# ghy1228/LDPC_Error_Floor

Measured on AMD Instinct MI355X. Metric: decoded codewords/sec, wman N576 R3/4, 20 NMS iters, higher is better.
Workload: dtype i32

## Files before the change

include/ldpc_nms.h:

```cpp
#ifndef LDPC_NMS_H
#define LDPC_NMS_H

#include <stdint.h>

#ifdef __cplusplus
extern "C" {
#endif

#define LDPC_NMS_ABI_VERSION 3

typedef struct ldpc_graph ldpc_graph;
typedef struct ldpc_ctx ldpc_ctx;

enum ldpc_status {
    LDPC_OK = 0,
    LDPC_ERR_ARG = -1,
    LDPC_ERR_HIP = -2,
    LDPC_ERR_OOM = -3,
    LDPC_ERR_STATE = -4,
    LDPC_ERR_UNSUPPORTED = -5
};

enum ldpc_decoding_type {
    LDPC_DEC_SP = 0,
    LDPC_DEC_MS = 1,
    LDPC_DEC_QMS = 2,
    LDPC_DEC_MS_NONUDGE = 3
};

enum ldpc_kernel {
    LDPC_KERNEL_AUTO = 0,
    LDPC_KERNEL_FLOOD = 1,
    LDPC_KERNEL_FUSED = 2
};

typedef struct ldpc_decode_params {
    int32_t T;
    int32_t decoding_type;
    int32_t q_bit;
    int32_t target_bits;
    float clip_llr;
    int32_t kernel;
    int32_t outputs_size;
    int32_t reserved;
} ldpc_decode_params;

typedef struct ldpc_decode_outputs {
    float* app_all;
    uint32_t* hard_bits;
    uint32_t* synd_bits;
    int64_t* counters;
    uint8_t* frame_flags;
    uint32_t* iter_wrong;
} ldpc_decode_outputs;

int ldpc_abi_version(void);
const char* ldpc_status_string(int status);

int ldpc_graph_create(const int32_t* proto, int32_t M, int32_t N, int32_t z, int32_t device,
                      ldpc_graph** out);
int ldpc_graph_destroy(ldpc_graph* g);
int ldpc_graph_query(const ldpc_graph* g, int32_t* dims);

int ldpc_weights_set(ldpc_graph* g, int32_t T, const float* alpha, const float* alpha_ucn,
                     const float* beta);

int ldpc_ctx_create(ldpc_graph* g, int64_t B_max, int32_t T_max, ldpc_ctx** out);
int ldpc_ctx_destroy(ldpc_ctx* c);

int ldpc_decode(ldpc_ctx* c, const float* llr_dev, int64_t B, const ldpc_decode_params* p,
                const ldpc_decode_outputs* o, void* stream);

int ldpc_kernel_info(const ldpc_ctx* c, const ldpc_decode_params* p, int64_t* bytes_per_cw,
                     char* name, int32_t name_len);

int ldpc_ctx_last_kernel(const ldpc_ctx* c, char* name, int32_t name_len);

int ldpc_channel_awgn(float* llr_dev, int64_t B, int32_t n_vars, double sigma, uint64_t seed,
                      int64_t offset, int32_t decoding_type, int32_t q_bit, int32_t punct_start,
                      int32_t punct_end, int32_t short_start, int32_t short_end, float clip_llr,
                      void* stream);

typedef struct ldpc_channel_params {
    double sigma;
    uint64_t seed;
    int64_t offset;
    int32_t punct_start, punct_end, short_start, short_end;
    int32_t reserved[4];
} ldpc_channel_params;

int ldpc_decode_awgn(ldpc_ctx* ctx, int64_t B, const ldpc_decode_params* params,
                     const ldpc_channel_params* channel, const ldpc_decode_outputs* outputs,
                     void* stream);

int ldpc_awgn_in_kernel(const ldpc_ctx* ctx, const ldpc_decode_params* params, int32_t has_short,
                        int32_t app);

typedef struct ldpc_es_outputs {
    int32_t size;
    int32_t reserved;
    int64_t* counters;
    uint8_t* frame_flags;
    uint8_t* n_iter;
    int64_t* iter_hist;
} ldpc_es_outputs;

int ldpc_decode_es(ldpc_ctx* ctx, const float* llr_dev, int64_t B, const ldpc_decode_params* params,
                   const ldpc_es_outputs* es_outputs, void* stream);
int ldpc_decode_awgn_es(ldpc_ctx* ctx, int64_t B, const ldpc_decode_params* params,
                        const ldpc_channel_params* channel, const ldpc_es_outputs* es_outputs,
                        void* stream);
int ldpc_es_supported(const ldpc_ctx* ctx, const ldpc_decode_params* params);

typedef struct ldpc_word_outputs {
    int32_t size;
    int32_t reserved;
    uint32_t* hard_last;
    uint8_t* word_flags;
    int64_t* counters;
    uint8_t* frame_flags;
} ldpc_word_outputs;

int ldpc_decode_word(ldpc_ctx* ctx, const float* llr_dev, int64_t B, const ldpc_decode_params* params,
                     const ldpc_word_outputs* word_outputs, void* stream);
int ldpc_word_supported(const ldpc_ctx* ctx, const ldpc_decode_params* params);

typedef struct ldpc_es_word_outputs {
    int32_t size;
    int32_t reserved;
    uint32_t* hard_stop;
    uint8_t* word_flags;
    int64_t* counters;
    uint8_t* frame_flags;
    uint8_t* n_iter;
    int64_t* iter_hist;
    uint64_t reserved1;
} ldpc_es_word_outputs;

int ldpc_decode_es_word(ldpc_ctx* ctx, const float* llr_dev, int64_t B, const ldpc_decode_params* params,
                        const ldpc_es_word_outputs* outputs, void* stream);
int ldpc_decode_awgn_es_word(ldpc_ctx* ctx, int64_t B, const ldpc_decode_params* params,
                             const ldpc_channel_params* channel, const ldpc_es_word_outputs* outputs,
                             void* stream);
int ldpc_es_word_supported(const ldpc_ctx* ctx, const ldpc_decode_params* params);

int ldpc_channel_awgn_rows(float* rows_dev, const int64_t* idx_dev, int64_t n, int32_t n_vars,
                           double sigma, uint64_t seed, int64_t offset, int32_t decoding_type,
                           int32_t q_bit, int32_t punct_start, int32_t punct_end,
                           int32_t short_start, int32_t short_end, float clip_llr, void* stream);

int ldpc_collect_frames(const uint8_t* flags_dev, int64_t B, uint32_t mask, uint32_t want,
                        int64_t* idx_dev, int64_t cap, int64_t* count_dev, void* stream);

int ldpc_gather_rows(const float* src_dev, int64_t n_cols, const int64_t* idx_dev, int64_t n,
                     float* dst_dev, void* stream);

#define LDPC_UNCOR_ROW_BOUND(n_cols) (13 + 48 * (int64_t)(n_cols))
int ldpc_format_uncor_rows(const float* rows, int64_t n, int64_t n_cols, char* out, int64_t cap,
                           int64_t* len);

#ifdef __cplusplus
}
#endif
#endif
```

include/ldpc_nms_debug.h:

```cpp
#ifndef LDPC_NMS_DEBUG_H
#define LDPC_NMS_DEBUG_H

#include <stdint.h>

#ifdef __cplusplus
extern "C" {
#endif

int ldpc_debug_bs_bounds(const int32_t* proto, int32_t M, int32_t N, int32_t z, int32_t T,
                         int32_t mode, int32_t alpha_uniform, int32_t beta_uniform, float clip,
                         int32_t flags, int32_t* violations, char* msg, int32_t msg_len);

#ifdef __cplusplus
}
#endif

#endif
```

ldpc_error_floor_amd/build.py:

```python
from __future__ import annotations

import argparse
import os
import shutil
import subprocess
import sys
import sysconfig
from concurrent.futures import ThreadPoolExecutor

PKG = os.path.dirname(os.path.abspath(__file__))
ROOT = os.path.dirname(PKG)
CSRC = os.path.join(PKG, "csrc")
INCLUDE = os.path.join(ROOT, "include")
BUILD = os.path.join(PKG, "_build")
ARCH = os.environ.get("LDPC_OFFLOAD_ARCH", "gfx950")

HIP_SOURCES = ["ldpc_capi.hip", "ldpc_flood.hip", "ldpc_fused.hip", "ldpc_fused5.hip",
               "ldpc_bs.hip", "ldpc_bsc.hip", "ldpc_ffl.hip", "ldpc_channel.hip", "ldpc_collect.hip",
               "ldpc_word.hip"]
HEADERS = ["ldpc_internal.h", "ldpc_fused.h", "ldpc_fused5_kernel.h", "ldpc_bs_kernel.h", "ldpc_bs_host.h", "ldpc_bitplane.h",
           "ldpc_awgn.h", "ldpc_host.h", "ldpc_quant.h"]
HOST_SOURCES = ["ldpc_host.cpp"]
F5_SHAPE_SRC = "ldpc_fused5_shape.hip"
BS_INST_SRC = "ldpc_bs_inst.hip"


def _table_count(header, decl):
    import re
    src = open(os.path.join(CSRC, header)).read()
    body = src.split(decl, 1)[1].split("\n};", 1)[0]
    return len(re.findall(r"^\s*\{", body, re.M))


def _f5_shape_count():
    return _table_count("ldpc_fused5_kernel.h", "constexpr Shape5 kShapes5[] = {")


def _bs_inst_count():
    return _table_count("ldpc_bs_kernel.h", "constexpr BsInst kBsInst[] = {")
LIB = os.path.join(PKG, "libldpc_nms.so")
EXT = os.path.join(PKG, "_ldpc_nms" + sysconfig.get_config_var("EXT_SUFFIX"))


BS_INST_FLAGS = ["-mllvm", "-amdgpu-use-amdgpu-trackers"]


def source_fingerprint() -> str:
    import hashlib
    h = hashlib.sha256()
    files = sorted(HIP_SOURCES + HEADERS + HOST_SOURCES + [F5_SHAPE_SRC, BS_INST_SRC])
    for f in files:
        with open(os.path.join(CSRC, f), "rb") as fh:
            h.update(f.encode() + b"\0" + fh.read())
    with open(os.path.join(INCLUDE, "ldpc_nms.h"), "rb") as fh:
        h.update(fh.read())
    h.update(" ".join(_flags()).encode())
    h.update(" ".join(BS_INST_FLAGS).encode())
    return h.hexdigest()[:16]


def _flags(absolute=False):
    inc = (INCLUDE, CSRC) if absolute else (os.path.relpath(INCLUDE, ROOT), os.path.relpath(CSRC, ROOT))
    return ["--offload-arch=" + ARCH, "-O3", "-std=c++17", "-fPIC", "-ffp-contract=off",
            "-I" + inc[0], "-I" + inc[1], "-Wall", "-Wno-unused-result",
            "-mllvm", "-pragma-unroll-threshold=500000"]


def _hipcc():
    for cand in (os.environ.get("HIPCC"), "/opt/rocm/bin/hipcc", shutil.which("hipcc")):
        if cand and os.path.exists(cand):
            return cand
    raise RuntimeError("hipcc not found (ROCm required to build the HIP extension)")


def _newer(target, deps):
    if not os.path.exists(target):
        return True
    t = os.path.getmtime(target)
    return any(os.path.getmtime(d) > t for d in deps if os.path.exists(d))


def _run(cmd):
    r = subprocess.run(cmd, capture_output=True, text=True)
    if r.returncode != 0:
        raise RuntimeError(f"build failed: {' '.join(cmd)}\n{r.stdout}\n{r.stderr}")
    return r


def build(force=False, jobs=4, verbose=False):
    os.makedirs(BUILD, exist_ok=True)
    hipcc = _hipcc()
    hdrs = [os.path.join(CSRC, h) for h in HEADERS] + [os.path.join(INCLUDE, "ldpc_nms.h")]
    flags = _flags(absolute=True)
    objs, jobs_list = [], []
    units = [(src, src.replace(".hip", ".o"), []) for src in HIP_SOURCES]
    units += [(src, src.replace(".cpp", ".o"), []) for src in HOST_SOURCES]
    units += [(F5_SHAPE_SRC, f"ldpc_fused5_s{i}.o", [f"-DF5_SHAPE={i}"])
              for i in range(_f5_shape_count())]
    units += [(BS_INST_SRC, f"ldpc_bs_i{i}.o", [f"-DBS_INST={i}"] + BS_INST_FLAGS)
              for i in range(_bs_inst_count())]
    for src, obj, defs in units:
        s = os.path.join(CSRC, src)
        o = os.path.join(BUILD, obj)
        objs.append(o)
        if force or _newer(o, [s] + hdrs + [os.path.abspath(__file__)]):
            jobs_list.append([hipcc] + flags + defs + ["-c", s, "-o", o])
    with ThreadPoolExecutor(max_workers=max(1, jobs)) as ex:
        for r in ex.map(_run, jobs_list):
            if verbose and r.stderr:
                print(r.stderr, file=sys.stderr)
    if force or _newer(LIB, objs):
        _run([hipcc, "--offload-arch=" + ARCH, "-shared", "-fPIC", "-o", LIB] + objs)
    py_src = os.path.join(CSRC, "pybind_module.cpp")
    if force or _newer(EXT, [py_src, LIB, os.path.join(INCLUDE, "ldpc_nms.h")]):
        import pybind11
        cxx = os.environ.get("CXX", "g++")
        _run([cxx, "-O2", "-std=c++17", "-shared", "-fPIC", "-fvisibility=hidden",
              "-I" + pybind11.get_include(), "-I" + sysconfig.get_paths()["include"],
              "-I" + INCLUDE, py_src, "-o", EXT, "-L" + PKG, "-lldpc_nms",
              "-Wl,-rpath,$ORIGIN"])
    return LIB, EXT


def main():
    ap = argparse.ArgumentParser()
    ap.add_argument("--force", action="store_true")
    ap.add_argument("--jobs", type=int, default=min(8, os.cpu_count() or 1))
    a = ap.parse_args()
    lib, ext = build(force=a.force, jobs=a.jobs, verbose=True)
    print(lib)
    print(ext)


if __name__ == "__main__":
    main()
```

ldpc_error_floor_amd/csrc/ldpc_bs.hip:

```cpp
#include <algorithm>
#include <array>
#include <cmath>
#include <cstdio>
#include <cstdlib>
#include <cstring>
#include <functional>
#include <string>
#include <utility>
#include <vector>

#include "ldpc_bs_host.h"

namespace ldpc {
namespace bs {

__global__ void k_bs_tables(const float* __restrict__ alpha, const float* __restrict__ alpha_ucn,
                            const float* __restrict__ beta, const int32_t* __restrict__ row_ptr,
                            int T, int E, int N, int arows, int ar, int bcols, float step, float inv,
                            int qmax, float cu, uint32_t* alut, uint32_t* blut) {
    const int f = blockIdx.x * blockDim.x + threadIdx.x;
    const int na = T * ar, nbt = T * bcols;
    if (f >= na + nbt) return;
    int g[16];
    uint32_t* out;
// ... 36 lines not shown
    int inst = -1, nw = 0, cn_lanes = 0, arows = 1, bcols = 1;
    uint32_t off_slots = 0, off_pad = 0, off_zero = 0, off_red = 0, off_alut = 0, off_blut = 0, off_hdz = 0,
             off_ch = 0, off_hdl = 0;
    uint32_t off_esu = 0;
    int cn_dmin = 0;
    bool ucn = false;
    bool colalign = false;
    float cu = 0.f;
    size_t lds = 0;
    std::vector<int32_t> lay;
};

static uint32_t q8_tab_lds(const BsPlan& p) { return p.off_slots; }
static bool q8_tab_fits(const BsPlan& p) {
    return (size_t)(p.off_pad - p.off_slots) >= sizeof(uint32_t) * AWGN_TAB_W;
}

static bool colalign_fits(const host::GraphTables& h, int nw_packed) {
    return h.z <= 32 && 32 * h.N <= 64 * 16 && (32 * h.N + 63) / 64 <= nw_packed + 1;
}

std::vector<int32_t> slot_layout_rows(const host::GraphTables& h, const std::vector<int>& rl, size_t* nslot) {
    std::vector<int32_t> lay((size_t)2 * h.M, 0);
    size_t cur = 0;
    for (int i = 0; i < h.M; ++i) {
        const int LPC = rl[(size_t)i], sep = 32 / LPC;
        auto ok = [&](int A) {
            for (int d = 1; d < LPC; ++d) {
                const int r = (d * A) % 32;
                if (std::min(r, 32 - r) < sep) return false;
            }
            return true;
        };
        const int deg = h.row_ptr[i + 1] - h.row_ptr[i];
        size_t first = cur;
        if (i > 0) first += (size_t)((((int64_t)lay[2 * (i - 1)] + h.z - (int64_t)cur) % 32 + 32) % 32);
        int A = ((deg + LPC - 1) / LPC) * h.z;
        while (!ok(A)) ++A;
        const int last_rows = (deg - (LPC - 1) + LPC - 1) / LPC;
        cur = first + (size_t)(LPC - 1) * A + (size_t)std::max(last_rows, 0) * h.z;
        lay[2 * i] = (int32_t)first;
        lay[2 * i + 1] = A;
    }
    *nslot = cur;
    return lay;
}
std::vector<int32_t> slot_layout(const host::GraphTables& h, int LPC, size_t* nslot) {
    return slot_layout_rows(h, std::vector<int>((size_t)h.M, LPC), nslot);
}

bool bs_mode(int mode) { return mode == MODE_Q5 || mode == MODE_QM5 || mode == MODE_Q4 || mode == MODE_Q3; }
float bs_step(int mode) { return mode == MODE_Q5 ? 0.5f : mode == MODE_Q3 ? 2.0f : 1.0f; }
int bs_qmax(int mode) { return mode == MODE_Q4 ? 7 : mode == MODE_Q3 ? 3 : QMAX; }
static float mode_step_bs(int mode) { return bs_step(mode); }

static BsPlan plan_inst(const DevGraph& g, int i, bool ucn, float clip, int min_cdeg, int mode, int T) {
    BsPlan p;
    const BsInst& k = kBsInst[i];
    const host::GraphTables& h = *g.host;
    if (h.max_cdeg > k.D || h.max_vdeg > k.DV || (ucn && !k.UCN)) return p;
    p.inst = i;
    p.ucn = ucn;
    const int nv = g.n_vars, nc = g.n_checks;
    p.cn_lanes = 64 * ((k.LPC * nc + 63) / 64);
    int vch = (nv + 63) / 64;
    const int cch = p.cn_lanes / 64;
    if (k.VPL == 1 && k.CPL == 1) {
        static const int eca = [] { const char* e = getenv("LDPC_BS_COLALIGN"); return e ? atoi(e) : 1; }();
        p.colalign = eca != 0 && colalign_fits(h, std::max(vch, cch));
        if (p.colalign) vch = (32 * h.N + 63) / 64;
    }
    if (k.VPL == 1 && k.CPL == 1) p.nw = std::max(vch, cch);
    else p.nw = std::max((vch + k.VPL - 1) / k.VPL, (cch + k.CPL - 1) / k.CPL);
    if (p.nw > 16) return p;
    if (k.VPL > 1 || k.CPL > 1) {
        p.nw = 16;
        if (vch > k.VPL * p.nw || cch > k.CPL * p.nw) return p;
    }
    const char* eap = getenv("LDPC_BS_AROWS");
    p.arows = ((g.w_alpha_uniform && !ucn) || (g.w_alpha_pair_uniform && !(eap && atoi(eap) == 0))) ? 1 : h.M;
    p.bcols = g.w_beta_uniform ? 1 : h.N;
    p.cn_dmin = (p.cn_lanes == k.LPC * nc) ? min_cdeg : 0;
    if (k.BIG) {
        const float cu = clip / mode_step_bs(mode);
        if (cu > (float)bs_qmax(mode)) p.cu = cu;
    }
    size_t nslot = 0;
    p.lay = slot_layout(h, k.LPC, &nslot);
    size_t o = 0;
    if (k.UCN) {
        p.off_hdz = (uint32_t)(4 * (size_t)nv);
        o = ((size_t)4 * (nv + 1) + 127) & ~(size_t)127;
    }
    p.off_slots = (uint32_t)o;
    p.off_pad = (uint32_t)(o + nslot * SLOT_B);
    p.off_zero = p.off_pad + SLOT_B;
    const size_t slot_end = (size_t)p.off_zero + SLOT_B;
    if (k.PK && slot_end > 65535) return p;
    if (k.UCN && p.off_hdz > 65535) return p;
    o = (slot_end + 15) & ~(size_t)15;
    p.off_red = (uint32_t)o;
    o += 64 + (((size_t)4 * T + 15) & ~(size_t)15) + 4 * FLORW;
    if (k.ES) {
        p.off_esu = (uint32_t)o;
        o += ((size_t)4 * T + 15) & ~(size_t)15;
    }
    p.off_alut = (uint32_t)o;
    o += (size_t)2 * (k.UCN ? 2 : 1) * p.arows * LUT_W * 4;
    p.off_blut = (uint32_t)o;
    o += (size_t)2 * p.bcols * BLUT_W * 4;
    if (k.PK && k.CPL == 1 && (k.ES ? (size_t)p.off_alut + (size_t)p.arows * LUT_W * 4 : o) > 65535) return p;
    if (k.CPL == 1) {
        p.off_ch = (uint32_t)o;
        o += (size_t)4 * 64 * p.nw;
    }
    if (k.UCN && k.CPL == 1) {
        const int EPL = (k.D + k.LPC - 1) / k.LPC, HDW = (EPL + 1) / 2;
        p.off_hdl = (uint32_t)o;
        o += (size_t)4 * HDW * 64 * p.nw;
    }
    p.lds = (o + 15) & ~(size_t)15;
    if (p.lds > BS_LDS_MAX) return p;
    p.ok = true;
    return p;
}

BsPlan bs_plan(const DevGraph& g, int mode, bool ucn, bool per_edge_w, float clip, int T, bool es = false) {
    BsPlan p;
    const char* e = getenv("LDPC_BS");
    if (e && atoi(e) == 0) return p;
    const char* el = getenv("LDPC_BS_LPC");
    const int want_lpc = el ? atoi(el) : 0;
    const char* ei = getenv("LDPC_BS_INST");
    const int want_inst = ei ? atoi(ei) : -1;
    if (!bs_mode(mode)) return p;
    if (per_edge_w || !g.host || !g.w_beta_nonneg) return p;
    const host::GraphTables& h = *g.host;
    int min_cdeg = 1 << 30;
    for (int i = 0; i < h.M; ++i) min_cdeg = std::min(min_cdeg, h.row_ptr[i + 1] - h.row_ptr[i]);
    if (min_cdeg < 2) return p;
    for (int i = 0; i < kBsNInst; ++i) {
        if (kBsInst[i].ES != es) continue;
        if (es) {
            BsPlan q = plan_inst(g, i, ucn, clip, min_cdeg, mode, T);
            if (q.ok) return q;
            continue;
        }
        if (want_lpc != 0 && want_lpc != kBsInst[i].LPC) continue;
        if (want_inst >= 0 && want_inst != i) continue;
        BsPlan q = plan_inst(g, i, ucn, clip, min_cdeg, mode, T);
        if (q.ok) return q;
    }
    return p;
}

#ifndef BS_DEAL_DEFAULT
#define BS_DEAL_DEFAULT 2
#endif
std::vector<int> deal_chunks(const std::vector<int>& cost, int nw, int cap) {
    const int n = (int)cost.size();
    std::vector<int> order(n), slot((size_t)nw * cap, -1);
    for (int c = 0; c < n; ++c) order[c] = c;
    std::stable_sort(order.begin(), order.end(), [&](int x, int y) { return cost[x] > cost[y]; });
    const char* e = getenv("LDPC_BS_DEAL");
    if (e && atoi(e) == 0) {
        std::vector<int> used(nw, 0), load(4, 0);
        for (int c : order) {
            int best = -1, bw = -1;
            for (int sm = 0; sm < 4; ++sm) {
                int w_s = -1;
                for (int w = sm; w < nw; w += 4)
                    if (used[w] < cap && (w_s < 0 || used[w] < used[w_s])) w_s = w;
                if (w_s >= 0 && (best < 0 || load[sm] < load[best])) { best = sm; bw = w_s; }
            }
            slot[(size_t)bw * cap + used[bw]] = c;
            ++used[bw];
            load[best] += cost[c];
        }
        return slot;
    }
    const int deal_mode = e ? atoi(e) : BS_DEAL_DEFAULT;
    if (deal_mode == 2 && cap == 1 && n <= nw && nw <= 16) {
        int slots[4] = {0, 0, 0, 0};
        for (int w = 0; w < nw; ++w) ++slots[w % 4];
        std::vector<int> cur(n, -1), best(n, -1);
        int load[4] = {0, 0, 0, 0}, used[4] = {0, 0, 0, 0};
        long long best_key = -1;
        std::function<void(int)> rec = [&](int i) {
            const int mx = std::max(std::max(load[0], load[1]), std::max(load[2], load[3]));
            if (best_key >= 0 && (long long)mx * 1000000 > best_key) return;
            if (i == n) {
                const long long key = (long long)mx * 1000000 + (long long)load[0] * load[0] + (long long)load[1] * load[1] +
                                      (long long)load[2] * load[2] + (long long)load[3] * load[3];
                if (best_key < 0 || key < best_key) { best_key = key; best = cur; }
                return;
            }
            for (int sm = 0; sm < 4; ++sm) {
                if (used[sm] >= slots[sm]) continue;
                bool dup = false;
                for (int q = 0; q < sm; ++q)
                    if (used[q] < slots[q] && load[q] == load[sm] && slots[q] - used[q] == slots[sm] - used[sm]) dup = true;
                if (dup) continue;
                load[sm] += cost[order[i]];
                ++used[sm];
                cur[i] = sm;
                rec(i + 1);
                load[sm] -= cost[order[i]];
                --used[sm];
            }
        };
        rec(0);
        int next[4] = {0, 1, 2, 3};
        for (int i = 0; i < n; ++i) {
            const int sm = best[i];
            slot[(size_t)next[sm]] = order[i];
            next[sm] += 4;
        }
        return slot;
    }
    std::vector<std::vector<int>> vch(nw);
    std::vector<int> vload(nw, 0);
    for (int c : order) {
        int best = -1;
        for (int w = 0; w < nw; ++w)
            if ((int)vch[w].size() < cap &&
                (best < 0 || vload[w] < vload[best] || (vload[w] == vload[best] && vch[w].size() < vch[best].size())))
                best = w;
        vch[best].push_back(c);
        vload[best] += cost[c];
    }
    std::vector<int> vorder(nw), sload(4, 0), next(4);
    for (int w = 0; w < nw; ++w) vorder[w] = w;
    std::stable_sort(vorder.begin(), vorder.end(), [&](int x, int y) { return vload[x] > vload[y]; });
    for (int sm = 0; sm < 4; ++sm) next[sm] = sm;
    for (int v : vorder) {
        int sm = -1;
        for (int q = 0; q < 4; ++q)
            if (next[q] < nw && (sm < 0 || sload[q] < sload[sm])) sm = q;
        const int w = next[sm];
        next[sm] += 4;
        sload[sm] += vload[v];
        for (size_t u = 0; u < vch[v].size(); ++u) slot[(size_t)w * cap + u] = vch[v][u];
    }
    return slot;
}

std::vector<int32_t> uniform_lanes(const host::GraphTables& h, int LPC, int cn_lanes) {
    std::vector<int32_t> lanes((size_t)cn_lanes, -1);
    const int nc = h.M * h.z;
    for (int ql = 0; ql < cn_lanes; ++ql)
        if (ql / LPC < nc) lanes[(size_t)ql] = (ql / LPC) | ((ql % LPC) << 16) | (LPC << 20);
    return lanes;
}

std::vector<int> check_chunk_cost_lanes(const host::GraphTables& h, const std::vector<int32_t>& lanes) {
    const int cch = (int)(lanes.size() / 64);
    std::vector<int> cost(cch, 2);
    for (int ch = 0; ch < cch; ++ch) {
        int pos = 0;
        for (int l = 0; l < 64; ++l) {
            const int32_t d = lanes[(size_t)64 * ch + l];
            if (d < 0) continue;
            const int i = (d & 0xFFFF) / h.z, L = (d >> 20) & 15;
            pos = std::max(pos, (h.row_ptr[i + 1] - h.row_ptr[i] + L - 1) / L);
        }
        cost[ch] += pos;
    }
    return cost;
}
std::vector<int> check_chunk_cost(const host::GraphTables& h, int LPC, int cch) {
    return check_chunk_cost_lanes(h, uniform_lanes(h, LPC, 64 * cch));
}

std::vector<int> column_rotation_lanes(const host::GraphTables& h, int EPL, const std::vector<int32_t>& lanes) {
    const int z = h.z, cn_lanes = (int)lanes.size();
    std::vector<int> toff(h.N, 0);
    {
        std::vector<std::vector<std::pair<int, int>>> grp;
        std::vector<std::vector<int>> bycol(h.N);
        for (int h0 = 0; h0 < cn_lanes; h0 += 32)
            for (int m = 0; m < EPL; ++m) {
                std::vector<std::pair<int, int>> gl;
                for (int ql = h0; ql < h0 + 32 && ql < cn_lanes; ++ql) {
                    const int32_t d = lanes[(size_t)ql];
                    if (d < 0) continue;
                    const int cc = d & 0xFFFF, cj = (d >> 16) & 15, LPC = (d >> 20) & 15;
                    const int i = cc / z, hc = cc - i * z, kk = LPC * m + cj;
                    if (kk >= h.row_ptr[i + 1] - h.row_ptr[i]) continue;
                    const int pe = h.row_ptr[i] + kk;
                    gl.emplace_back(h.pe_col[pe], (hc + h.pe_shift[pe]) % z);
                }
                if (gl.empty()) continue;
                for (const auto& x : gl)
                    if (bycol[x.first].empty() || bycol[x.first].back() != (int)grp.size())
                        bycol[x.first].push_back((int)grp.size());
                grp.push_back(std::move(gl));
            }
        auto gcost = [&](const std::vector<std::pair<int, int>>& gl) {
            int cnt[32] = {0}, mx = 0, sq = 0;
            uint32_t seen[32];
            int ns = 0;
            for (const auto& x : gl) {
                const uint32_t t = (uint32_t)(x.first * z + (x.second + toff[x.first]) % z);
                bool dup = false;
                for (int q = 0; q < ns && !dup; ++q) dup = seen[q] == t;
                if (dup) continue;
// ... 134 lines not shown
    int vcost_before = 0, vcost_after = 0;
    std::vector<uint32_t> A((size_t)64 * DV);
    std::vector<int> dl(64);
    for (int w = 0; w < p.nw; ++w)
        for (int u = 0; u < k.VPL; ++u) {
            const int ch = vslot[(size_t)w * k.VPL + u];
            int dmax = 0, dmin = 1 << 30;
            if (ch < 0) {
                wdeg[3 * ((size_t)u * p.nw + w)] = -1;
                wdeg[3 * ((size_t)u * p.nw + w) + 1] = 0;
                wdeg[3 * ((size_t)u * p.nw + w) + 2] = -1;
                continue;
            }
            int col = -2;
            std::fill(A.begin(), A.end(), p.off_zero);
            std::fill(dl.begin(), dl.end(), 0);
            for (int l = 0; l < 64; ++l) {
                const int o = 64 * ch + l;
                if (o >= nvo || order[o] < 0) { dmin = 0; continue; }
                const int v = order[o], j = v / z, hh = v - j * z;
                col = (col == -2 || col == j) ? j : -1;
                const int c0 = h.col_ptr[j], dv = h.col_ptr[j + 1] - c0;
                for (int f = 0; f < dv; ++f) {
                    const int pe = h.col_pe[c0 + f], i = h.pe_row[pe];
                    int hc = hh - h.pe_shift[pe];
                    hc = hc < 0 ? hc + z : hc;
                    A[(size_t)l * DV + f] = slot_addr(i, pe - h.row_ptr[i], hc);
                }
                dl[l] = dv;
                dmax = std::max(dmax, dv);
                dmin = std::min(dmin, dv);
            }
            if (vorder) {
                const std::pair<int, int> c = host::order_variable_edges(A, dl, DV, std::min(DV, dmax));
                vcost_before += c.first;
                vcost_after += c.second;
            }
            for (int l = 0; l < 64; ++l) {
                const int o = 64 * ch + l;
                if (o >= nvo || order[o] < 0) continue;
                uint32_t* q = &vn[((size_t)u * nl + 64 * w + l) * VNW];
                for (int pw = 0; pw < VNA; ++pw) q[pw] = 0u;
                for (int f = 0; f < DV; ++f) put(q, f, A[(size_t)l * DV + f]);
                q[VNA] = k.UCN ? ((uint32_t)order[o] | (hd_index(order[o]) << 16)) : (uint32_t)order[o];
            }
            wdeg[3 * ((size_t)u * p.nw + w)] = dmax;
            wdeg[3 * ((size_t)u * p.nw + w) + 1] = dmin;
            wdeg[3 * ((size_t)u * p.nw + w) + 2] = col < 0 ? -1 : col;
        }
    if (getenv("LDPC_BS_VORDER_LOG"))
        fprintf(stderr, "bsl variable-phase bank cycles per slot word: %d -> %d\n", vcost_before, vcost_after);
    const int cch = p.cn_lanes / 64;
    std::vector<int32_t> cchunk((size_t)p.nw * k.CPL, -1);
    if (k.CPL == 1 && k.VPL == 1) {
        for (int w = 0; w < p.nw; ++w) cchunk[w] = w < cch ? w : -1;
    } else {
        const std::vector<int> cs = deal_chunks(check_chunk_cost(h, LPC, cch), p.nw, k.CPL);
        for (size_t x = 0; x < cs.size(); ++x) cchunk[x] = cs[x];
    }
    std::vector<uint32_t> chd;
    if (k.UCN) {
        chd.assign((size_t)p.cn_lanes * HDW, 0u);
        for (int ql = 0; ql < p.cn_lanes; ++ql) {
            const int cc = ql / LPC, cj = ql % LPC;
            for (int m = 0; m < EPL; ++m) {
                uint32_t addr = p.off_hdz;
                const int kk = LPC * m + cj;
                if (cc < g.n_checks) {
                    const int i = cc / z, hc = cc - i * z;
                    if (kk < h.row_ptr[i + 1] - h.row_ptr[i]) {
                        const int pe = h.row_ptr[i] + kk;
                        const int v = h.pe_col[pe] * z + (hc + h.pe_shift[pe]) % z;
                        addr = 4 * hd_index(v);
                    }
                }
                chd[(size_t)ql * HDW + (m >> 1)] |= addr << (16 * (m & 1));
            }
        }
    }
    BsHostTables t;
    t.vn.swap(vn);
    t.wdeg.swap(wdeg);
    t.cchunk.swap(cchunk);
    t.chd.swap(chd);
    return t;
}
static int bs_graph_tables(const DevGraph& g, const BsPlan& p, void*& graph, int& inst, hipStream_t s) {
    if (graph && inst != p.inst) {
        (void)hipFree(graph);
        graph = nullptr;
    }
    if (graph) return LDPC_OK;
    BsHostTables t = bs_host_tables(g, p);
    const std::vector<uint32_t>& vn = t.vn;
    const std::vector<int32_t>& wdeg = t.wdeg;
    const std::vector<int32_t>& cchunk = t.cchunk;
    const std::vector<uint32_t>& chd = t.chd;
    const size_t nwords = vn.size() + wdeg.size() + p.lay.size() + cchunk.size() + chd.size();
    void* d = nullptr;
    if (hipMalloc(&d, nwords * 4) != hipSuccess) { (void)hipGetLastError(); return LDPC_ERR_OOM; }
    uint32_t* dp = reinterpret_cast<uint32_t*>(d);
    size_t at = 0;
    bool ok = true;
    auto up = [&](const void* src, size_t n) {
        if (n) ok = ok && hipMemcpyAsync(dp + at, src, n * 4, hipMemcpyHostToDevice, s) == hipSuccess;
        at += n;
    };
    up(vn.data(), vn.size());
    up(wdeg.data(), wdeg.size());
    up(p.lay.data(), p.lay.size());
    up(cchunk.data(), cchunk.size());
    up(chd.data(), chd.size());
    if (!ok || hipStreamSynchronize(s) != hipSuccess) {
        (void)hipFree(d);
        return LDPC_ERR_HIP;
    }
    graph = d;
    inst = p.inst;
    return LDPC_OK;
}

static BsPlan bs_route(const DevGraph& g, const BsReq& r, bool* to_bsc) {
    BsPlan p = bs_plan(g, r.mode, r.ucn, r.per_edge_w, r.clip, r.T, r.es);
    *to_bsc = !p.ok && (!r.es || !bs_plan(g, r.mode, r.ucn, r.per_edge_w, r.clip, r.T).ok);
    return p;
}

bool bs_supported(const DevGraph& g, const BsReq& r) {
    bool to_bsc;
    return bs_route(g, r, &to_bsc).ok || (to_bsc && bsc_supported(g, r));
}

bool bs_q8_ok(const DevGraph& g, const BsReq& r, bool has_short) {
    bool to_bsc;
    const BsPlan p = bs_route(g, r, &to_bsc);
    if (!p.ok) return to_bsc && bsc_q8_ok(g, r, has_short);
    return (!has_short || p.cu > 0.f) && q8_tab_fits(p);
}

const char* bs_kernel_name(const DevGraph& g, const BsReq& r) {
    static thread_local char buf[64];
    bool to_bsc;
    const BsPlan p = bs_route(g, r, &to_bsc);
    if (!p.ok) return to_bsc ? bsc_kernel_name(g, r) : "";
    const BsInst& k = kBsInst[p.inst];
    char x[16] = "";
    if (k.VPL > 1 || k.CPL > 1) snprintf(x, sizeof(x), ",x%d/%d", k.VPL, k.CPL);
    snprintf(buf, sizeof(buf), "bsl[p32,w%d,d%d,v%d,l%d%s%s%s]", p.nw, k.D, k.DV, k.LPC, x, p.ucn ? ",ucn" : "",
             r.es ? ",es" : "");
    return buf;
}

static int bs_run(const DevGraph& g, const Bufs& b, FusedWorkspace& ws, const BsPlan& p, const float* llr,
                  const BsReq& r, const BsOut& o, hipStream_t s) {
    void*& graph = r.es ? ws.bs_es_graph : ws.bs_graph;
    int st = bs_graph_tables(g, p, graph, r.es ? ws.bs_es_graph_inst : ws.bs_graph_inst, s);
    if (st != LDPC_OK) return st;
    const BsInst& k = kBsInst[p.inst];
    const float step = mode_step_bs(r.mode);
    const int ar = (k.UCN ? 2 : 1) * p.arows;
    uint32_t *alut = nullptr, *blut = nullptr;
    st = bs_make_tables(b, g, p.arows, ar, p.bcols, step, bs_qmax(r.mode), p.cu, r.ucn, ws, &alut, &blut, s);
    if (st != LDPC_OK) return st;
    const int DV = k.DV;
    const int VNW = (k.PK ? (DV + 1) / 2 : DV) + 1;
    const uint32_t* gt = reinterpret_cast<const uint32_t*>(graph);
    BsLaunch a{};
    a.n_iter = o.n_iter;
    a.iter_hist = o.iter_hist;
    a.hdw = o.hdw;
    a.word = o.word ? 1 : 0;
    a.llr = llr;
    a.gen = bs_gen(b, q8_tab_lds(p));
    a.B = b.B;
    a.n_vars = g.n_vars;
    a.n_checks = g.n_checks;
    a.T = b.T;
    a.target_bits = b.target_bits;
    a.cn_lanes = p.cn_lanes;
    a.cn_dmin = p.cn_dmin;
    a.fold_wave = p.cn_lanes < 64 * p.nw ? (uint32_t)(p.nw - 1) : (p.nw > 1 ? 1u : 0u);
    a.inv = 1.0f / step;
    a.cu = p.cu > 0.f ? p.cu : -1.f;
    a.qmax = bs_qmax(r.mode);
    a.ucn = p.ucn ? 1 : 0;
    a.ucn_iter = g.w_ucn_iter;
    a.beta_id = g.w_beta_id_mask;
    a.row_ptr = g.row_ptr;
    a.z = g.z;
    a.vn_tab = gt;
    const size_t nvt = (size_t)k.VPL * 64 * p.nw * VNW;
    a.vn_wdeg = reinterpret_cast<const int32_t*>(gt + nvt);
    a.row_lay = a.vn_wdeg + 3 * (size_t)k.VPL * p.nw;
    a.cn_chunk = a.row_lay + 2 * (size_t)g.M;
    a.cn_hd = reinterpret_cast<const uint32_t*>(a.cn_chunk + (size_t)p.nw * k.CPL);
    a.alut = alut;
    a.blut = blut;
    a.arows = p.arows;
    a.bcols = p.bcols;
    a.btid = (bs_qmax(r.mode) == QMAX && !getenv("LDPC_BS_NOBFIX")) ? g.beta_tid : nullptr;
    a.btid_n = g.N;
    a.counters = o.counters;
    a.flags = o.flags;
    a.bad = o.bad;
    a.iter_wrong = r.es ? nullptr : b.iter_wrong;
    a.hdx = o.hdx;
    bs_stagger(k.VPL > 1 || k.CPL > 1, &a.stagger, &a.stagger_n);
    a.off_slots = p.off_slots;
    a.off_pad = p.off_pad;
    a.off_zero = p.off_zero;
    a.off_red = p.off_red;
    a.off_alut = p.off_alut;
    a.off_blut = p.off_blut;
    a.off_hdz = p.off_hdz;
    a.off_hdl = p.off_hdl;
    a.off_ch = p.off_ch;
    if (const char* e = getenv("LDPC_DIAG_ABLATE")) a.ablate = atoi(e);
    const int npacks = (int)((b.B + PACK - 1) / PACK);
    int grid = -1;
    if (const char* e = getenv("LDPC_BS_GRID")) grid = std::max(atoi(e), 0);
    static const auto kLaunch = launch_table(std::make_integer_sequence<int, kBsNInst>{});
    static const size_t lds_min = [] { const char* e = getenv("LDPC_BS_LDS_MIN"); return e ? (size_t)atol(e) : 0; }();
    const size_t lds = std::min(std::max(p.lds, lds_min), (size_t)BS_LDS_MAX);
    const uint64_t rkey = (uint64_t)p.inst << 48 | (uint64_t)p.nw << 32 | (uint64_t)lds;
    if (ws.bs_resident_key != rkey) {
        ws.bs_resident_key = rkey;
        std::fill(ws.bs_resident, ws.bs_resident + 3, 0);
    }
#ifdef BS_STAMP
    static unsigned long long* dst = nullptr;
    if (!dst && hipMalloc(reinterpret_cast<void**>(&dst), 256 * 8) != hipSuccess) return LDPC_ERR_OOM;
    if (hipMemsetAsync(dst, 0, 256 * 8, s) != hipSuccess) return LDPC_ERR_HIP;
    a.stamps = dst;
    st = kLaunch[p.inst](a, npacks, p.nw, lds, s, b.q8 != nullptr, grid, ws.bs_resident);
    unsigned long long hst[256];
    if (st != LDPC_OK || hipMemcpyAsync(hst, dst, sizeof(hst), hipMemcpyDeviceToHost, s) != hipSuccess ||
        hipStreamSynchronize(s) != hipSuccess)
        return st != LDPC_OK ? st : LDPC_ERR_HIP;
    fprintf(stderr, "bs_stamp inst %d T %d q8 %d: per pack, shader clocks [check, check-barrier, var, var-barrier | "
            "entry, channel, ch-barrier, tables, first-var, check-setup | epilogue]\n", p.inst, b.T, b.q8 != nullptr);
    static const int order[] = {0, 1, 2, 3, 8, 9, 10, 11, 12, 4, 5};
    for (int w = 0; w < p.nw && w < 16; ++w) {
        const double n = (double)(hst[16 * w + 15] ? hst[16 * w + 15] : 1);
        fprintf(stderr, "  wave %2d:", w);
        for (const int i : order) fprintf(stderr, " %8.0f", hst[16 * w + i] / n);
        fprintf(stderr, "  | SIMD %5.3f %5.3f %5.3f %5.3f\n", (hst[16 * w + 13] & 0xFFFFFFFFull) / n,
                (hst[16 * w + 13] >> 32) / n, (hst[16 * w + 14] & 0xFFFFFFFFull) / n, (hst[16 * w + 14] >> 32) / n);
    }
    return st;
#else
    return kLaunch[p.inst](a, npacks, p.nw, lds, s, b.q8 != nullptr, grid, ws.bs_resident);
#endif
}

int bs_decode(const DevGraph& g, const Bufs& b, FusedWorkspace& ws, const float* llr, const BsReq& r,
              const BsOut& o, hipStream_t s) {
    bool to_bsc;
    const BsPlan p = bs_route(g, r, &to_bsc);
    if (!p.ok) return to_bsc ? bsc_decode(g, b, ws, llr, r, o, s) : LDPC_ERR_UNSUPPORTED;
    return bs_run(g, b, ws, p, llr, r, o, s);
}

}

namespace ldpc {
namespace bs {
struct BoundsReport {
    int violations = 0;
    std::string first;
    void fail(const char* what, long long idx, long long lim) {
        if (violations++ == 0) {
            char buf[160];
            snprintf(buf, sizeof(buf), "%s: index %lld outside [0, %lld)", what, idx, lim);
            first = buf;
        }
    }
    void in(const char* what, long long idx, long long lim) {
        if (idx < 0 || idx >= lim) fail(what, idx, lim);
    }
    void lds(const char* what, long long a, long long n, long long lo, long long hi) {
        if (a < lo || a + n > hi) fail(what, a, hi);
    }
    void apart(const char* what, long long a, long long n, long long b, long long m) {
        if (a < b + m && b < a + n) fail(what, a + n, b);
    }
};

static int bs_bounds_check(const DevGraph& g, const BsPlan& p, const BsHostTables& t, int T, int flags,
                           BoundsReport& r) {
    const BsInst& k = kBsInst[p.inst];
    const host::GraphTables& h = *g.host;
    const int LPC = k.LPC, VPL = k.VPL, CPL = k.CPL, DV = k.DV;
    const int EPL = (k.D + LPC - 1) / LPC, HDW = (EPL + 1) / 2, OB = 4 / LPC;
    const int VNA = k.PK ? (DV + 1) / 2 : DV, VNW = VNA + 1;
    const int NT = 64 * p.nw, nwv = p.nw, nv = g.n_vars, z = h.z;
    const bool UCN = k.UCN, ucn = UCN && (p.ucn || k.ES);
    const int AR = UCN ? 2 * p.arows : p.arows;
    const long long AL = (long long)AR * LUT_W, BL = (long long)p.bcols * BLUT_W;
    const long long lds = (long long)p.lds;
    const bool SKIPM = CPL > 1;
    const bool GBL = CPL == 1;
    const bool HDL = UCN && CPL == 1;
    if (getenv("LDPC_BOUNDS_VERBOSE"))
        fprintf(stderr, "bs plan: inst %d nw %d ucn %d lds %lld (slots %u..%u, alut %u, blut %u, ch %u, hdl %u)\n",
                p.inst, p.nw, (int)p.ucn, lds, p.off_slots, p.off_pad, p.off_alut, p.off_blut, p.off_ch, p.off_hdl);
    r.in("lds size", lds, (long long)BS_LDS_MAX + 1);
    if ((long long)t.vn.size() != (long long)VPL * NT * VNW) r.fail("vn_tab size", (long long)t.vn.size(), (long long)VPL * NT * VNW);
    r.lds("RED", p.off_red, 4LL * (16 + ((T + 3) & ~3) + FLORW), 0, k.ES ? p.off_esu : p.off_alut);
    if (k.ES) {
        r.lds("syndrome words", p.off_esu, 4LL * T, p.off_red, p.off_alut);
        r.apart("syndrome words / RED", p.off_esu, 4LL * T, p.off_red, 4LL * (16 + ((T + 3) & ~3) + FLORW));
        if (p.off_esu != p.off_red + 4u * (uint32_t)(16 + ((T + 3) & ~3) + FLORW)) r.fail("syndrome words' offset", p.off_esu, p.off_red);
        if (p.off_alut & 15) r.fail("alpha tables off 16 B", p.off_alut & 15, 1);
    }
    r.lds("ALUT", p.off_alut, 4 * 2 * AL, 0, p.off_blut);
    r.lds("BLUT", p.off_blut, 4 * 2 * BL, 0, lds);
    r.lds("PAD+ZERO", p.off_pad, 2 * SLOT_B, p.off_slots, p.off_red);
    if (UCN) r.lds("HD", 0, 4LL * (nv + 1), 0, p.off_slots);
    if (q8_tab_fits(p)) {
        const long long tb = q8_tab_lds(p);
        const long long tn = (flags & LDPC_BOUNDS_BIG_TABLES) ? (long long)(p.off_pad - p.off_slots) + 4
                                                              : 4LL * AWGN_TAB_W;
        r.lds("channel tables", tb, tn, p.off_slots, p.off_pad);
        if (UCN) r.apart("channel tables / HD", tb, tn, 0, 4LL * (nv + 1));
        r.apart("channel tables / PAD+ZERO", tb, tn, p.off_pad, 2 * SLOT_B);
        r.apart("channel tables / RED", tb, tn, p.off_red, (long long)p.off_alut - p.off_red);
        r.apart("channel tables / ALUT", tb, tn, p.off_alut, 4 * 2 * AL);
        r.apart("channel tables / BLUT", tb, tn, p.off_blut, 4 * 2 * BL);
    }
    for (int u = 0; u < VPL; ++u)
        for (int w = 0; w < nwv; ++w) {
            const long long wi = 3LL * (u * nwv + w);
            r.in("vn_wdeg", wi + 2, (long long)t.wdeg.size());
            if (wi + 2 >= (long long)t.wdeg.size()) continue;
            const int dw = t.wdeg[(size_t)wi], pcol = t.wdeg[(size_t)wi + 2];
            if (pcol >= 0) r.in("btid column", pcol, h.N);
            if (dw >= 0 && T > 1) {
                const long long col = p.bcols == 1 ? 0 : pcol;
                if (col >= 0) r.in("btid", (long long)(T - 1) * h.N + col, (long long)T * h.N);
            }
            for (int l = 0; l < 64; ++l) {
                const long long ti = ((long long)u * NT + 64LL * w + l) * VNW;
                r.in("vn_tab", ti + VNA, (long long)t.vn.size());
                if (ti + VNA >= (long long)t.vn.size()) continue;
                const uint32_t* q = &t.vn[(size_t)ti];
                const int vv = (int)q[VNA];
                const int v = (UCN && vv >= 0) ? (vv & 0xFFFF) : vv;
                if (v >= nv) r.fail("variable", v, nv);
                if (vv >= 0 && UCN) r.in("HD index", (long long)((uint32_t)vv >> 16), nv);
                if (vv >= 0 && p.bcols > 1) r.in("beta table", v / (nv / p.bcols), p.bcols);
                for (int f = 0; f < DV && f < dw; ++f) {
                    const uint32_t a = k.PK ? ((f & 1) ? (q[f >> 1] >> 16) : (q[f >> 1] & 0xFFFFu)) : q[f];
                    if (a != p.off_zero) r.lds("variable slot", a, SLOT_B, p.off_slots, p.off_pad);
                }
            }
        }
    for (int w = 0; w < nwv; ++w)
        for (int c = 0; c < CPL; ++c) {
            r.in("cn_chunk", (long long)w * CPL + c, (long long)t.cchunk.size());
            const int gchunk = CPL == 1 ? w : t.cchunk[(size_t)w * CPL + c];
            const bool active = CPL == 1 ? w * 64 < p.cn_lanes : gchunk >= 0;
            int gm = EPL;
            if (SKIPM) {
                uint32_t any = 0u;
                for (int l = 0; l < 64; ++l) {
                    const int ql = std::max(gchunk, 0) * 64 + l, cc = ql / LPC;
                    const int ci = std::min(cc / z, g.n_checks / z - 1);
                    const int gdeg = cc < g.n_checks ? h.row_ptr[ci + 1] - h.row_ptr[ci] : 0;
                    any |= (1u << ((gdeg + LPC - 1) / LPC)) - 1u;
                }
                gm = __builtin_popcount(any);
                if (active) r.in("real positions - 1 (the min2 switch)", gm - 1, EPL);
            }
            for (int l = 0; l < 64; ++l) {
                const int ql = std::max(gchunk, 0) * 64 + l, cc = ql / LPC, cj = l % LPC;
                const int ci = std::min(cc / z, g.n_checks / z - 1);
                r.in("row_ptr", ci + 1, h.M + 1);
                r.in("row_lay", 2LL * ci + 1, (long long)p.lay.size());
                const int gdeg = cc < g.n_checks ? h.row_ptr[ci + 1] - h.row_ptr[ci] : 0;
                if (UCN) {
                    const bool guard = (flags & LDPC_BOUNDS_PRE_GUARD) ? true : ql < p.cn_lanes;
                    if (ucn && gchunk >= 0 && guard)
                        for (int pp = 0; pp < HDW; ++pp) r.in("cn_hd", (long long)ql * HDW + pp, (long long)t.chd.size());
                }
                if (GBL) r.lds("per-lane words", p.off_ch + 4LL * (64 * w + l), 4, p.off_ch, lds);
                if (HDL)
                    for (int pp = 0; pp < HDW; ++pp) r.lds("HD addresses", p.off_hdl + 4LL * (pp * NT + 64 * w + l), 4, p.off_hdl, lds);
                if (!active) continue;
                const long long gbase = p.off_slots +
                    ((long long)p.lay[2 * ci] + (long long)cj * p.lay[2 * ci + 1] + (cc - ci * z)) * SLOT_B;
                for (int m = 0; m < EPL; ++m) {
                    if (SKIPM && m >= gm) continue;
                    const bool re = LPC * m + LPC - 1 < p.cn_dmin || LPC * m + cj < gdeg;
                    const long long a = re ? gbase + (long long)m * z * SLOT_B : p.off_pad;
                    r.lds("check slot", a, SLOT_B, p.off_slots, p.off_red);
                    if (re && a + SLOT_B > p.off_pad) r.fail("check slot past the slot region", a, p.off_pad);
                    if (ucn && cc < g.n_checks && ql < p.cn_lanes && (size_t)ql * HDW + (m >> 1) < t.chd.size()) {
                        const uint32_t hw = t.chd[(size_t)ql * HDW + (m >> 1)];
                        const uint32_t ha = (m & 1) ? (hw >> 16) : (hw & 0xFFFFu);
                        r.lds("HD read", ha, 4, 0, (long long)p.off_hdz + 4);
                    }
                }
                const long long ctab = p.off_alut + (long long)(p.arows > 1 ? ci : 0) * LUT_W * 4 + (long long)cj * OB * 64;
                const long long last = ctab + 4LL * AL + (UCN ? (long long)p.arows * LUT_W * 4 : 0) + (OB - 1) * 64 + 3 * 16;
                r.lds("alpha table", ctab, 16, p.off_alut, p.off_alut + 4 * 2 * AL);
                if (k.PK && CPL == 1) r.in("packed alpha-table address", ctab, 65536);
                r.lds("alpha table (odd t, alpha')", last, 16, p.off_alut, p.off_alut + 4 * 2 * AL);
            }
        }
    return r.violations;
}
}
}

extern "C" int ldpc_debug_bs_bounds(const int32_t* proto, int32_t M, int32_t N, int32_t z, int32_t T,
                                    int32_t mode, int32_t alpha_uniform, int32_t beta_uniform,
                                    float clip, int32_t flags, int32_t* violations, char* msg,
                                    int32_t msg_len) {
    using namespace ldpc;
    using namespace ldpc::bs;
    if (!proto || !violations || T <= 0) return LDPC_ERR_ARG;
    host::GraphTables h;
    const int st = host::build_graph(proto, M, N, z, h);
    if (st != LDPC_OK) return st;
    DevGraph g{};
    g.M = h.M; g.N = h.N; g.z = h.z; g.E = h.E;
    g.n_checks = h.M * h.z; g.n_vars = h.N * h.z; g.n_edges = h.E * h.z; g.max_cdeg = h.max_cdeg;
    g.h_row_ptr = h.row_ptr.data();
    g.host = &h;
    g.w_alpha_uniform = alpha_uniform;
    g.w_alpha_pair_uniform = alpha_uniform;
    g.w_beta_uniform = beta_uniform;
    g.w_beta_nonneg = 1;
    int min_cdeg = 1 << 30;
    for (int i = 0; i < h.M; ++i) min_cdeg = std::min(min_cdeg, h.row_ptr[i + 1] - h.row_ptr[i]);
    int checked = 0;
    *violations = 0;
    std::string first;
    for (int i = 0; i < kBsNInst; ++i)
        for (int u = 0; u < 2; ++u) {
            if (kBsInst[i].ES && !(flags & LDPC_BOUNDS_ES)) continue;
            const BsPlan p = plan_inst(g, i, u != 0, clip, min_cdeg, mode, T);
            if (!p.ok) continue;
            const BsHostTables t = bs_host_tables(g, p);
            BoundsReport r;
            bs_bounds_check(g, p, t, T, flags, r);
            ++checked;
            if (r.violations && first.empty()) {
                char buf[64];
                snprintf(buf, sizeof(buf), "instance %d%s: ", i, u ? " ucn" : "");
                first = std::string(buf) + r.first;
            }
            *violations += r.violations;
        }
    for (int b1 = 0; b1 < 2; ++b1) {
        if (b1 && !beta_uniform) continue;
        g.w_beta_one = b1;
        BoundsReport r;
        const int n = bsc_debug_bounds(g, mode, clip, T, flags, r.violations, r.first);
        if (n <= 0) continue;
        ++checked;
        if (r.violations && first.empty()) first = std::string(b1 ? "bsc beta=1: " : "bsc: ") + r.first;
        *violations += r.violations;
    }
    g.w_beta_one = 1;
    if ((flags & LDPC_BOUNDS_ES_BSC) && beta_uniform && !bs_plan(g, mode, false, false, clip, T).ok) {
        BoundsReport r;
        if (bsc_debug_bounds(g, mode, clip, T, flags, r.violations, r.first, true) > 0) {
            ++checked;
            if (r.violations && first.empty()) first = std::string("bsc early stop: ") + r.first;
            *violations += r.violations;
        }
    }
    if (msg && msg_len > 0) {
        std::strncpy(msg, first.c_str(), (size_t)msg_len - 1);
        msg[msg_len - 1] = 0;
    }
    return checked;
}
```

ldpc_error_floor_amd/csrc/ldpc_bs_kernel.h:

```cpp
#pragma once
#include <type_traits>
#include <cstdint>

#include "ldpc_beta_tabs.h"
#include "ldpc_fused.h"
#include "ldpc_fused5_kernel.h"
#include "ldpc_bitplane.h"

namespace ldpc {
namespace bs {

constexpr int PACK = 32;
constexpr int SLOT_W = 5;
constexpr int SLOT_B = SLOT_W * 4;
constexpr int LUT_W = 64;
constexpr int BLUT_W = LUT_W + 4;
constexpr int QMAX = 15;
constexpr size_t BS_LDS_MAX = 160 * 1024;

struct BsInst { int D, DV, LPC, VPL, CPL; bool UCN, BIG, PK; int WPE; bool ES = false; };
constexpr BsInst kBsInst[] = {
    {15, 6, 4, 1, 1, false, false, true, 8},
    {16, 8, 4, 1, 1, false, false, true, 8},
    {15, 6, 2, 1, 1, false, false, true, 8},
    {24, 4, 4, 1, 1, true, true, true, 6},
    {10, 8, 2, 2, 2, false, true, false, 4},
    {10, 8, 2, 2, 2, true, true, false, 4},
    {10, 8, 4, 2, 3, true, true, false, 4},
    {15, 6, 4, 1, 1, true, false, true, 6, true},
    {24, 4, 4, 1, 1, true, true, true, 6, true},
};
constexpr int kBsNInst = sizeof(kBsInst) / sizeof(kBsInst[0]);

struct BsGen {
    const uint32_t* tab;
    uint32_t k0, k1;
    int64_t offset;
    int nb, kmin;
    int ps, pe, ss, se;
    uint32_t lds;
};

struct BsArgs {
    const float* llr;
    int64_t B;
    int n_vars, n_checks, T, target_bits, cn_lanes, cn_dmin;
    float inv;
    float cu;
    int qmax;
    int ucn;
    uint64_t beta_id;
    const int32_t* row_ptr;
    const int32_t* row_lay;
    int z;
    const uint32_t* vn_tab;
    const int32_t* vn_wdeg;
    const int32_t* cn_chunk;
    const uint32_t* cn_hd;
    const uint32_t* alut;
    const uint32_t* blut;
    int arows, bcols;
    const int32_t* btid;
    int btid_n;
    int64_t* counters;
    uint8_t* flags;
    uint32_t* bad;
    uint32_t* iter_wrong;
    int stagger, stagger_n;
    uint32_t* hdx;
    uint32_t off_slots, off_pad, off_zero, off_red, off_alut, off_blut, off_hdz;
    uint32_t fold_wave;
    uint32_t off_ch;
    int ablate;
    uint64_t ucn_iter;
    uint32_t off_hdl;
    BsGen gen;
    unsigned long long* stamps;
};

struct BsArgsEs : BsArgs {
    uint8_t* n_iter;
    int64_t* iter_hist;
};

struct BsArgsEw : BsArgsEs {
    uint32_t* hdw;
};

struct BsArgsXp : BsArgs {
    int word;
};

template <class A>
__device__ __forceinline__ const __attribute__((address_space(4))) A& kern_args() {
    return *(const __attribute__((address_space(4))) A*)__builtin_amdgcn_kernarg_segment_ptr();
}

typedef unsigned int v4u __attribute__((ext_vector_type(4)));
typedef __attribute__((address_space(3))) uint32_t LdsW;
typedef __attribute__((address_space(3))) v4u LdsQ;

__device__ __forceinline__ uint32_t lds_w(uint32_t addr) { return *reinterpret_cast<const LdsW*>(addr); }
__device__ __forceinline__ v4u lds_q(uint32_t addr) { return *reinterpret_cast<const LdsQ*>(addr); }
__device__ __forceinline__ void lds_put(uint32_t addr, uint32_t x) { *reinterpret_cast<LdsW*>(addr) = x; }

__device__ __forceinline__ void read_slot(uint32_t& n, uint32_t (&M)[4], uint32_t addr) {
    const LdsW* p = reinterpret_cast<const LdsW*>(addr);
    n = p[0];
    M[0] = p[1];
    M[1] = p[2];
    M[2] = p[3];
    M[3] = p[4];
}
__device__ __forceinline__ void write_slot(uint32_t addr, uint32_t n, const uint32_t (&M)[4]) {
    LdsW* p = reinterpret_cast<LdsW*>(addr);
    p[0] = n;
    p[1] = M[0];
    p[2] = M[1];
    p[3] = M[2];
    p[4] = M[3];
}

template <int NI>
__device__ __forceinline__ void lut(uint32_t (&o)[NI][4], const uint32_t (&in)[NI][4], uint32_t tab) {
    uint32_t tj = tab;
#pragma unroll
    for (int j = 0; j < 4; ++j) {
        if (j > 0) asm volatile("" : "+v"(tj) : "v"(o[0][j - 1]));
        uint32_t g[NI][4];
#pragma unroll
        for (int q = 0; q < 4; ++q) {
            const v4u w = lds_q(tj + (uint32_t)(j * 64 + q * 16));
#pragma unroll
            for (int u = 0; u < NI; ++u) {
                const uint32_t l0 = B3(T_LEAF, in[u][0], w.x, w.y), l1 = B3(T_LEAF, in[u][0], w.z, w.w);
                g[u][q] = mux(in[u][1], l1, l0);
            }
        }
#pragma unroll
        for (int u = 0; u < NI; ++u)
            o[u][j] = mux(in[u][3], mux(in[u][2], g[u][3], g[u][2]), mux(in[u][2], g[u][1], g[u][0]));
    }
}

typedef __attribute__((address_space(4))) const uint32_t ConstW;
__device__ __forceinline__ uint32_t leaf_s(uint32_t m, uint32_t X, uint32_t Y) {
    uint32_t t, l;
    asm("v_and_b32 %0, %1, %2" : "=v"(t) : "s"(X), "v"(m));
    asm("v_xor_b32 %0, %1, %2" : "=v"(l) : "s"(Y), "v"(t));
    return l;
}
__device__ __forceinline__ void lut_s(uint32_t (&o)[4], const uint32_t (&a)[4], const ConstW* tab) {
#pragma unroll
    for (int j = 0; j < 4; ++j) {
        uint32_t g[4];
#pragma unroll
        for (int q = 0; q < 4; ++q) {
            const uint32_t l0 = leaf_s(a[0], tab[j * 16 + 4 * q], tab[j * 16 + 4 * q + 1]);
            const uint32_t l1 = leaf_s(a[0], tab[j * 16 + 4 * q + 2], tab[j * 16 + 4 * q + 3]);
            g[q] = mux(a[1], l1, l0);
// ... 134 lines not shown
    a = X[0][3] | cand[0];
#pragma unroll
    for (int m = 1; m < K; ++m) a = B3(T_ANDOR, a, X[m][3], cand[m]);
    a = grp_and<LPC>(a);
    m2[3] = a;
#pragma unroll
    for (int m = 0; m < K; ++m) c2[m] = B3(T_NANDEQ, cand[m], X[m][3], a);
#pragma unroll
    for (int i = 2; i >= 0; --i) {
        a = X[0][i] | ~c2[0];
#pragma unroll
        for (int m = 1; m < K; ++m) a = B3(T_ANDORN, a, X[m][i], c2[m]);
        a = grp_and<LPC>(a);
        m2[i] = a;
        if (i > 0) {
#pragma unroll
            for (int m = 0; m < K; ++m) c2[m] = B3(T_ANDEQ, c2[m], X[m][i], a);
        }
    }
#pragma unroll
    for (int i = 0; i < 4; ++i) m2[i] = mux(two, m1[i], m2[i]);
}

#ifdef BS_DIAG
#define ABL(bit) (a.ablate & (bit))
#else
#define ABL(bit) 0
#endif
#ifdef BS_MARK
#define PH(name, k) asm volatile(";@ph " name ".%0" ::"i"(k))
#define PH4(name, k, x) asm volatile(";@ph " name ".%4" : "+v"(x[0]), "+v"(x[1]), "+v"(x[2]), "+v"(x[3]) : "i"(k))
#define PH8(name, k, x, y)                                                                        \
    asm volatile(";@ph " name ".%8" : "+v"(x[0]), "+v"(x[1]), "+v"(x[2]), "+v"(x[3]), "+v"(y[0]),  \
                 "+v"(y[1]), "+v"(y[2]), "+v"(y[3]) : "i"(k))
#define PH9(name, k, x, y, z)                                                                     \
    asm volatile(";@ph " name ".%9" : "+v"(x[0]), "+v"(x[1]), "+v"(x[2]), "+v"(x[3]), "+v"(y[0]),  \
                 "+v"(y[1]), "+v"(y[2]), "+v"(y[3]), "+v"(z) : "i"(k))
#else
#define PH(name, k) ((void)0)
#define PH4(name, k, x) ((void)0)
#define PH8(name, k, x, y) ((void)0)
#define PH9(name, k, x, y, z) ((void)0)
#endif
__device__ __forceinline__ void t8x8(uint32_t& lo, uint32_t& hi) {
    uint32_t t;
    t = B3((TA ^ TB) & TC, lo, lo >> 7, 0x00AA00AAu);
    lo = B3(T_XOR3, lo, t, t << 7);
    t = B3((TA ^ TB) & TC, hi, hi >> 7, 0x00AA00AAu);
    hi = B3(T_XOR3, hi, t, t << 7);
    t = B3((TA ^ TB) & TC, lo, lo >> 14, 0x0000CCCCu);
    lo = B3(T_XOR3, lo, t, t << 14);
    t = B3((TA ^ TB) & TC, hi, hi >> 14, 0x0000CCCCu);
    hi = B3(T_XOR3, hi, t, t << 14);
    t = B3((TA ^ TB) & TC, lo, hi << 4, 0xF0F0F0F0u);
    lo ^= t;
    hi ^= t >> 4;
}
template <bool BIG>
__device__ __forceinline__ void pack_bytes(const uint32_t (&D)[8], uint32_t valid, uint32_t& cs,
                                           uint32_t (&cm)[4], uint32_t& bg) {
    uint32_t lo[4], hi[4];
#pragma unroll
    for (int g = 0; g < 4; ++g) {
        lo[g] = D[2 * g];
        hi[g] = D[2 * g + 1];
        t8x8(lo[g], hi[g]);
    }
    const uint32_t a = __builtin_amdgcn_perm(lo[1], lo[0], 0x06020400u), b = __builtin_amdgcn_perm(lo[1], lo[0], 0x07030501u);
    const uint32_t c = __builtin_amdgcn_perm(lo[3], lo[2], 0x06020400u), d = __builtin_amdgcn_perm(lo[3], lo[2], 0x07030501u);
    const uint32_t L0 = __builtin_amdgcn_perm(c, a, 0x05040100u) & valid, L2 = __builtin_amdgcn_perm(c, a, 0x07060302u) & valid;
    const uint32_t L1 = __builtin_amdgcn_perm(d, b, 0x05040100u) & valid, L3 = __builtin_amdgcn_perm(d, b, 0x07060302u) & valid;
    const uint32_t e = __builtin_amdgcn_perm(hi[1], hi[0], 0x05010400u), f = __builtin_amdgcn_perm(hi[3], hi[2], 0x05010400u);
    const uint32_t n = ~__builtin_amdgcn_perm(f, e, 0x05040100u) & valid;
    bg = BIG ? (__builtin_amdgcn_perm(f, e, 0x07060302u) & valid) : 0u;
    cs = n;
    cm[0] = L0;
    cm[1] = B3(T_XAND, L1, n, L0);
    cm[2] = B3(T_XAND, L2, n, L0 | L1);
    cm[3] = B3(T_XAND, L3, n, L0 | L1 | L2);
}
template <bool BIG>
__device__ __forceinline__ int pack_channel(const float (&xv)[PACK], float inv, int qmax, float cu,
                                            uint32_t valid, uint32_t& cs, uint32_t (&cm)[4], uint32_t& bg) {
    const float qf = (float)qmax;
    uint32_t D[8];
    int off = 0;
#pragma unroll
    for (int k = 0; k < 8; ++k) D[k] = 0u;
#pragma unroll
    for (int r = 0; r < PACK; ++r) {
        const float x = xv[r] * inv;
        const float q = __builtin_amdgcn_fmed3f(rintf(x), -qf, qf);
        const bool big = BIG && fabsf(x) == cu;
        off |= (q != x && !big) ? 1 : 0;
        D[r >> 2] = __builtin_amdgcn_cvt_pk_u8_f32(q + (big ? 48.f : 16.f), r & 3, D[r >> 2]);
    }
    pack_bytes<BIG>(D, valid, cs, cm, bg);
    return off;
}
typedef unsigned int v2u_g __attribute__((ext_vector_type(2)));
typedef __attribute__((address_space(3))) const v2u_g LdsU2;
__device__ __forceinline__ void gen_bytes(const BsGen& g, int64_t pk, int v, int qmax, uint32_t (&D)[8]) {
    const int bit = v + 1;
    if (g.ss > 0 && bit >= g.ss && bit <= g.se) {
#pragma unroll
        for (int i = 0; i < 8; ++i) D[i] = (uint32_t)(48 - qmax) * 0x01010101u;
        return;
    }
    if (g.ps > 0 && bit >= g.ps && bit <= g.pe) {
#pragma unroll
        for (int i = 0; i < 8; ++i) D[i] = 0x10101010u;
        return;
    }
    LdsU2* bucket = reinterpret_cast<LdsU2*>((uintptr_t)g.lds);
    const LdsW* thi = reinterpret_cast<const LdsW*>((uintptr_t)(g.lds + 8u * (1u << AWGN_KB)));
    const LdsW* tlo = thi + AWGN_NB_MAX;
    const uint64_t g0 = (uint64_t)g.offset + (uint64_t)pk * 32u;
    const int sh = (int)(g.offset & 3);
    const uint32_t boff = (uint32_t)(16 + g.kmin);
    auto word = [&](const int (&l)[4]) __attribute__((always_inline)) -> uint32_t {
        return ((uint32_t)l[0] + boff) | ((uint32_t)l[1] + boff) << 8 | ((uint32_t)l[2] + boff) << 16 |
               ((uint32_t)l[3] + boff) << 24;
    };
#pragma unroll
    for (int i = 0; i < 8; ++i) {
        const uint64_t gq = (g0 + 4u * (uint32_t)i) >> 2;
        int la[4];
        awgn_levels4b(g, bucket, thi, tlo, (uint32_t)v, gq, la);
        uint32_t w = word(la);
        if (sh) {
            int lb[4];
            awgn_levels4b(g, bucket, thi, tlo, (uint32_t)v, gq + 1, lb);
            w = __builtin_amdgcn_alignbyte(word(lb), w, (uint32_t)sh);
        }
        D[i] = w;
    }
}
__device__ __forceinline__ void gen_tables(const BsGen& g, int tid, int NT) {
    copy_async(g.lds, g.tab, AWGN_TAB_W, __builtin_amdgcn_readfirstlane(tid >> 6), NT);
}

constexpr double STAGGER_US = 60.0;
constexpr int FLORW = 32;
constexpr bool bs_loops(const BsInst& k) { return k.VPL == 1 && k.CPL == 1 && !k.UCN; }
#if defined(BS_INST) && BS_INST <= 2
#define BS_LOOP_TU 1
#else
#define BS_LOOP_TU 0
#endif
#define BS_PACK_SETUP(pk)                                                                          \
    const int64_t b0 = (int64_t)(pk) * PACK;                                                       \
    const int nvalid = (int)min<int64_t>(PACK, a.B - b0);                                          \
    const uint32_t valid = (nvalid >= 32) ? 0xFFFFFFFFu : ((1u << nvalid) - 1u);                   \
    uint32_t* RED = reinterpret_cast<uint32_t*>(smem + a.off_red);                                 \
    const int flor = 16 + ((a.T + 3) & ~3);                                                        \
    const int AR = UCN ? 2 * a.arows : a.arows;                                                    \
    const int AL = AR * LUT_W, BL = a.bcols * BLUT_W;                                              \
    uint32_t* ALUT = reinterpret_cast<uint32_t*>(smem + a.off_alut);                               \
    uint32_t* BLUT = reinterpret_cast<uint32_t*>(smem + a.off_blut);                               \
    const bool ucn = UCN && a.ucn;                                                                 \
    auto ucn_on = [&](int t) __attribute__((always_inline)) -> bool {                              \
        return ucn && (t >= 64 || ((a.ucn_iter >> t) & 1));                                        \
    };

template <int D, int DV, int LPC, int VPL, int CPL, bool UCN, bool BIG, bool PK, int WPE, bool XP, int LB, bool Q8,
          bool ES = false, bool EW = false>
__global__ void __launch_bounds__(LB) __attribute__((amdgpu_waves_per_eu(WPE)))
k_bs(std::conditional_t<ES, std::conditional_t<EW, BsArgsEw, BsArgsEs>, std::conditional_t<XP, BsArgsXp, BsArgs>> a) {
    static_assert(LPC == 2 || LPC == 4, "lanes per check");
    using KArgs = std::conditional_t<ES, std::conditional_t<EW, BsArgsEw, BsArgsEs>, std::conditional_t<XP, BsArgsXp, BsArgs>>;
    static_assert(!ES || (UCN && VPL == 1 && CPL == 1 && !XP), "early stop: one-chunk UCN-compiled instances");
    static_assert(!EW || ES, "the stop-iteration word: early-stop builds");
    constexpr int SB = (DV * QMAX + QMAX <= 127) ? 8 : 9;
    constexpr int EPL = (D + LPC - 1) / LPC;
    constexpr bool SKIPM = CPL > 1;
    constexpr int OB = 4 / LPC;
    constexpr int VNA = PK ? (DV + 1) / 2 : DV;
    constexpr int VNW = VNA + 1;
    constexpr int HDW = (EPL + 1) / 2;
    constexpr bool PKG = PK && CPL == 1;
    constexpr bool ONE = VPL == 1 && CPL == 1;
    constexpr int PRIO = ONE ? (DV >= 6 ? 4 : 2) : 0;
    constexpr int PROPRIO = PRIO == 4 ? 3 : 0;
    constexpr bool T0A = ONE;
    constexpr bool EBR = T0A;
    constexpr int SBSET = ONE ? 3 : 2;
    constexpr int KEEP0 = ONE ? 3 : (UCN ? 4 : 7);
    constexpr int KEEP = DV <= 4 ? DV : (KEEP0 < DV ? KEEP0 : DV - 1);
    constexpr bool BKPF = !XP && VPL > 1;
    extern __shared__ __attribute__((aligned(16))) unsigned char smem[];
    if ((uint32_t)(uintptr_t)smem != 0u) __builtin_trap();
#ifdef BS_STAMP
    uint64_t sacc[13] = {};
    uint64_t sts = __builtin_amdgcn_s_memtime();
#define BS_ST(i)                                                                                   \
    do {                                                                                           \
        const uint64_t tn_ = __builtin_amdgcn_s_memtime();                                         \
        sacc[i] += tn_ - sts;                                                                      \
        sts = tn_;                                                                                 \
    } while (0)
#else
#define BS_ST(i) ((void)0)
#endif
    const int tid = threadIdx.x;
    const int NT = blockDim.x;
    const int lane = tid & 63;
    const int wave = __builtin_amdgcn_readfirstlane(tid >> 6);
    const int nwv = NT >> 6;
    const int nv = a.n_vars;
#if !BS_LOOP_TU
    BS_PACK_SETUP(blockIdx.x)
#endif

    if (PROPRIO > 0) __builtin_amdgcn_s_setprio(PROPRIO);
    uint32_t va[VPL][VNA];
    int vv[VPL], dw[VPL], dwmin[VPL], pcol[VPL];
    uint32_t tab_b[VPL];
#pragma unroll
    for (int u = 0; u < VPL; ++u) {
        const uint32_t* vt = a.vn_tab + ((size_t)u * NT + tid) * VNW;
#pragma unroll
        for (int p = 0; p < VNA; ++p) va[u][p] = vt[p];
        vv[u] = (int)vt[VNA];
        dw[u] = __builtin_amdgcn_readfirstlane(a.vn_wdeg[3 * (u * nwv + wave)]);
        dwmin[u] = __builtin_amdgcn_readfirstlane(a.vn_wdeg[3 * (u * nwv + wave) + 1]);
        pcol[u] = __builtin_amdgcn_readfirstlane(a.vn_wdeg[3 * (u * nwv + wave) + 2]);
        tab_b[u] = (a.bcols > 1 && vv[u] >= 0) ? (uint32_t)(((UCN ? (vv[u] & 0xFFFF) : vv[u]) / (nv / a.bcols)) * BLUT_W * 4) : 0u;
    }
    constexpr int FOLDB = BS_LOOP_TU ? 0x100 : 0;
    int cn_dmin = a.cn_dmin | ((FOLDB && (uint32_t)wave == a.fold_wave) ? FOLDB : 0);

    if (a.stagger > 0 && (int)blockIdx.x < a.stagger_n) {
        const int n = (int)(((uint32_t)blockIdx.x * 97u % (uint32_t)a.stagger_n) * (uint32_t)a.stagger /
                            (uint32_t)a.stagger_n);
        for (int i = 0; i < n; ++i) __builtin_amdgcn_s_sleep(8);
    }
#if BS_LOOP_TU
    auto lane_now = [&]() __attribute__((always_inline)) -> int {
        uint32_t all = ~0u;
        asm volatile("" : "+s"(all));
        return (int)__builtin_amdgcn_mbcnt_hi(all, __builtin_amdgcn_mbcnt_lo(all, 0u));
    };
    unsigned pack = blockIdx.x;
#ifdef BS_STAMP
    unsigned long long npk = 0ull;
#endif
    do {
    if (pack != blockIdx.x) {
        __syncthreads();
        if (PROPRIO > 0) __builtin_amdgcn_s_setprio(PROPRIO);
    }
    typedef __attribute__((address_space(4))) const BsArgs PackArgs;
    PackArgs* kap = (PackArgs*)__builtin_amdgcn_kernarg_segment_ptr();
    asm volatile("" : "+s"(kap));
    PackArgs& a = *kap;
    const int tid = wave * 64 + lane_now(), lane = tid & 63;
    BS_PACK_SETUP(pack)
#define BS_PK pack
#define BS_NEXT_PACK continue
#define BS_LANE_IS0 (lane_now() == 0)
#else
#define BS_PK blockIdx.x
#define BS_NEXT_PACK return
#define BS_LANE_IS0 (lane == 0)
#endif
    if (tid < SLOT_W) {
        reinterpret_cast<uint32_t*>(smem + a.off_pad)[tid] = 0xFFFFFFFFu;
        reinterpret_cast<uint32_t*>(smem + a.off_zero)[tid] = 0u;
    }
    if (UCN && tid == 0) lds_put(a.off_hdz, 0u);
    if (tid < 8) RED[tid] = (tid == 1) ? 0xFFFFFFFFu : 0u;
#ifdef BS_STAMP
    if (tid == 0) {
        uint32_t hw0;
        asm volatile("s_getreg_b32 %0, hwreg(HW_REG_HW_ID)" : "=s"(hw0));
        RED[12] = (hw0 >> 4) & 3u;
    }
#endif
    if (tid < FLORW) RED[flor + tid] = 0u;
    [[maybe_unused]] uint32_t es_done = ~valid;
    if constexpr (ES) {
        for (int w = tid; w < a.T; w += NT) RED[flor + FLORW + w] = 0u;
    }
    [[maybe_unused]] uint32_t es_hd = 0u;
#if BS_LOOP_TU
    BsGen gen{};
    if constexpr (Q8) {
        gen.tab = a.gen.tab;
        gen.k0 = a.gen.k0;
        gen.k1 = a.gen.k1;
        gen.offset = a.gen.offset;
        gen.nb = a.gen.nb;
        gen.kmin = a.gen.kmin;
        gen.ps = a.gen.ps;
        gen.pe = a.gen.pe;
        gen.ss = a.gen.ss;
        gen.se = a.gen.se;
        gen.lds = a.gen.lds;
    }
#define BS_GEN gen
#else
#define BS_GEN a.gen
#endif
    if constexpr (Q8) gen_tables(BS_GEN, tid, NT);
    if (Q8 || !EBR) __syncthreads();
    BS_ST(8);
    uint32_t cs[VPL], cm[VPL][4], bg[VPL];
    int off = 0;
    if (T0A) {
        copy_async(a.off_alut, a.alut, AL, wave, NT);
        copy_async(a.off_blut, a.blut, BL, wave, NT);
    }
    const __amdgpu_buffer_rsrc_t llr_rs = __builtin_amdgcn_make_buffer_rsrc(
        (void*)(a.llr + b0 * nv), 0, nvalid * nv * 4, 0x00020000);
    auto llr_at = [&](int r, int v) __attribute__((always_inline)) -> float {
        return __builtin_bit_cast(float, __builtin_amdgcn_raw_buffer_load_b32(llr_rs, 4 * v, 4 * r * nv, 0));
    };
    auto var_of = [&](int u) __attribute__((always_inline)) -> int {
        return (UCN && vv[u] >= 0) ? (vv[u] & 0xFFFF) : vv[u];
    };
    float xv[VPL][PACK];
#if BS_LOOP_TU
#pragma unroll
    for (int r = 0; r < PACK; ++r) xv[0][r] = 0.f;
#endif
    if constexpr (Q8) {
#pragma unroll
        for (int u = 0; u < VPL; ++u) {
            cs[u] = 0u;
            bg[u] = 0u;
#pragma unroll
            for (int p = 0; p < 4; ++p) cm[u][p] = 0u;
            const int v = var_of(u);
            if (v >= 0 && !ABL(32)) {
                uint32_t Dq[8];
                gen_bytes(BS_GEN, BS_PK, v, a.qmax, Dq);
                pack_bytes<BIG>(Dq, valid, cs[u], cm[u], bg[u]);
            }
        }
    } else {
    if (var_of(0) >= 0 && !ABL(32)) {
#pragma unroll
        for (int r = 0; r < PACK; ++r) xv[0][r] = llr_at(r, var_of(0));
    }
    if (EBR) {
        asm volatile("" ::: "memory");
        __builtin_amdgcn_s_waitcnt(0xC07F);
        __builtin_amdgcn_s_barrier();
        asm volatile("" ::: "memory");
    }
#pragma unroll
    for (int u = 0; u < VPL; ++u) {
        cs[u] = 0u;
        bg[u] = 0u;
#pragma unroll
        for (int p = 0; p < 4; ++p) cm[u][p] = 0u;
        const int v = var_of(u);
        const int u1 = u + 1 < VPL ? u + 1 : u;
        const int vn = (u + 1 < VPL && !ABL(32)) ? var_of(u1) : -1;
        if (v >= 0 && !ABL(32))
            off |= pack_channel<BIG>(xv[u], a.inv, a.qmax, a.cu, valid, cs[u], cm[u], bg[u]);
        if (vn >= 0) {
#pragma unroll
            for (int r = 0; r < PACK; ++r) xv[u1][r] = llr_at(r, vn);
        }
    }
    }
    if (off) atomicOr(&RED[7], 1u);
    BS_ST(9);
    __syncthreads();
    BS_ST(10);
    if (RED[7]) {
        if constexpr (ES) {
            if (tid < nvalid) {
                if (a.flags) a.flags[b0 + tid] = 0x80;
                if (kern_args<KArgs>().n_iter) kern_args<KArgs>().n_iter[b0 + tid] = 0;
            }
        }
        if (tid == 0) a.bad[BS_PK] = 1u;
        BS_NEXT_PACK;
    }
    if (tid == 0) a.bad[BS_PK] = 0u;
    if (!T0A) {
        for (int w = tid; w < AL; w += NT) ALUT[w] = a.alut[w];
        for (int w = tid; w < BL; w += NT) BLUT[w] = a.blut[w];
        __syncthreads();
    }
    BS_ST(11);

    int bkp[VPL];
#pragma unroll
    for (int u = 0; u < VPL; ++u) bkp[u] = -1;
    auto beta_lw = [&](const int u, const uint32_t bslice, const int tb, const uint32_t (&cmu)[4],
                       uint32_t (&lw)[4], const bool use_bk) __attribute__((always_inline)) {
        int bk = -1;
        if constexpr (!XP) {
            if (use_bk && a.btid) {
                const int col = (a.bcols == 1) ? 0 : pcol[u];
                if (BKPF) bk = __builtin_amdgcn_readfirstlane(bkp[u]);
                else if (col >= 0)
                    bk = __builtin_amdgcn_readfirstlane((int)((const ConstW*)a.btid)[(size_t)tb * a.btid_n + col]);
            }
        }
        if (ABL(2) || (tb < 64 && ((a.beta_id >> tb) & 1))) {
            PH("vn_beta_id", u);
#pragma unroll
            for (int i = 0; i < 4; ++i) lw[i] = cmu[i];
        } else if (bk >= 0 && bk < kNBetaTab) {
            PH("vn_beta_fix", u);
            beta_asm(lw, cmu, bk);
            if constexpr (BIG) {
                if (a.bcols == 1) {
                    const ConstW* tg = (const ConstW*)(a.blut) + (size_t)tb * BLUT_W;
#pragma unroll
                    for (int i = 0; i < 4; ++i) lw[i] = mux(bg[u], tg[LUT_W + i], lw[i]);
                } else {
                    const v4u gb = lds_q(bslice + tab_b[u] + LUT_W * 4);
                    lw[0] = mux(bg[u], gb.x, lw[0]);
                    lw[1] = mux(bg[u], gb.y, lw[1]);
                    lw[2] = mux(bg[u], gb.z, lw[2]);
                    lw[3] = mux(bg[u], gb.w, lw[3]);
                }
            }
        } else if (a.bcols == 1) {
            PH("vn_beta_sg", u);
            const ConstW* tg = (const ConstW*)(a.blut) + (size_t)tb * BLUT_W;
            lut_s(lw, cmu, tg);
            if constexpr (BIG) {
#pragma unroll
                for (int i = 0; i < 4; ++i) lw[i] = mux(bg[u], tg[LUT_W + i], lw[i]);
            }
        } else {
            PH("vn_beta_lds", u);
            const uint32_t btab = bslice + tab_b[u];
            const uint32_t cmi[1][4] = {{cmu[0], cmu[1], cmu[2], cmu[3]}};
            uint32_t lo[1][4];
            lut<1>(lo, cmi, btab);
#pragma unroll
            for (int i = 0; i < 4; ++i) lw[i] = lo[0][i];
            if constexpr (BIG) {
                const v4u gb = lds_q(btab + LUT_W * 4);
                lw[0] = mux(bg[u], gb.x, lw[0]);
                lw[1] = mux(bg[u], gb.y, lw[1]);
                lw[2] = mux(bg[u], gb.z, lw[2]);
                lw[3] = mux(bg[u], gb.w, lw[3]);
            }
        }
    };
    auto vn_phase = [&](const bool first, const bool last, const uint32_t bslice, const int tb)
                        __attribute__((always_inline)) {
        (void)tid;
        uint32_t wr = 0u, apos = 0u, nb = 0u;
#pragma unroll
        for (int u = 0; u < VPL; ++u) {
            if (VPL > 1 && dw[u] < 0) continue;
            PH("vn_setup", (last ? 100 : 0) + u);
#pragma unroll
            for (int p = 0; p < VNA; ++p) asm volatile("" : "+v"(va[u][p]));
            auto vaddr = [&](int f) __attribute__((always_inline)) -> uint32_t {
                if constexpr (PK) return (f & 1) ? (va[u][f >> 1] >> 16) : (va[u][f >> 1] & 0xFFFFu);
                else return va[u][f];
            };
            const int v = (UCN && vv[u] >= 0) ? (vv[u] & 0xFFFF) : vv[u];
            const uint32_t hda = UCN ? 4u * ((uint32_t)vv[u] >> 16) : 0u;
            const uint32_t cmu[4] = {cm[u][0], cm[u][1], cm[u][2], cm[u][3]};
            const bool counted = v >= 0 && v < a.target_bits;
            uint32_t lw[1][4];
            PH("vn_beta", (last ? 100 : 0) + u);
            if (!last) beta_lw(u, bslice, tb, cmu, lw[0], !first);
            const int dwu = dw[u];
            auto vbody = [&](auto sbc) __attribute__((always_inline)) {
                constexpr int SB = decltype(sbc)::value;
                uint32_t mn[KEEP > 0 ? KEEP : 1], mb[KEEP > 0 ? KEEP : 1][4];
                uint32_t S[SB];
#pragma unroll
                for (int i = 0; i < SB; ++i) S[i] = 0u;
                if (!first) {
#pragma unroll
                    for (int f = 0; f < DV; ++f) {
                        if (f < dwu) {
                            PH("vn_sum", 1000 * (SB - 6) + (last ? 100 : 0) + 10 * u + f);
                            uint32_t M[4], n, b[4];
                            read_slot(n, M, vaddr(f));
#pragma unroll
                            for (int i = 0; i < 4; ++i) b[i] = M[i] ^ n;
                            if (f == 0) set_b<SB>(S, b, n);
                            else add_b<SB>(S, b, n);
                            if (f < KEEP) {
                                mn[f < KEEP ? f : 0] = n;
#pragma unroll
                                for (int i = 0; i < 4; ++i) mb[f < KEEP ? f : 0][i] = b[i];
                            }
                        }
                    }
                    if constexpr (SB == 8) PH8("vn_app", 1000 * (SB - 6) + (last ? 100 : 0) + u, S, (S + 4));
                    else PH("vn_app", 1000 * (SB - 6) + (last ? 100 : 0) + u);
                    uint32_t hd, nz = 0u;
                    const uint32_t c_s = cs[u];
                    if (last) {
                        uint32_t A[SB];
#pragma unroll
                        for (int i = 0; i < SB; ++i) A[i] = S[i];
                        const uint32_t cb[4] = {cmu[0] ^ c_s, cmu[1] ^ c_s, cmu[2] ^ c_s, cmu[3] ^ c_s};
                        add_b<SB>(A, cb, c_s);
                        hd = ~A[SB - 1];
#pragma unroll
                        for (int i = 0; i < SB; ++i) nz |= A[i];
                    } else {
                        uint32_t c = c_s;
#pragma unroll
                        for (int i = 0; i < SB - 1; ++i) c = B3(T_MAJ, S[i], i < 4 ? (cmu[i] ^ c_s) : c_s, c);
                        hd = B3(T_XNOR3, S[SB - 1], c_s, c);
                    }
                    if (UCN && !last && v >= 0 && (ES || ucn_on(tb))) lds_put(hda, hd);
                    hd &= valid;
                    if constexpr (XP) {
                        const bool word = kern_args<KArgs>().word != 0;
                        const size_t row = word ? (size_t)BS_PK : (size_t)(tb - 1) * (size_t)((a.B + 31) >> 5) + BS_PK;
                        if (v >= 0 && (last || !word)) a.hdx[row * nv + v] = hd;
                    }
                    if (ABL(8)) hd = 0u;
                    if (counted) {
                        wr |= hd;
                        if (last) {
                            apos |= hd & nz;
                            if constexpr (ES) nb += (uint32_t)__popc(hd & ~es_done);
                            else
                            nb += (uint32_t)__popc(hd);
                        }
                    }
                    if constexpr (EW) {
                        if (last) es_hd |= hd & ~es_done;
                    }
                }
                if (last) return;
                if constexpr (SB == 8) PH8("vn_tv", 1000 * (SB - 6) + (last ? 100 : 0) + u, S, (S + 4));
                else PH("vn_tv", 1000 * (SB - 6) + (last ? 100 : 0) + u);
                uint32_t lb[4];
#pragma unroll
                for (int i = 0; i < 4; ++i) lb[i] = lw[0][i] ^ cs[u];
                add_b<SB>(S, lb, cs[u]);
                uint32_t Tv[6];
                clamp6<SB>(Tv, S);
                const int dwm = dwmin[u];
                if (first) {
                    if (UCN && v >= 0 && ucn_on(0)) lds_put(hda, ~Tv[5]);
                    uint32_t x[7], X[4];
#pragma unroll
                    for (int i = 0; i < 7; ++i) x[i] = Tv[i < 6 ? i : 5];
                    abs_sat(X, x);
#pragma unroll
                    for (int f = 0; f < DV; ++f)
                        if (f < dwu && (f < dwm || vaddr(f) != a.off_zero)) write_slot(vaddr(f), x[6], X);
                } else {
#pragma unroll
                    for (int f = 0; f < DV; ++f) {
                        if (f < dwu) {
                            if (ABL(4)) continue;
                            PH("vn_vc", 1000 * (SB - 6) + (last ? 100 : 0) + 10 * u + f);
                            uint32_t x[7], X[4], n, b[4];
                            if (f < KEEP) {
                                n = mn[f < KEEP ? f : 0];
#pragma unroll
                                for (int i = 0; i < 4; ++i) b[i] = mb[f < KEEP ? f : 0][i];
                            } else {
                                uint32_t M[4];
                                read_slot(n, M, vaddr(f));
#pragma unroll
                                for (int i = 0; i < 4; ++i) b[i] = M[i] ^ n;
                            }
                            sub_tv(x, Tv, b, n);
                            abs_sat(X, x);
                            if (f < dwm || vaddr(f) != a.off_zero) write_slot(vaddr(f), x[6], X);
                        }
                    }
                }
            };
            if constexpr (SB >= 8) {
                if ((SBSET & 1) && dwu * QMAX + QMAX <= 63) vbody(std::integral_constant<int, 7>{});
                else if ((SBSET & 2) && SB == 9 && dwu * QMAX + QMAX <= 127) vbody(std::integral_constant<int, (SB == 9 ? 8 : SB)>{});
                else vbody(std::integral_constant<int, SB>{});
            } else {
                vbody(std::integral_constant<int, SB>{});
            }
        }
        if (!first && !last) {
            PH("vn_flags", 0);
            if (!ABL(8)) {
                const uint32_t la = __builtin_amdgcn_mbcnt_hi(~0u, __builtin_amdgcn_mbcnt_lo(~0u, 0u)) & 31u;
                __hip_atomic_fetch_or(RED + flor + la, wr, __ATOMIC_RELAXED, __HIP_MEMORY_SCOPE_WORKGROUP);
            }
        } else if (!first) {
            PH("vn_flags", last ? 100 : 0);
            if (!ABL(8)) wr = wave_or(wr);
            if (last) {
                apos = wave_or(apos);
                nb = wave_add(nb);
            }
            if (BS_LANE_IS0) {
                if (wr) atomicOr(&RED[0], wr);
                if (last) {
                    if (apos) atomicOr(&RED[2], apos);
                    if (nb) atomicAdd(&RED[3], nb);
                }
            }
        }
    };

    vn_phase(true, false, a.off_blut, 0);
    BS_ST(12);
    const int cj = lane % LPC;
    int gchunk[CPL], gdeg[CPL], gm[CPL];
    uint32_t gbase[CPL], gtab[CPL], ghd[CPL][UCN ? HDW : 1];
#pragma unroll
    for (int c = 0; c < CPL; ++c) {
        gchunk[c] = (CPL == 1) ? wave : __builtin_amdgcn_readfirstlane(a.cn_chunk[wave * CPL + c]);
        const int ql = max(gchunk[c], 0) * 64 + lane;
        const int cc = ql / LPC;
        const int ci = min(cc / a.z, a.n_checks / a.z - 1);
        gdeg[c] = (cc < a.n_checks) ? a.row_ptr[ci + 1] - a.row_ptr[ci] : 0;
        gm[c] = SKIPM ? (int)__popc(wave_or((1u << ((gdeg[c] + LPC - 1) / LPC)) - 1u)) : EPL;
        gbase[c] = a.off_slots + (uint32_t)((a.row_lay[2 * ci] + cj * a.row_lay[2 * ci + 1] + (cc - ci * a.z)) * SLOT_B);
        gtab[c] = a.off_alut + (uint32_t)((a.arows > 1 ? ci : 0) * LUT_W * 4) + (uint32_t)(cj * OB * 64);
        if constexpr (PKG) gbase[c] |= gtab[c] << 16;
        if constexpr (UCN) {
#pragma unroll
            for (int p = 0; p < HDW; ++p) ghd[c][p] = ((ES || ucn) && gchunk[c] >= 0 && ql < a.cn_lanes) ? a.cn_hd[(size_t)ql * HDW + p] : 0u;
        }
    }
    constexpr bool RPW = CPL > 1;
    constexpr int RB = EPL;
    static_assert(CPL * RB <= 32, "real-position word");
    static_assert(!SKIPM || EPL <= 8, "BS_MIN2_CASE covers 1..8");
    uint32_t rpk = 0u;
#pragma unroll
    for (int c = 0; c < CPL; ++c)
#pragma unroll
        for (int m = 0; m < EPL; ++m)
            if (RPW && (LPC * m + LPC - 1 < cn_dmin || LPC * m + cj < gdeg[c])) rpk |= 1u << (RB * c + m);
    const uint32_t cstride = (uint32_t)(a.z * SLOT_B);
    const uint32_t tabu = (uint32_t)(a.arows * LUT_W * 4);
    constexpr bool GBL = CPL == 1;
    if constexpr (GBL) lds_put(a.off_ch + 4u * (uint32_t)tid, gbase[0]);
    constexpr bool HDL = UCN && CPL == 1;
    if constexpr (HDL) {
#pragma unroll
        for (int p = 0; p < HDW; ++p) lds_put(a.off_hdl + 4u * (uint32_t)(p * NT + tid), ghd[0][p]);
    }
    __syncthreads();

    BS_ST(4);
    for (int t = 0; t < (ABL(16) ? 0 : a.T); ++t) {
        PH("top", 0);
        if (!ONE && wave == 0 && t > 0) {
            const uint32_t ln = __builtin_amdgcn_mbcnt_hi(~0u, __builtin_amdgcn_mbcnt_lo(~0u, 0u));
            uint32_t x = ln < 32u ? RED[flor + ln] : 0u;
            if (ln < 32u) RED[flor + ln] = 0u;
            const uint32_t w0 = wave_or(x);
            RED[16 + t - 1] = w0;
            RED[1] &= w0;
        }
        const int nx = (t + 1) & 1;
#pragma unroll
        for (int u = 0; u < VPL; ++u) asm volatile("" : "+s"(dw[u]), "+s"(dwmin[u]));
        if (!RPW) asm volatile("" : "+s"(cn_dmin));
        const int cdm = FOLDB ? (cn_dmin & (FOLDB - 1)) : cn_dmin;
        if (RPW) {
#pragma unroll
            for (int u = 0; u < VPL; ++u) asm volatile("" : "+v"(vv[u]));
        }
        if (t + 1 < a.T) {
            int cw = wave, al = AL, bl = BL, bcl = a.bcols;
            if (!(Q8 && VPL == 1 && CPL == 1 && !UCN))
                asm volatile("" : "+s"(cw), "+s"(al), "+s"(bl), "+s"(bcl));
            const uint32_t* alut_p = a.alut;
            const uint32_t* blut_p = a.blut;
            uint32_t off_al = a.off_alut, off_bl = a.off_blut;
            if constexpr (VPL == 1 && CPL == 1 && !(Q8 && !UCN)) {
                typedef __attribute__((address_space(4))) const BsArgs ConstArgs;
                ConstArgs* ka = (ConstArgs*)__builtin_amdgcn_kernarg_segment_ptr();
                asm volatile("" : "+s"(ka));
                alut_p = ka->alut;
                blut_p = ka->blut;
                off_al = ka->off_alut;
                off_bl = ka->off_blut;
            }
            copy_async(off_al + 4u * (uint32_t)(nx * al), alut_p + (size_t)(t + 1) * al, al, cw, NT);
            if (bcl > 1)
                copy_async(off_bl + 4u * (uint32_t)(nx * bl), blut_p + (size_t)(t + 1) * bl, bl, cw, NT);
        }
        if constexpr (BKPF) {
            if (t + 1 < a.T && a.btid) {
#pragma unroll
                for (int u = 0; u < VPL; ++u) {
                    const int col = (a.bcols == 1) ? 0 : pcol[u];
                    bkp[u] = col >= 0 ? a.btid[(size_t)(t + 1) * a.btid_n + col] : -1;
                }
            }
        }
        if (PRIO == 2) __builtin_amdgcn_s_setprio(1);
        if (PRIO == 4) __builtin_amdgcn_s_setprio(2);
#pragma unroll
        for (int c = 0; c < CPL; ++c) {
            const bool active = (CPL == 1) ? wave * 64 < a.cn_lanes : (gchunk[c] >= 0);
            if (!active || ABL(1)) continue;
            PH("ck_addr", c);
            uint32_t cbase;
            if constexpr (GBL) {
                uint32_t all = ~0u;
                asm volatile("" : "+s"(all));
                const uint32_t ln = __builtin_amdgcn_mbcnt_hi(all, __builtin_amdgcn_mbcnt_lo(all, 0u));
                cbase = lds_w(a.off_ch + ((uint32_t)wave << 8) + 4u * ln);
            } else {
                cbase = gbase[c];
                asm volatile("" : "+v"(cbase));
            }
            uint32_t ctab = PKG ? (cbase >> 16) : gtab[c];
            if constexpr (PKG) cbase &= 0xFFFFu;
            int gmc = gm[c];
            asm volatile("" : "+s"(gmc));
            uint32_t rp = rpk;
            if (RPW) asm volatile("" : "+v"(rp));
            const int cdeg = gdeg[c];
            auto real = [&](int m) __attribute__((always_inline)) -> bool {
                if constexpr (RPW) return ((rp >> (RB * c + m)) & 1u) != 0u;
                else return LPC * m + LPC - 1 < cdm || LPC * m + cj < cdeg;
            };
            auto caddr = [&](int m) __attribute__((always_inline)) -> uint32_t {
                return real(m) ? cbase + m * cstride : a.off_pad;
            };
            uint32_t Xs[EPL][4], ns[EPL];
            PH("ck_read", c);
#pragma unroll
            for (int m = 0; m < EPL; ++m) read_slot(ns[m], Xs[m], caddr(m));
            uint32_t syn = 0u;
            PH("ck_syn", c);
            const bool ucn_t = ucn_on(t);
            if constexpr (UCN) {
                if (ucn_t || (ES && t > 0)) {
                    uint32_t hwv[HDW];
                    if constexpr (HDL) {
                        uint32_t all = ~0u;
                        asm volatile("" : "+s"(all));
                        const uint32_t ln = __builtin_amdgcn_mbcnt_hi(all, __builtin_amdgcn_mbcnt_lo(all, 0u));
#pragma unroll
                        for (int p = 0; p < HDW; ++p)
                            hwv[p] = lds_w(a.off_hdl + 4u * (uint32_t)(p * NT) + ((uint32_t)wave << 8) + 4u * ln);
                    } else {
#pragma unroll
                        for (int p = 0; p < HDW; ++p) {
                            asm volatile("" : "+v"(ghd[c][p]));
                            hwv[p] = ghd[c][p];
                        }
                    }
#pragma unroll
                    for (int m = 0; m < EPL; ++m) {
                        if (SKIPM && m >= gmc) continue;
                        const uint32_t hw = hwv[m >> 1];
                        syn ^= lds_w((m & 1) ? (hw >> 16) : (hw & 0xFFFFu));
                    }
                    syn ^= qperm<QP_X1>(syn);
                    if (LPC == 4) syn ^= qperm<QP_X2>(syn);
                    if constexpr (ES) {
                        if (t > 0) {
                            const uint32_t wu = wave_or(syn);
                            if (wu && BS_LANE_IS0)
                                __hip_atomic_fetch_or(RED + flor + FLORW + (t - 1), wu,
                                                      __ATOMIC_RELAXED, __HIP_MEMORY_SCOPE_WORKGROUP);
                        }
                    }
                }
            }
            PH4("ck_min", c, Xs[EPL - 1]);
            uint32_t m1[4] = {Xs[0][0], Xs[0][1], Xs[0][2], Xs[0][3]}, m2[4] = {~0u, ~0u, ~0u, ~0u};
            uint32_t par = ns[0];
            uint32_t cand[EPL];
#pragma unroll
            for (int m = 1; m < EPL; ++m) par ^= ns[m];
            if constexpr (SKIPM) {
                switch (gmc) {
#define BS_MIN2_CASE(k)                                                                            \
    case k:                                                                                        \
        if constexpr (k <= EPL) {                                                                  \
            PH("ck_mink", 16 * c + k);                                                             \
            min2_bits<k, LPC>(m1, m2, cand, Xs);                                                   \
            _Pragma("unroll") for (int m = k; m < EPL; ++m) cand[m] = 0u;                          \
        } else {                                                                                   \
            __builtin_unreachable();                                                               \
        }                                                                                          \
        break;
                    BS_MIN2_CASE(1) BS_MIN2_CASE(2) BS_MIN2_CASE(3) BS_MIN2_CASE(4) BS_MIN2_CASE(5)
                    BS_MIN2_CASE(6) BS_MIN2_CASE(7) BS_MIN2_CASE(8)
#undef BS_MIN2_CASE
                    default:
                        __builtin_unreachable();
                }
            } else {
                min2_bits<EPL, LPC>(m1, m2, cand, Xs);
            }
            PH9("ck_merge", c, m1, m2, par);
            par ^= qperm<QP_X1>(par);
            if (LPC == 4) par ^= qperm<QP_X2>(par);
            uint32_t q1[4], q2[4];
            PH9("ck_tab", c, m1, m2, par);
            {
                const uint32_t mm[2][4] = {{m1[0], m1[1], m1[2], m1[3]}, {m2[0], m2[1], m2[2], m2[3]}};
                const uint32_t tab = ctab + (uint32_t)((t & 1) * AL * 4);
                uint32_t qb[OB][2];
                bool any_unsat = false;
                if constexpr (UCN) any_unsat = ucn_t && (CPL == 1 || __builtin_amdgcn_ballot_w64(syn != 0u) != 0ull);
#pragma unroll
                for (int b = 0; b < OB; ++b) {
                    uint32_t o[2];
                    lut_bit<2>(o, mm, tab + (uint32_t)(b * 64));
                    if constexpr (UCN) {
                        if (any_unsat) {
                            uint32_t ou[2];
                            lut_bit<2>(ou, mm, tab + tabu + (uint32_t)(b * 64));
                            o[0] = mux(syn, ou[0], o[0]);
                            o[1] = mux(syn, ou[1], o[1]);
                        }
                    }
                    qb[b][0] = o[0];
                    qb[b][1] = o[1];
                }
                if (LPC == 4) {
                    q1[0] = qperm<0x00>(qb[0][0]); q1[1] = qperm<0x55>(qb[0][0]);
                    q1[2] = qperm<0xAA>(qb[0][0]); q1[3] = qperm<0xFF>(qb[0][0]);
                    q2[0] = qperm<0x00>(qb[0][1]); q2[1] = qperm<0x55>(qb[0][1]);
                    q2[2] = qperm<0xAA>(qb[0][1]); q2[3] = qperm<0xFF>(qb[0][1]);
                } else {
                    q1[0] = qperm<0xA0>(qb[0][0]); q1[1] = qperm<0xA0>(qb[OB - 1][0]);
                    q1[2] = qperm<0xF5>(qb[0][0]); q1[3] = qperm<0xF5>(qb[OB - 1][0]);
                    q2[0] = qperm<0xA0>(qb[0][1]); q2[1] = qperm<0xA0>(qb[OB - 1][1]);
                    q2[2] = qperm<0xF5>(qb[0][1]); q2[3] = qperm<0xF5>(qb[OB - 1][1]);
                }
            }
#pragma unroll
            for (int m = 0; m < EPL; ++m) {
                if (m == 0) PH8("ck_pass2", 16 * c, q1, q2);
                if (real(m)) {
                    if (m > 0) PH("ck_pass2", 16 * c + m);
                    uint32_t Mg[4];
#pragma unroll
                    for (int i = 0; i < 4; ++i) Mg[i] = mux(cand[m], q2[i], q1[i]);
                    write_slot(cbase + m * cstride, par ^ ns[m], Mg);
                }
            }
        }
        if constexpr (ONE) {
            const bool folds = FOLDB ? (cn_dmin & FOLDB) != 0 : (uint32_t)wave == a.fold_wave;
            if (folds && t > 0) {
                const uint32_t ln = __builtin_amdgcn_mbcnt_hi(~0u, __builtin_amdgcn_mbcnt_lo(~0u, 0u));
                uint32_t x = ln < 32u ? RED[flor + ln] : 0u;
                if (ln < 32u) RED[flor + ln] = 0u;
                const uint32_t w0 = wave_or(x);
                RED[16 + t - 1] = w0;
                RED[1] &= w0;
            }
        }
        BS_ST(0);
        __syncthreads();
        BS_ST(1);
        if constexpr (ES) {
            if (t > 0) {
                const uint32_t un = (uint32_t)__builtin_amdgcn_readfirstlane((int)RED[flor + FLORW + t - 1]);
                const uint32_t nn = ~un & ~es_done;
                es_done |= nn;
                if (nn) {
                    const int v = vv[0] >= 0 ? (vv[0] & 0xFFFF) : -1;
                    uint32_t nb = 0u;
                    if constexpr (EW) {
                        if (v >= 0) {
                            const uint32_t h = lds_w(4u * ((uint32_t)vv[0] >> 16)) & nn;
                            es_hd |= h;
                            if (v < a.target_bits) nb = (uint32_t)__popc(h);
                        }
                    } else
                    if (v >= 0 && v < a.target_bits)
                        nb = (uint32_t)__popc(lds_w(4u * ((uint32_t)vv[0] >> 16)) & nn);
                    nb = wave_add(nb);
                    if (nb && BS_LANE_IS0) atomicAdd(&RED[3], nb);
                }
                if (es_done == 0xFFFFFFFFu) break;
            }
        }
        if (PRIO == 2) __builtin_amdgcn_s_setprio(0);
        if (PRIO == 4) {
            if (dw[0] >= DV - 1) __builtin_amdgcn_s_setprio(1);
            else __builtin_amdgcn_s_setprio(0);
        }
        const uint32_t bslice = a.off_blut + (uint32_t)(nx * BL * 4);
        if (t == a.T - 1) vn_phase(false, true, bslice, t + 1);
        else vn_phase(false, false, bslice, t + 1);
        BS_ST(2);
        __syncthreads();
        BS_ST(3);
    }
    int64_t* e_counters = a.counters;
    uint8_t* e_flags = a.flags;
    uint32_t* e_iter_wrong = a.iter_wrong;
    int64_t e_B = a.B;
    if constexpr (Q8 || (VPL == 1 && CPL == 1 && UCN)) {
        typedef __attribute__((address_space(4))) const BsArgs ConstArgs;
        ConstArgs* ka = (ConstArgs*)__builtin_amdgcn_kernarg_segment_ptr();
        asm volatile("" : "+s"(ka));
        e_counters = ka->counters;
        e_flags = ka->flags;
        e_iter_wrong = ka->iter_wrong;
        e_B = ka->B;
    }
#if BS_LOOP_TU
    const int te = wave * 64 + lane_now();
#else
    const int te = tid;
#endif
    if constexpr (EW) {
        uint32_t* hdw = kern_args<KArgs>().hdw;
        const int v = vv[0] >= 0 ? (vv[0] & 0xFFFF) : -1;
        if (hdw && v >= 0) hdw[(size_t)BS_PK * nv + v] = es_hd;
    }
    if constexpr (ES) {
        __syncthreads();
        if (wave == 0) {
            const uint32_t* ESU = RED + flor + FLORW;
            const int r = te & 31;
            const bool on = te < nvalid;
            int stop = a.T - 1;
            uint32_t all = 1u, wl = 0u;
            bool open = true;
            for (int t = 0; t < a.T; ++t) {
                const bool lastt = t == a.T - 1;
                const uint32_t w = lastt ? RED[0] : RED[16 + t];
                const uint32_t u = lastt ? 0u : ESU[t];
                if (open) {
                    wl = (w >> r) & 1u;
                    all &= wl;
                    if (!((u >> r) & 1u)) {
                        stop = t;
                        open = false;
                    }
                }
            }
            const unsigned long long mw = __builtin_amdgcn_ballot_w64(on && wl != 0u);
            const unsigned long long ma = __builtin_amdgcn_ballot_w64(on && all != 0u);
            if (on) {
                if (e_flags) e_flags[b0 + te] = (uint8_t)(all | (wl << 1));
                if (kern_args<KArgs>().n_iter) kern_args<KArgs>().n_iter[b0 + te] = (uint8_t)(stop + 1);
            }
            if (te == 0 && e_counters) {
                unsigned long long* cc = reinterpret_cast<unsigned long long*>(e_counters);
                const unsigned long long c0 = RED[3], c1 = __popcll(mw), c2 = __popcll(ma);
                if (c0) atomicAdd(cc + 0, c0);
                if (c1) atomicAdd(cc + 1, c1);
                if (c2) atomicAdd(cc + 2, c2);
            }
            if (kern_args<KArgs>().iter_hist) {
                unsigned long long rem = __builtin_amdgcn_ballot_w64(on);
                while (rem) {
                    const int l = __builtin_ctzll(rem);
                    const int ts = __builtin_amdgcn_readlane(stop, l);
                    const unsigned long long m = __builtin_amdgcn_ballot_w64(on && stop == ts);
                    if (te == l)
                        atomicAdd(reinterpret_cast<unsigned long long*>(kern_args<KArgs>().iter_hist) + ts,
                                  (unsigned long long)__popcll(m));
                    rem &= ~m;
                }
            }
        }
    }
    if constexpr (!ES) {
    if (te == 0) {
        const uint32_t wl = RED[0] & valid;
        const uint32_t all = RED[1] & RED[0] & valid;
        const uint32_t ap = RED[2] & valid;
        RED[16 + a.T - 1] = RED[0];
        if (e_counters) {
            unsigned long long* cc = reinterpret_cast<unsigned long long*>(e_counters);
            const unsigned long long c0 = RED[3], c1 = __popc(wl), c2 = __popc(all),
                                     c3 = 2ull * __popc(ap) + __popc(wl & ~ap);
            if (c0) atomicAdd(cc + 0, c0);
            if (c1) atomicAdd(cc + 1, c1);
            if (c2) atomicAdd(cc + 2, c2);
            if (c3) atomicAdd(cc + 3, c3);
        }
        RED[5] = all;
        RED[6] = wl;
    }
    if (e_flags || e_iter_wrong) {
        __syncthreads();
        if (e_flags && te < nvalid)
            e_flags[b0 + te] = (uint8_t)(((RED[5] >> te) & 1) | (((RED[6] >> te) & 1) << 1));
        if (e_iter_wrong)
            for (int t = te; t < a.T; t += NT)
                e_iter_wrong[(size_t)t * (size_t)((e_B + 31) >> 5) + BS_PK] = RED[16 + t] & valid;
    }
    }
    BS_ST(5);
#if BS_LOOP_TU
#ifdef BS_STAMP
    ++npk;
#endif
    } while ((pack += gridDim.x) < (unsigned)((a.B + PACK - 1) / PACK));
#elif defined(BS_STAMP)
    const unsigned long long npk = 1ull;
#endif
#undef BS_PK
#undef BS_NEXT_PACK
#undef BS_LANE_IS0
#undef BS_GEN
#ifdef BS_STAMP
    if (a.stamps && lane == 0 && wave < 16) {
#pragma unroll
        for (int i = 0; i < 13; ++i) atomicAdd(a.stamps + 16 * wave + i, (unsigned long long)sacc[i]);
        atomicAdd(a.stamps + 16 * wave + 15, npk);
        uint32_t hw;
        asm volatile("s_getreg_b32 %0, hwreg(HW_REG_HW_ID)" : "=s"(hw));
        const uint32_t simd = (((hw >> 4) & 3u) - reinterpret_cast<uint32_t*>(smem + a.off_red)[12]) & 3u;
        atomicAdd(a.stamps + 16 * wave + 13 + (simd >> 1), npk << (32 * (simd & 1)));
    }
#endif
#undef BS_ST
}

struct BsLaunch : BsArgsEw {
    int word;
};

template <class K>
K kernel_arg_of(void (*)(K));
template <class K, class L>
K bs_kernel_args(const L& a) {
    if constexpr (std::is_base_of_v<K, L>) return a;
    else return K{a, a.word};
}
template <auto Fn>
void bs_max_lds() {
    static const hipError_t once = hipFuncSetAttribute(reinterpret_cast<const void*>(Fn),
                                                       hipFuncAttributeMaxDynamicSharedMemorySize, (int)BS_LDS_MAX);
    (void)once;
}
template <auto Fn, class L>
int bs_launch_kernel(const L& a, int nblocks, int nw, size_t lds, hipStream_t s) {
    bs_max_lds<Fn>();
    hipLaunchKernelGGL(Fn, dim3(nblocks), dim3(64 * nw), lds, s, bs_kernel_args<decltype(kernel_arg_of(Fn))>(a));
    return hipGetLastError() == hipSuccess ? LDPC_OK : LDPC_ERR_HIP;
}

template <int I, bool XP, bool Q8>
int launch_bs_x(const BsLaunch& a, int npacks, int nw, size_t lds, hipStream_t s, int grid, int* resident) {
    constexpr BsInst k = kBsInst[I];
    static_assert(bs_loops(k) == (BS_LOOP_TU != 0), "BS_LOOP_TU lists the instances of bs_loops");
    constexpr auto fn = &k_bs<k.D, k.DV, k.LPC, k.VPL, k.CPL, k.UCN, k.BIG, k.PK, k.WPE, XP, 1024, Q8>;
    int nblocks = npacks;
    if constexpr (bs_loops(k)) {
        if (grid < 0) {
            if (*resident <= 0) {
                bs_max_lds<fn>();
                int dev = 0, ncu = 0, per_cu = 0;
                if (hipGetDevice(&dev) != hipSuccess ||
                    hipDeviceGetAttribute(&ncu, hipDeviceAttributeMultiprocessorCount, dev) != hipSuccess ||
                    hipOccupancyMaxActiveBlocksPerMultiprocessor(&per_cu, reinterpret_cast<const void*>(fn),
                                                                 64 * nw, lds) != hipSuccess ||
                    ncu <= 0 || per_cu <= 0) {
                    (void)hipGetLastError();
                    return LDPC_ERR_HIP;
                }
                *resident = ncu * per_cu;
            }
            grid = *resident;
        }
        if (grid > 0 && grid < npacks) nblocks = grid;
    }
    return bs_launch_kernel<fn>(a, nblocks, nw, lds, s);
}

template <int I, bool Q8, bool EW>
int launch_bs_es_x(const BsLaunch& a, int npacks, int nw, size_t lds, hipStream_t s) {
    constexpr BsInst k = kBsInst[I];
    static_assert(k.ES && !bs_loops(k), "an early-stop instance");
    return bs_launch_kernel<&k_bs<k.D, k.DV, k.LPC, k.VPL, k.CPL, k.UCN, k.BIG, k.PK, k.WPE, false, 1024, Q8, true, EW>>(
        a, npacks, nw, lds, s);
}
template <int I>
int launch_bs_any(const BsLaunch& a, int npacks, int nw, size_t lds, hipStream_t s, bool q8, int grid, int* resident) {
    if constexpr (kBsInst[I].ES) {
        if (a.hdx) return LDPC_ERR_UNSUPPORTED;
        if (a.hdw)
            return q8 ? launch_bs_es_x<I, true, true>(a, npacks, nw, lds, s)
                      : launch_bs_es_x<I, false, true>(a, npacks, nw, lds, s);
        return q8 ? launch_bs_es_x<I, true, false>(a, npacks, nw, lds, s)
                  : launch_bs_es_x<I, false, false>(a, npacks, nw, lds, s);
    } else {
        if (a.hdx) return q8 ? LDPC_ERR_UNSUPPORTED : launch_bs_x<I, true, false>(a, npacks, nw, lds, s, grid, resident + 1);
        return q8 ? launch_bs_x<I, false, true>(a, npacks, nw, lds, s, grid, resident + 2)
                  : launch_bs_x<I, false, false>(a, npacks, nw, lds, s, grid, resident);
    }
}

template <int I>
int bs_launch(const BsLaunch& a, int npacks, int nw, size_t lds, hipStream_t s, bool q8, int grid, int* resident);

}
}
```

ldpc_error_floor_amd/csrc/ldpc_capi.hip:

```cpp
#include <cstdio>
#include <cstring>
#include <functional>
#include <new>
#include <vector>

#include "ldpc_awgn.h"
#include "ldpc_internal.h"
#include "ldpc_fused.h"

using namespace ldpc;

struct ldpc_graph {
    int device = 0;
    host::GraphTables h;
    int32_t* d_tables = nullptr;
    DevGraph dev{};
    int T_w = 0;
    int per_edge_w = 0;
    std::vector<int32_t> row_merge;
    int32_t* d_row_merge = nullptr;
    float* d_alpha = nullptr;
    float* d_alpha_ucn = nullptr;
    float* d_beta = nullptr;
    int32_t* d_beta_tid = nullptr;
// ... 619 lines not shown
                              : c->fused.last_kernel;
    set_last_kernel(c, served, false, q8 || (gen && kern == LDPC_KERNEL_FUSED));

    if (count && kern == LDPC_KERNEL_FLOOD) {
        hipLaunchKernelGGL(k_finalize, dim3(std::min(1024, (ntiles + 255) / 256)), dim3(256), 0, s, b,
                           out.counters, out.frame_flags);
        if (out.iter_wrong) {
            const int64_t total = (int64_t)p->T * ((B + 31) / 32);
            hipLaunchKernelGGL(k_iter_wrong, dim3((unsigned)std::min<int64_t>(4096, (total + 255) / 256)),
                               dim3(256), 0, s, b, out.iter_wrong);
        }
    }
    if (want_bits) {
        HdSrc src{};
        src.npk = (B + 31) / 32;
        src.ntiles = ntiles;
        src.n_vars = g->h.N * g->h.z;
        if (kern == LDPC_KERNEL_FUSED) {
            const HdView v = fused_bits_view(c->fused);
            src.tile = v.tile;
            src.pack = v.pack;
            src.bad = v.bad;
        } else {
            src.tile = c->hd;
        }
        if (out.hard_bits) {
            const int nw = (g->h.N * g->h.z + 31) / 32;
            const int64_t total = (int64_t)p->T * B * nw;
            hipLaunchKernelGGL(k_export_hard, dim3((unsigned)std::min<int64_t>(4096, (total + 255) / 256)),
                               dim3(256), 0, s, src, B, out.hard_bits, p->T, nw);
        }
        if (out.synd_bits) {
            const int nw = (g->h.M * g->h.z + 31) / 32;
            const int64_t total = (int64_t)p->T * B * nw;
            hipLaunchKernelGGL(k_export_synd, dim3((unsigned)std::min<int64_t>(4096, (total + 255) / 256)),
                               dim3(256), 0, s, g->dev, src, B, out.synd_bits, p->T, nw);
        }
    }
    return hipGetLastError() == hipSuccess ? LDPC_OK : LDPC_ERR_HIP;
}

static int bs_request(const ldpc_ctx* c, int64_t B, const ldpc_decode_params* p, bool es, BsReq* r) {
    const ldpc_graph* g = c->g;
    if (!g->d_alpha || !g->d_beta) return LDPC_ERR_STATE;
    int mode = -1;
    const int chk = host::check_decode(g->h, B, c->B_max, c->T_max, g->T_w, p, &mode);
    if (chk != LDPC_OK) return chk;
    if (p->kernel != LDPC_KERNEL_AUTO && p->kernel != LDPC_KERNEL_FUSED)
        return p->kernel == LDPC_KERNEL_FLOOD ? LDPC_ERR_UNSUPPORTED : LDPC_ERR_ARG;
    *r = BsReq{mode, g->d_alpha_ucn != nullptr, false, p->clip_llr, p->T, es};
    if (p->decoding_type != LDPC_DEC_QMS || g->per_edge_w || !fused_bs_supported(g->dev, *r))
        return LDPC_ERR_UNSUPPORTED;
    return LDPC_OK;
}

static int bs_request_supported(const ldpc_ctx* c, const ldpc_decode_params* p, bool es) {
    if (!c || !p) return LDPC_ERR_ARG;
    BsReq r{};
    const int st = bs_request(c, 1, p, es, &r);
    return st == LDPC_OK ? 1 : st == LDPC_ERR_UNSUPPORTED ? 0 : st;
}
int ldpc_es_supported(const ldpc_ctx* c, const ldpc_decode_params* p) { return bs_request_supported(c, p, true); }
int ldpc_es_word_supported(const ldpc_ctx* c, const ldpc_decode_params* p) { return ldpc_es_supported(c, p); }
int ldpc_word_supported(const ldpc_ctx* c, const ldpc_decode_params* p) { return bs_request_supported(c, p, false); }

struct BsOuts {
    int64_t* counters;
    uint8_t *frame_flags, *n_iter;
    int64_t* iter_hist;
    uint32_t* rows;
    uint8_t* word_flags;
};
static BsOuts bs_outs(const ldpc_es_outputs* o) {
    return BsOuts{o->counters, o->frame_flags, o->n_iter, o->iter_hist, nullptr, nullptr};
}
static BsOuts bs_outs(const ldpc_es_word_outputs* o) {
    return BsOuts{o->counters, o->frame_flags, o->n_iter, o->iter_hist, o->hard_stop, o->word_flags};
}
static BsOuts bs_outs(const ldpc_word_outputs* o) {
    return BsOuts{o->counters, o->frame_flags, nullptr, nullptr, o->hard_last, o->word_flags};
}

static int decode_bs_impl(ldpc_ctx* c, const float* llr_dev, int64_t B, const ldpc_decode_params* p, bool es,
                          const BsOuts& o, void* stream, const uint32_t* q8, const AwgnParams* gen8) {
    BsReq r{};
    const int rq = bs_request(c, B, p, es, &r);
    if (rq != LDPC_OK) return rq;
    ldpc_graph* g = c->g;
    hipStream_t s = reinterpret_cast<hipStream_t>(stream);
    DeviceGuard dg(g->device);
    Bufs b = make_bufs(c, B, p);
    b.q8 = q8;
    b.gen8 = gen8;
    BsOut bo{};
    bo.counters = o.counters;
    bo.flags = o.frame_flags;
    bo.n_iter = o.n_iter;
    bo.iter_hist = o.iter_hist;
    const int st = fused_decode_bs(g->dev, b, c->fused, llr_dev, r, c->B_max, c->ntiles_max, bo, o.rows,
                                   o.word_flags, s);
    if (st != LDPC_OK) return st;
    set_last_kernel(c, bs_kernel_name(g->dev, r), o.rows != nullptr, q8 != nullptr);
    return hipGetLastError() == hipSuccess ? LDPC_OK : LDPC_ERR_HIP;
}

static int decode_awgn_es_impl(ldpc_ctx* c, int64_t B, const ldpc_decode_params* p, const ldpc_channel_params* ch,
                               const BsOuts& o, void* stream) {
    BsReq r{};
    const int st = bs_request(c, B, p, true, &r);
    if (st != LDPC_OK) return st;
    const bool q8 = awgn_q8_on() && bs_q8_ok(c->g->dev, r, ch->short_start > 0);
    return decode_awgn_with(c, B, p, ch, awgn_of(ch, p), q8, stream,
                            [&](const float* llr, const uint32_t* tab, const AwgnParams* gen8) {
                                return decode_bs_impl(c, llr, B, p, true, o, stream, tab, gen8);
                            });
}

int ldpc_decode_es(ldpc_ctx* c, const float* llr_dev, int64_t B, const ldpc_decode_params* p,
                   const ldpc_es_outputs* o, void* stream) {
    if (!c || !llr_dev || !p || !o || o->size != (int32_t)sizeof(ldpc_es_outputs)) return LDPC_ERR_ARG;
    return decode_bs_impl(c, llr_dev, B, p, true, bs_outs(o), stream, nullptr, nullptr);
}

int ldpc_decode_awgn_es(ldpc_ctx* c, int64_t B, const ldpc_decode_params* p, const ldpc_channel_params* ch,
                        const ldpc_es_outputs* o, void* stream) {
    if (!c || !p || !ch || !o || o->size != (int32_t)sizeof(ldpc_es_outputs) || !(ch->sigma > 0.0) ||
        ch->offset < 0)
        return LDPC_ERR_ARG;
    return decode_awgn_es_impl(c, B, p, ch, bs_outs(o), stream);
}

static_assert(sizeof(ldpc_es_word_outputs) == 64, "ldpc_es_word_outputs is part of ABI 3");
int ldpc_decode_es_word(ldpc_ctx* c, const float* llr_dev, int64_t B, const ldpc_decode_params* p,
                        const ldpc_es_word_outputs* o, void* stream) {
    if (!o || o->size != (int32_t)sizeof(ldpc_es_word_outputs) || !o->hard_stop) return LDPC_ERR_ARG;
    if (!c || !llr_dev || !p) return LDPC_ERR_ARG;
    return decode_bs_impl(c, llr_dev, B, p, true, bs_outs(o), stream, nullptr, nullptr);
}

int ldpc_decode_awgn_es_word(ldpc_ctx* c, int64_t B, const ldpc_decode_params* p, const ldpc_channel_params* ch,
                             const ldpc_es_word_outputs* o, void* stream) {
    if (!o || o->size != (int32_t)sizeof(ldpc_es_word_outputs) || !o->hard_stop) return LDPC_ERR_ARG;
    if (!c || !p || !ch || !(ch->sigma > 0.0) || ch->offset < 0) return LDPC_ERR_ARG;
    return decode_awgn_es_impl(c, B, p, ch, bs_outs(o), stream);
}

int ldpc_decode_word(ldpc_ctx* c, const float* llr_dev, int64_t B, const ldpc_decode_params* p,
                     const ldpc_word_outputs* o, void* stream) {
    if (!c || !llr_dev || !p || !o || o->size != (int32_t)sizeof(ldpc_word_outputs) || !o->hard_last)
        return LDPC_ERR_ARG;
    return decode_bs_impl(c, llr_dev, B, p, false, bs_outs(o), stream, nullptr, nullptr);
}

int ldpc_ctx_last_kernel(const ldpc_ctx* c, char* name, int32_t name_len) {
    if (!c || !name || name_len <= 0) return LDPC_ERR_ARG;
    std::strncpy(name, c->last_kernel, (size_t)name_len - 1);
    name[name_len - 1] = 0;
    return LDPC_OK;
}

}
```

ldpc_error_floor_amd/csrc/ldpc_fused.h:

```cpp
#pragma once
#include <string>

#include "ldpc_internal.h"

namespace ldpc {

struct FusedWorkspace {
    uint64_t* hd = nullptr;
    int64_t hd_elems = 0;
    void* tables = nullptr;
    size_t tables_bytes = 0;
    void* bs_graph = nullptr;
    int bs_graph_inst = -1;
    void* bs_es_graph = nullptr;
    int bs_es_graph_inst = -1;
    void* bs_lut = nullptr;
    size_t bs_lut_bytes = 0;
    uint32_t* bs_bad = nullptr;
    int64_t bs_bad_n = 0;
    int bs_resident[3] = {0, 0, 0};
    uint64_t bs_resident_key = ~0ull;
    uint32_t* hdx = nullptr;
    int64_t hdx_elems = 0;
    bool bits_packed = false;
    uint32_t* hdw = nullptr;
    int64_t hdw_elems = 0;
    const char* last_kernel = "";
    uint64_t key_gad[4] = {~0ull, 0, 0, 0}, key_qtab[4] = {~0ull, 0, 0, 0}, key_bslut[4] = {~0ull, 0, 0, 0};
};

template <class T, class N>
int dev_grow(T*& p, N& have, size_t n, size_t elem) {
    if ((size_t)have >= n) return LDPC_OK;
    if (p) (void)hipFree(p);
    p = nullptr;
    have = 0;
    if (hipMalloc(reinterpret_cast<void**>(&p), n * elem) != hipSuccess) {
        (void)hipGetLastError();
        return LDPC_ERR_OOM;
    }
    have = (N)n;
    return LDPC_OK;
}
template <class T, class N>
int dev_grow(T*& p, N& have, size_t n) { return dev_grow(p, have, n, sizeof(T)); }

bool fused_supported(const DevGraph& g, int mode, int T, float clip_llr);
int64_t fused_bytes_per_cw(const DevGraph& g, int T);
int fused_decode(const DevGraph& g, Bufs& b, FusedWorkspace& ws, const float* llr, int mode,
                 bool ucn, bool want_bits, int ntiles_max, int T_max, int per_edge_w,
                 int64_t* counters, uint8_t* flags, hipStream_t s);
struct HdView {
    const uint64_t* tile;
    const uint32_t* pack;
    const uint32_t* bad;
};
HdView fused_bits_view(const FusedWorkspace& ws);
const char* fused_kernel_name(const DevGraph& g, int mode, int T, float clip_llr, bool ucn,
                              bool per_edge_w);

bool fused5_supported(const DevGraph& g, int T);
const char* fused5_shape_name(const DevGraph& g, int T);
int fused5_decode(const DevGraph& g, const Bufs& b, FusedWorkspace& ws, const float* llr,
                  int qmax, float step, int clip_u, bool per_edge_w, uint64_t* hd_out,
                  int64_t* counters, uint8_t* flags, hipStream_t s, const uint32_t* only = nullptr);
int fused5_cw(const DevGraph& g, int T);

struct BsReq {
    int mode;
    bool ucn, per_edge_w;
    float clip;
    int T;
    bool es;
};
struct BsOut {
    int64_t* counters;
    uint8_t* flags;
    uint32_t* bad;
    uint32_t* hdx;
    bool word;
    uint8_t* n_iter;
    int64_t* iter_hist;
    uint32_t* hdw;
};
bool bs_supported(const DevGraph& g, const BsReq& r);
bool bs_q8_ok(const DevGraph& g, const BsReq& r, bool has_short);
const char* bs_kernel_name(const DevGraph& g, const BsReq& r);
bool bsc_supported(const DevGraph& g, const BsReq& r);
bool bsc_q8_ok(const DevGraph& g, const BsReq& r, bool has_short);
const char* bsc_kernel_name(const DevGraph& g, const BsReq& r);
int bs_decode(const DevGraph& g, const Bufs& b, FusedWorkspace& ws, const float* llr, const BsReq& r,
              const BsOut& o, hipStream_t s);
int bsc_decode(const DevGraph& g, const Bufs& b, FusedWorkspace& ws, const float* llr, const BsReq& r,
               const BsOut& o, hipStream_t s);
enum { LDPC_BOUNDS_PRE_GUARD = 1, LDPC_BOUNDS_BIG_TABLES = 2, LDPC_BOUNDS_ES = 4, LDPC_BOUNDS_ES_BSC = 8 };
int bsc_debug_bounds(const DevGraph& g, int mode, float clip, int T, int flags, int& violations,
                     std::string& first, bool es = false);
bool fused_q8_ok(const DevGraph& g, int mode, int T, float clip, bool ucn, bool per_edge_w, bool has_short);
bool fused_awgn_v5(const DevGraph& g, int mode, int T, float clip, bool ucn, bool per_edge_w, bool app);
constexpr int WORD_MAX_VARS = 4096;
bool fused_bs_supported(const DevGraph& g, const BsReq& r);
int fused_decode_bs(const DevGraph& g, const Bufs& b, FusedWorkspace& ws, const float* llr, const BsReq& r,
                    int64_t B_max, int ntiles_max, BsOut o, uint32_t* rows, uint8_t* word_flags, hipStream_t s);
int word_out(const DevGraph& g, const uint32_t* planes, const uint32_t* bad, int64_t B, uint32_t* hard_last,
             uint8_t* word_flags, uint8_t* frame_flags, hipStream_t s);
void fused_free(FusedWorkspace& ws);

bool ffl_mode(int mode);
bool ffl_supported(const DevGraph& g, int mode, bool ucn, bool per_edge_w);
const char* ffl_kernel_name(const DevGraph& g, int mode, bool ucn, bool per_edge_w);
int ffl_decode(const DevGraph& g, const Bufs& b, const float* llr, int mode, bool ucn, bool per_edge_w,
               int64_t* counters, uint8_t* flags, hipStream_t s);

}
```

ldpc_error_floor_amd/csrc/pybind_module.cpp:

```cpp
#include <pybind11/numpy.h>
#include <pybind11/pybind11.h>

#include <algorithm>
#include <stdexcept>
#include <string>

#include "ldpc_nms.h"

namespace py = pybind11;

static void check(int st, const char* what) {
    if (st < 0)
        throw std::runtime_error(std::string(what) + ": " + ldpc_status_string(st) + " (" +
                                 std::to_string(st) + ")");
}

struct Graph {
    ldpc_graph* h = nullptr;
    explicit Graph(py::array_t<int32_t, py::array::c_style | py::array::forcecast> proto, int z,
                   int device) {
        if (proto.ndim() != 2) throw std::invalid_argument("proto must be 2-D");
        check(ldpc_graph_create(proto.data(), (int32_t)proto.shape(0), (int32_t)proto.shape(1), z,
                                device, &h),
              "ldpc_graph_create");
// ... 221 lines not shown
        py::arg("n_iter") = 0, py::arg("iter_hist") = 0, py::arg("stream") = 0);
    m.def(
        "decode_awgn_es_word",
        [](Ctx& c, int64_t B, int T, int decoding_type, int q_bit, int target_bits, float clip,
           int kernel, double sigma, uint64_t seed, int64_t offset, int ps, int pe, int ss, int se,
           uintptr_t hard_stop, uintptr_t word_flags, uintptr_t counters, uintptr_t flags,
           uintptr_t n_iter, uintptr_t iter_hist, uintptr_t stream) {
            ldpc_decode_params p = make_params(T, decoding_type, q_bit, target_bits, clip, kernel);
            ldpc_channel_params ch = make_channel(sigma, seed, offset, ps, pe, ss, se);
            ldpc_es_word_outputs o = make_es_word_outputs(hard_stop, word_flags, counters, flags, n_iter, iter_hist);
            int st;
            {
                py::gil_scoped_release nogil;
                st = ldpc_decode_awgn_es_word(c.h, B, &p, &ch, &o, reinterpret_cast<void*>(stream));
            }
            check(st, "ldpc_decode_awgn_es_word");
        },
        py::arg("ctx"), py::arg("B"), py::arg("T"), py::arg("decoding_type"), py::arg("q_bit"),
        py::arg("target_bits"), py::arg("clip"), py::arg("kernel"), py::arg("sigma"),
        py::arg("seed"), py::arg("offset"), py::arg("punct_start"), py::arg("punct_end"),
        py::arg("short_start"), py::arg("short_end"), py::arg("hard_stop"), py::arg("word_flags") = 0,
        py::arg("counters") = 0, py::arg("flags") = 0, py::arg("n_iter") = 0, py::arg("iter_hist") = 0,
        py::arg("stream") = 0);
    m.def(
        "es_word_supported",
        [](Ctx& c, int T, int decoding_type, int q_bit, int target_bits, int kernel, float clip) {
            ldpc_decode_params p = make_params(T, decoding_type, q_bit, target_bits, clip, kernel);
            const int st = ldpc_es_word_supported(c.h, &p);
            check(st, "ldpc_es_word_supported");
            return st == 1;
        },
        py::arg("ctx"), py::arg("T"), py::arg("decoding_type"), py::arg("q_bit"),
        py::arg("target_bits"), py::arg("kernel"), py::arg("clip_llr") = 20.0f);
    m.def(
        "decode_word",
        [](Ctx& c, uintptr_t llr, int64_t B, int T, int decoding_type, int q_bit, int target_bits,
           float clip, int kernel, uintptr_t hard_last, uintptr_t word_flags, uintptr_t counters,
           uintptr_t flags, uintptr_t stream) {
            ldpc_decode_params p = make_params(T, decoding_type, q_bit, target_bits, clip, kernel);
            ldpc_word_outputs o{};
            o.size = (int32_t)sizeof(ldpc_word_outputs);
            o.hard_last = reinterpret_cast<uint32_t*>(hard_last);
            o.word_flags = reinterpret_cast<uint8_t*>(word_flags);
            o.counters = reinterpret_cast<int64_t*>(counters);
            o.frame_flags = reinterpret_cast<uint8_t*>(flags);
            int st;
            {
                py::gil_scoped_release nogil;
                st = ldpc_decode_word(c.h, reinterpret_cast<const float*>(llr), B, &p, &o,
                                      reinterpret_cast<void*>(stream));
            }
            check(st, "ldpc_decode_word");
        },
        py::arg("ctx"), py::arg("llr"), py::arg("B"), py::arg("T"), py::arg("decoding_type"),
        py::arg("q_bit"), py::arg("target_bits"), py::arg("clip"), py::arg("kernel"),
        py::arg("hard_last"), py::arg("word_flags") = 0, py::arg("counters") = 0, py::arg("flags") = 0,
        py::arg("stream") = 0);
    m.def(
        "word_supported",
        [](Ctx& c, int T, int decoding_type, int q_bit, int target_bits, int kernel, float clip) {
            ldpc_decode_params p = make_params(T, decoding_type, q_bit, target_bits, clip, kernel);
            const int st = ldpc_word_supported(c.h, &p);
            check(st, "ldpc_word_supported");
            return st == 1;
        },
        py::arg("ctx"), py::arg("T"), py::arg("decoding_type"), py::arg("q_bit"),
        py::arg("target_bits"), py::arg("kernel"), py::arg("clip_llr") = 20.0f);
    m.def(
        "channel_awgn",
        [](uintptr_t llr, int64_t B, int n_vars, double sigma, uint64_t seed, int64_t offset,
           int decoding_type, int q_bit, int ps, int pe, int ss, int se, float clip,
           uintptr_t stream) {
            int st;
            {
                py::gil_scoped_release nogil;
                st = ldpc_channel_awgn(reinterpret_cast<float*>(llr), B, n_vars, sigma, seed, offset,
                                       decoding_type, q_bit, ps, pe, ss, se, clip,
                                       reinterpret_cast<void*>(stream));
            }
            check(st, "ldpc_channel_awgn");
        },
        py::arg("llr"), py::arg("B"), py::arg("n_vars"), py::arg("sigma"), py::arg("seed"),
        py::arg("offset"), py::arg("decoding_type"), py::arg("q_bit"), py::arg("punct_start"),
        py::arg("punct_end"), py::arg("short_start"), py::arg("short_end"), py::arg("clip"),
        py::arg("stream") = 0);
    m.def(
        "channel_awgn_rows",
        [](uintptr_t rows, uintptr_t idx, int64_t n, int n_vars, double sigma, uint64_t seed,
           int64_t offset, int decoding_type, int q_bit, int ps, int pe, int ss, int se, float clip,
           uintptr_t stream) {
            check(ldpc_channel_awgn_rows(reinterpret_cast<float*>(rows), reinterpret_cast<const int64_t*>(idx),
                                         n, n_vars, sigma, seed, offset, decoding_type, q_bit, ps, pe,
                                         ss, se, clip, reinterpret_cast<void*>(stream)),
                  "ldpc_channel_awgn_rows");
        },
        py::arg("rows"), py::arg("idx"), py::arg("n"), py::arg("n_vars"), py::arg("sigma"),
        py::arg("seed"), py::arg("offset"), py::arg("decoding_type"), py::arg("q_bit"),
        py::arg("punct_start"), py::arg("punct_end"), py::arg("short_start"), py::arg("short_end"),
        py::arg("clip"), py::arg("stream") = 0);
    m.def(
        "collect_frames",
        [](uintptr_t flags, int64_t B, uint32_t mask, uint32_t want, uintptr_t idx, int64_t cap,
           uintptr_t count, uintptr_t stream) {
            check(ldpc_collect_frames(reinterpret_cast<const uint8_t*>(flags), B, mask, want,
                                      reinterpret_cast<int64_t*>(idx), cap,
                                      reinterpret_cast<int64_t*>(count),
                                      reinterpret_cast<void*>(stream)),
                  "ldpc_collect_frames");
        },
        py::arg("flags"), py::arg("B"), py::arg("mask"), py::arg("want"), py::arg("idx"),
        py::arg("cap"), py::arg("count"), py::arg("stream") = 0);
    m.def(
        "gather_rows",
        [](uintptr_t src, int64_t n_cols, uintptr_t idx, int64_t n, uintptr_t dst, uintptr_t stream) {
            check(ldpc_gather_rows(reinterpret_cast<const float*>(src), n_cols,
                                   reinterpret_cast<const int64_t*>(idx), n,
                                   reinterpret_cast<float*>(dst), reinterpret_cast<void*>(stream)),
                  "ldpc_gather_rows");
        },
        py::arg("src"), py::arg("n_cols"), py::arg("idx"), py::arg("n"), py::arg("dst"),
        py::arg("stream") = 0);
    m.def(
        "kernel_info",
        [](Ctx& c, int T, int decoding_type, int q_bit, int target_bits, int kernel, float clip) {
            ldpc_decode_params p = make_params(T, decoding_type, q_bit, target_bits, clip, kernel);
            int64_t bytes = 0;
            char name[64] = {0};
            check(ldpc_kernel_info(c.h, &p, &bytes, name, 64), "ldpc_kernel_info");
            return py::make_tuple(bytes, std::string(name));
        },
        py::arg("ctx"), py::arg("T"), py::arg("decoding_type"), py::arg("q_bit"),
        py::arg("target_bits"), py::arg("kernel"), py::arg("clip_llr") = 20.0f);
    m.def(
        "awgn_in_kernel",
        [](Ctx& c, int T, int decoding_type, int q_bit, int target_bits, int kernel, float clip,
           bool has_short, bool app) {
            ldpc_decode_params p = make_params(T, decoding_type, q_bit, target_bits, clip, kernel);
            const int r = ldpc_awgn_in_kernel(c.h, &p, has_short ? 1 : 0, app ? 1 : 0);
            check(r < 0 ? r : 0, "ldpc_awgn_in_kernel");
            return r == 1;
        },
        py::arg("ctx"), py::arg("T"), py::arg("decoding_type"), py::arg("q_bit"),
        py::arg("target_bits"), py::arg("kernel"), py::arg("clip_llr") = 20.0f,
        py::arg("has_short") = false, py::arg("app") = false);
    m.def(
        "last_kernel",
        [](Ctx& c) {
            char name[64] = {0};
            check(ldpc_ctx_last_kernel(c.h, name, 64), "ldpc_ctx_last_kernel");
            return std::string(name);
        },
        py::arg("ctx"));
    m.def(
        "format_uncor_rows",
        [](py::array_t<float, py::array::c_style | py::array::forcecast> rows) {
            if (rows.ndim() != 2 || rows.shape(1) <= 0)
                throw std::invalid_argument("rows must be [n, n_cols] with n_cols > 0");
            const int64_t n = rows.shape(0), nc = rows.shape(1);
            const int64_t step = std::max<int64_t>(1, (64 << 20) / LDPC_UNCOR_ROW_BOUND(nc));
            std::string out, buf;
            out.reserve((size_t)(n * (12 + 6 * nc)));
            buf.resize((size_t)(std::min(n, step) * LDPC_UNCOR_ROW_BOUND(nc)));
            {
                py::gil_scoped_release nogil;
                for (int64_t r0 = 0; r0 < n; r0 += step) {
                    const int64_t k = std::min(step, n - r0);
                    int64_t len = 0;
                    check(ldpc_format_uncor_rows(rows.data() + r0 * nc, k, nc, buf.data(),
                                                 (int64_t)buf.size(), &len),
                          "ldpc_format_uncor_rows");
                    out.append(buf.data(), (size_t)len);
                }
            }
            return py::bytes(out);
        },
        py::arg("rows"));
}
```

ldpc_error_floor_amd/decoder.py:

```python
from __future__ import annotations

from dataclasses import dataclass
from typing import Optional

import numpy as np

from . import _native
from .code import TannerGraph
from .config import DECODING_MS, DECODING_MS_NONUDGE, DECODING_QMS, DECODING_SP, VALID_Q_BITS
from .weights import DecoderWeights

__all__ = ["NMSDecoder", "Decoder", "DecodeResult", "KERNELS"]

KERNELS = {"auto": 0, "flood": 1, "fused": 2}


@dataclass
class DecodeResult:
    app: Optional["object"] = None
    hard: Optional["object"] = None
    synd: Optional["object"] = None
    counters: Optional["object"] = None
    flags: Optional["object"] = None
    iter_wrong: Optional["object"] = None
# ... 181 lines not shown
        if B == 0:
            return res
        ctx = self._ensure_ctx(B, T)
        if stream is None:
            stream = torch.cuda.current_stream(dev)
        ptr = lambda t: 0 if t is None else t.data_ptr()
        outs = (res.hard_last.data_ptr(), ptr(res.word_flags), ptr(res.counters), ptr(res.flags),
                ptr(res.n_iter), ptr(res.iter_hist), stream.cuda_stream)
        if channel is not None:
            sigma, seed, offset, punct, short = channel
            self._ext.decode_awgn_es_word(ctx, B, T, self.decoding_type, self.q_bit, nt, self.clip,
                                          KERNELS[kernel or self.kernel], float(sigma), int(seed), int(offset),
                                          int(punct[0]), int(punct[1]), int(short[0]), int(short[1]), *outs)
            return res
        self._ext.decode_es_word(ctx, llr.data_ptr(), B, T, self.decoding_type, self.q_bit, nt, self.clip,
                                 KERNELS[kernel or self.kernel], *outs)
        if on_off_grid == "raise":
            self._raise_off_grid(res, stream, "early_stop", word_flags)
        return res

    def _es_outputs(self, res, B, T, counters, flags, n_iter, iter_hist):
        torch = self._torch
        dev = self.device
        if counters is True:
            counters = torch.zeros(4, dtype=torch.int64, device=dev)
        if counters is not None:
            if counters.dtype != torch.int64 or counters.numel() < 4 or counters.device != dev:
                raise ValueError("counters must be an int64[4] tensor on the decoder's device")
            res.counters = counters
        if isinstance(flags, torch.Tensor):
            if flags.dtype != torch.uint8 or flags.device != dev or flags.numel() < B:
                raise ValueError("flags tensor must be uint8 on the decoder's device, >= B long")
            res.flags = flags
        elif flags:
            res.flags = torch.empty(B, dtype=torch.uint8, device=dev)
        if n_iter:
            res.n_iter = torch.empty(B, dtype=torch.uint8, device=dev)
        if iter_hist is True:
            iter_hist = torch.zeros(T, dtype=torch.int64, device=dev)
        if iter_hist is not None and iter_hist is not False:
            if (not isinstance(iter_hist, torch.Tensor) or iter_hist.dtype != torch.int64 or
                    iter_hist.numel() < T or iter_hist.device != dev or not iter_hist.is_contiguous()):
                raise ValueError("iter_hist must be a contiguous int64[T] tensor on the decoder's device")
            res.iter_hist = iter_hist
        return res

    @staticmethod
    def _es_check_exports(**exports):
        bad = [k for k, v in exports.items() if v]
        if bad:
            raise ValueError("early_stop serves counters, flags, n_iter and iter_hist only, not " +
                             ", ".join(bad))

    def decode(self, llr, T: Optional[int] = None, app: Optional[bool] = None, hard: bool = False,
               synd: bool = False, counters=None, flags: bool = False, kernel: Optional[str] = None,
               stream=None, target_bits: Optional[int] = None, iter_wrong: bool = False,
               early_stop: bool = False, n_iter: bool = False, iter_hist=None,
               on_off_grid: str = "raise", hard_last=False, word_flags: bool = False) -> DecodeResult:
        torch = self._torch
        T = self.T if T is None else int(T)
        nt = self.target_bits if target_bits is None else int(target_bits)
        if T > self.T:
            raise ValueError(f"T={T} exceeds the {self.T} iterations the weights cover")
        if hard_last is not False and hard_last is not None and early_stop:
            self._es_check_exports(app=app, hard=hard, synd=synd, iter_wrong=iter_wrong)
            llr = self._as_llr(llr)
            return self._decode_es_word(llr, int(llr.shape[0]), T, nt, hard_last, word_flags, counters, flags,
                                        n_iter, iter_hist, kernel, stream, on_off_grid)
        if hard_last is not False and hard_last is not None:
            bad = [k for k, v in dict(app=app, hard=hard, synd=synd, iter_wrong=iter_wrong,
                                      n_iter=n_iter, iter_hist=iter_hist is not None and iter_hist is not False).items() if v]
            if bad:
                raise ValueError("hard_last serves word_flags, counters and flags only, not " + ", ".join(bad))
            return self._decode_word(llr, T, nt, hard_last, word_flags, counters, flags, kernel, stream, on_off_grid)
        if word_flags:
            raise ValueError("word_flags is an output of hard_last=True")
        if early_stop:
            self._es_check_exports(app=app, hard=hard, synd=synd, iter_wrong=iter_wrong)
            if on_off_grid not in ("raise", "mark"):
                raise ValueError("on_off_grid must be 'raise' or 'mark'")
            llr = self._as_llr(llr)
            B = int(llr.shape[0])
            res = DecodeResult()
            if B == 0:
                return self._es_outputs(res, 0, T, counters, flags, n_iter, iter_hist)
            ctx = self._ensure_ctx(B, T)
            want_n = n_iter or on_off_grid == "raise"
            self._es_outputs(res, B, T, counters, flags, want_n, iter_hist)
            if stream is None:
                stream = torch.cuda.current_stream(self.device)
            ptr = lambda t: 0 if t is None else t.data_ptr()
            self._ext.decode_es(ctx, llr.data_ptr(), B, T, self.decoding_type, self.q_bit, nt, self.clip,
                                KERNELS[kernel or self.kernel], ptr(res.counters), ptr(res.flags),
                                ptr(res.n_iter), ptr(res.iter_hist), stream.cuda_stream)
            if on_off_grid == "raise":
                stream.synchronize()
                nbad = int((res.n_iter == 0).sum().item())
                if nbad:
                    raise ValueError(f"early_stop: {nbad} frames are in packs with LLRs off the quantizer "
                                     "grid and were not decoded (on_off_grid='mark' returns them marked)")
                if not n_iter:
                    res.n_iter = None
            return res
        if n_iter or (iter_hist is not None and iter_hist is not False):
            raise ValueError("n_iter and iter_hist are outputs of early_stop=True")
        app = True if app is None else app
        llr = self._as_llr(llr)
        B = int(llr.shape[0])
        if B == 0:
            return self._empty_result(T, nt, hard, synd, counters, flags, app, iter_wrong)
        ctx = self._ensure_ctx(B, T)
        res = DecodeResult()
        dev = self.device
        if app:
            res.app = torch.empty((T, B, nt), dtype=torch.float32, device=dev)
        if hard:
            res.hard = torch.empty((T, B, (self.n_vars + 31) // 32), dtype=torch.int32, device=dev)
        if synd:
            res.synd = torch.empty((T, B, (self.n_checks + 31) // 32), dtype=torch.int32, device=dev)
        if counters is True:
            counters = torch.zeros(4, dtype=torch.int64, device=dev)
        if counters is not None:
            if counters.dtype != torch.int64 or counters.numel() < 4 or counters.device != dev:
                raise ValueError("counters must be an int64[4] tensor on the decoder's device")
            res.counters = counters
        if isinstance(flags, torch.Tensor):
            if flags.dtype != torch.uint8 or flags.device != dev or flags.numel() < B:
                raise ValueError("flags tensor must be uint8 on the decoder's device, >= B long")
            res.flags = flags
        elif flags:
            res.flags = torch.empty(B, dtype=torch.uint8, device=dev)
        if iter_wrong:
            res.iter_wrong = torch.empty((T, (B + 31) // 32), dtype=torch.int32, device=dev)
        if stream is None:
            stream = torch.cuda.current_stream(dev)
        ptr = lambda t: 0 if t is None else t.data_ptr()
        self._ext.decode(ctx, llr.data_ptr(), B, T, self.decoding_type, self.q_bit,
                         nt, self.clip, KERNELS[kernel or self.kernel],
                         ptr(res.app), ptr(res.hard), ptr(res.synd), ptr(res.counters),
                         ptr(res.flags), stream.cuda_stream, ptr(res.iter_wrong))
        return res

    def generates_channel_in_kernel(self, T=None, kernel=None, app: bool = False) -> bool:
        T = self.T if T is None else T
        ctx = self._ensure_ctx(1, T)
        short = getattr(self, "short", (0, 0)) or (0, 0)
        return bool(self._ext.awgn_in_kernel(ctx, T, self.decoding_type, self.q_bit, self.target_bits,
                                             KERNELS[kernel or self.kernel], self.clip,
                                             has_short=short[0] > 0, app=app))

    def last_kernel(self) -> str:
        return "" if self._ctx is None else self._ext.last_kernel(self._ctx)

    def _empty_result(self, T, nt, hard, synd, counters, flags, app, iter_wrong=False):
        torch = self._torch
        dev = self.device
        res = DecodeResult()
        if app:
            res.app = torch.empty((T, 0, nt), dtype=torch.float32, device=dev)
        if hard:
            res.hard = torch.empty((T, 0, (self.n_vars + 31) // 32), dtype=torch.int32, device=dev)
        if synd:
            res.synd = torch.empty((T, 0, (self.n_checks + 31) // 32), dtype=torch.int32, device=dev)
        if counters is True:
            counters = torch.zeros(4, dtype=torch.int64, device=dev)
        res.counters = counters if counters is not None else None
        if isinstance(flags, torch.Tensor):
            res.flags = flags[:0]
        elif flags:
            res.flags = torch.empty(0, dtype=torch.uint8, device=dev)
        if iter_wrong:
            res.iter_wrong = torch.empty((T, 0), dtype=torch.int32, device=dev)
        return res

    def decode_awgn(self, B: int, sigma: float, seed: int, offset: int = 0, punct=None, short=None,
                    T: Optional[int] = None, app: bool = False, counters=None, flags=None,
                    kernel: Optional[str] = None, stream=None, iter_wrong: bool = False,
                    early_stop: bool = False, n_iter: bool = False, iter_hist=None,
                    hard_last=False, word_flags: bool = False) -> DecodeResult:
        want_word = hard_last is not False and hard_last is not None
        if want_word and not early_stop:
            raise ValueError("decode_awgn does not serve hard_last: use decode(awgn(...), hard_last=True)")
        if word_flags and not want_word:
            raise ValueError("word_flags is an output of hard_last=True")
        torch = self._torch
        T = self.T if T is None else int(T)
        punct = getattr(self, "punct", (0, 0)) if punct is None else punct
        short = getattr(self, "short", (0, 0)) if short is None else short
        if early_stop:
            self._es_check_exports(app=app, iter_wrong=iter_wrong)
            if T > self.T:
                raise ValueError(f"T={T} exceeds the {self.T} iterations the weights cover")
            B = int(B)
            if want_word:
                return self._decode_es_word(None, B, T, self.target_bits, hard_last, word_flags, counters, flags,
                                            n_iter, iter_hist, kernel, stream, "mark",
                                            channel=(sigma, seed, offset, punct, short))
            res = DecodeResult()
            if B == 0:
                return self._es_outputs(res, 0, T, counters, flags, n_iter, iter_hist)
            ctx = self._ensure_ctx(B, T)
            self._es_outputs(res, B, T, counters, flags, n_iter, iter_hist)
            if stream is None:
                stream = torch.cuda.current_stream(self.device)
            ptr = lambda t: 0 if t is None else t.data_ptr()
            self._ext.decode_awgn_es(ctx, B, T, self.decoding_type, self.q_bit, self.target_bits,
                                     self.clip, KERNELS[kernel or self.kernel], float(sigma), int(seed),
                                     int(offset), int(punct[0]), int(punct[1]), int(short[0]),
                                     int(short[1]), ptr(res.counters), ptr(res.flags), ptr(res.n_iter),
                                     ptr(res.iter_hist), stream.cuda_stream)
            return res
        if n_iter or (iter_hist is not None and iter_hist is not False):
            raise ValueError("n_iter and iter_hist are outputs of early_stop=True")
        if int(B) == 0:
            return self._empty_result(T, self.target_bits, False, False, counters, flags, app, iter_wrong)
        ctx = self._ensure_ctx(int(B), T)
        dev = self.device
        res = DecodeResult()
        if app:
            res.app = torch.empty((T, B, self.target_bits), dtype=torch.float32, device=dev)
        if counters is True:
            counters = torch.zeros(4, dtype=torch.int64, device=dev)
        if counters is not None:
            if counters.dtype != torch.int64 or counters.numel() < 4 or counters.device != dev:
                raise ValueError("counters must be an int64[4] tensor on the decoder's device")
            res.counters = counters
        if isinstance(flags, torch.Tensor):
            if flags.dtype != torch.uint8 or flags.device != dev or flags.numel() < B:
                raise ValueError("flags tensor must be uint8 on the decoder's device, >= B long")
            res.flags = flags
        elif flags:
            res.flags = torch.empty(B, dtype=torch.uint8, device=dev)
        if iter_wrong:
            res.iter_wrong = torch.empty((T, (int(B) + 31) // 32), dtype=torch.int32, device=dev)
        if stream is None:
            stream = torch.cuda.current_stream(dev)
        ptr = lambda t: 0 if t is None else t.data_ptr()
        self._ext.decode_awgn(ctx, int(B), T, self.decoding_type, self.q_bit, self.target_bits,
                              self.clip, KERNELS[kernel or self.kernel], float(sigma), int(seed),
                              int(offset), int(punct[0]), int(punct[1]), int(short[0]),
                              int(short[1]), ptr(res.app), ptr(res.counters), ptr(res.flags),
                              stream.cuda_stream, ptr(res.iter_wrong))
        return res

    def _uncorrected_index(self, flags, stream):
        torch = self._torch
        B = int(flags.shape[0])
        idx = torch.empty(max(B, 1), dtype=torch.int64, device=self.device)
        cnt = torch.empty(1, dtype=torch.int64, device=self.device)
        self._ext.collect_frames(flags.data_ptr(), B, 1, 1, idx.data_ptr(), B, cnt.data_ptr(),
                                 stream.cuda_stream)
        stream.synchronize()
        n = int(cnt.item())
        return torch.sort(idx[:n]).values.contiguous()

    def collect_uncorrected(self, flags, llr, stream=None):
        torch = self._torch
        if stream is None:
            stream = torch.cuda.current_stream(self.device)
        sel = self._uncorrected_index(flags, stream)
        n = int(sel.numel())
        if n == 0:
            return np.zeros((0, self.n_vars), np.float32)
        llr = llr.reshape(llr.shape[0], -1)
        rows = torch.empty((n, self.n_vars), dtype=torch.float32, device=self.device)
        for s0 in range(0, n, 65535):
            s1 = min(n, s0 + 65535)
            self._ext.gather_rows(llr.data_ptr(), self.n_vars, sel[s0:].data_ptr(), s1 - s0,
                                  rows[s0:].data_ptr(), stream.cuda_stream)
        return rows.cpu().numpy()

    def collect_uncorrected_awgn(self, flags, sigma: float, seed: int, offset: int = 0,
                                 punct=None, short=None, stream=None):
        torch = self._torch
        if stream is None:
            stream = torch.cuda.current_stream(self.device)
        punct = getattr(self, "punct", (0, 0)) if punct is None else punct
        short = getattr(self, "short", (0, 0)) if short is None else short
        with torch.cuda.stream(stream):
            sel = self._uncorrected_index(flags, stream)
            n = int(sel.numel())
            if n == 0:
                return np.zeros((0, self.n_vars), np.float32)
            rows = torch.empty((n, self.n_vars), dtype=torch.float32, device=self.device)
            self._ext.channel_awgn_rows(rows.data_ptr(), sel.data_ptr(), n, self.n_vars, float(sigma),
                                        int(seed), int(offset), self.decoding_type, self.q_bit,
                                        int(punct[0]), int(punct[1]), int(short[0]), int(short[1]),
                                        self.clip, stream.cuda_stream)
            return rows.cpu().numpy()

    def format_uncor_rows(self, rows):
        return self._ext.format_uncor_rows(rows)

    def awgn(self, B: int, sigma: float, seed: int, offset: int = 0, punct=None, short=None,
             out=None, stream=None):
        torch = self._torch
        punct = getattr(self, "punct", (0, 0)) if punct is None else punct
        short = getattr(self, "short", (0, 0)) if short is None else short
        if out is None:
            out = torch.empty((B, self.n_vars), dtype=torch.float32, device=self.device)
        if stream is None:
            stream = torch.cuda.current_stream(self.device)
        self._ext.channel_awgn(out.data_ptr(), int(B), self.n_vars, float(sigma), int(seed),
                               int(offset), self.decoding_type, self.q_bit, int(punct[0]),
                               int(punct[1]), int(short[0]), int(short[1]), self.clip,
                               stream.cuda_stream)
# ... 26 lines not shown
```

Before: 272.4 million.

## Add frozen-geometry kernel specialization for wman N576 bit-sliced decoder

Adds a compile-time specialization of the bit-sliced pack-loop kernel for the WiMAX N576 geometry. LDS offsets, thread count, column counts and check-lane counts become constexpr. The host checks that the runtime plan matches the frozen constants, adjusting for T up to 20, and routes to the new instance when it does. The aim is to cut scalar kernarg loads and runtime index arithmetic, at the price of an extra kernel instantiation and a plan-equality check that must stay in sync with the layout.

```diff
diff --git a/include/ldpc_nms.h b/include/ldpc_nms.h
--- a/include/ldpc_nms.h
+++ b/include/ldpc_nms.h
@@ -75,6 +75,8 @@
                      char* name, int32_t name_len);
 
 int ldpc_ctx_last_kernel(const ldpc_ctx* c, char* name, int32_t name_len);
+
+int ldpc_ctx_last_frozen(const ldpc_ctx* c);
 
 int ldpc_channel_awgn(float* llr_dev, int64_t B, int32_t n_vars, double sigma, uint64_t seed,
                       int64_t offset, int32_t decoding_type, int32_t q_bit, int32_t punct_start,
diff --git a/include/ldpc_nms_debug.h b/include/ldpc_nms_debug.h
--- a/include/ldpc_nms_debug.h
+++ b/include/ldpc_nms_debug.h
@@ -11,6 +11,11 @@
                          int32_t mode, int32_t alpha_uniform, int32_t beta_uniform, float clip,
                          int32_t flags, int32_t* violations, char* msg, int32_t msg_len);
 
+int ldpc_debug_bs_frozen(const int32_t* proto, int32_t M, int32_t N, int32_t z, int32_t T, int32_t mode,
+                         int32_t alpha_uniform, int32_t beta_uniform, int32_t ucn, int32_t kind,
+                         float clip, int32_t* plan, int32_t* frozen, int32_t n, char* names,
+                         int32_t names_len);
+
 #ifdef __cplusplus
 }
 #endif
diff --git a/ldpc_error_floor_amd/build.py b/ldpc_error_floor_amd/build.py
--- a/ldpc_error_floor_amd/build.py
+++ b/ldpc_error_floor_amd/build.py
@@ -18,7 +18,7 @@
 HIP_SOURCES = ["ldpc_capi.hip", "ldpc_flood.hip", "ldpc_fused.hip", "ldpc_fused5.hip",
                "ldpc_bs.hip", "ldpc_bsc.hip", "ldpc_ffl.hip", "ldpc_channel.hip", "ldpc_collect.hip",
                "ldpc_word.hip"]
-HEADERS = ["ldpc_internal.h", "ldpc_fused.h", "ldpc_fused5_kernel.h", "ldpc_bs_kernel.h", "ldpc_bs_host.h", "ldpc_bitplane.h",
+HEADERS = ["ldpc_internal.h", "ldpc_fused.h", "ldpc_fused5_kernel.h", "ldpc_bs_kernel.h", "ldpc_bs_frozen.h", "ldpc_bs_host.h", "ldpc_bitplane.h",
            "ldpc_awgn.h", "ldpc_host.h", "ldpc_quant.h"]
 HOST_SOURCES = ["ldpc_host.cpp"]
 F5_SHAPE_SRC = "ldpc_fused5_shape.hip"
diff --git a/ldpc_error_floor_amd/csrc/ldpc_bs.hip b/ldpc_error_floor_amd/csrc/ldpc_bs.hip
--- a/ldpc_error_floor_amd/csrc/ldpc_bs.hip
+++ b/ldpc_error_floor_amd/csrc/ldpc_bs.hip
@@ -212,6 +212,39 @@
         if (q.ok) return q;
     }
     return p;
+}
+
+typedef std::array<int32_t, kBsFrozenFields> BsGeoFields;
+static const char* const bs_frozen_names[kBsFrozenFields] = {
+    "inst", "n_vars", "n_checks", "z", "N", "cn_lanes", "cn_dmin", "NT", "nw", "arows", "bcols", "AL", "BL",
+    "cstride", "off_slots", "off_pad", "off_zero", "off_red", "off_alut", "off_blut", "off_ch", "lds"};
+static BsGeoFields bs_plan_fields(const DevGraph& g, const BsPlan& p) {
+    const int ar = (p.inst >= 0 && kBsInst[p.inst].UCN ? 2 : 1) * p.arows;
+    return {p.inst, g.n_vars, g.n_checks, g.z, g.N, p.cn_lanes, p.cn_dmin, 64 * p.nw, p.nw, p.arows, p.bcols,
+            ar * LUT_W, p.bcols * BLUT_W, g.z * SLOT_B, (int32_t)p.off_slots, (int32_t)p.off_pad,
+            (int32_t)p.off_zero, (int32_t)p.off_red, (int32_t)p.off_alut, (int32_t)p.off_blut,
+            (int32_t)p.off_ch, (int32_t)p.lds};
+}
+static BsGeoFields bs_frozen_fields() {
+    typedef BsFrozenWman W;
+    return {W::inst, W::n_vars, W::n_checks, W::z, W::N, W::cn_lanes, W::cn_dmin, W::NT, W::nw, W::arows,
+            W::bcols, W::AL, W::BL, (int32_t)W::cstride, (int32_t)W::off_slots, (int32_t)W::off_pad,
+            (int32_t)W::off_zero, (int32_t)W::off_red, (int32_t)W::off_alut, (int32_t)W::off_blut,
+            (int32_t)W::off_ch, (int32_t)W::lds};
+}
+static bool bs_frozen_fit(const DevGraph& g, BsPlan& p, const BsReq& r, bool exports) {
+    const char* e = getenv("LDPC_BS_FROZEN");
+    if (e && atoi(e) == 0) return false;
+    if (!p.ok || p.inst != BsFrozenWman::inst || p.ucn || r.es || exports || r.T > BsFrozenWman::T_CAP) return false;
+    BsPlan q = p;
+    const uint32_t d = (uint32_t)(((4 * BsFrozenWman::T_CAP + 15) & ~15) - ((4 * r.T + 15) & ~15));
+    q.off_alut += d;
+    q.off_blut += d;
+    q.off_ch += d;
+    q.lds += d;
+    if (bs_plan_fields(g, q) != bs_frozen_fields()) return false;
+    p = q;
+    return true;
 }
 
 #ifndef BS_DEAL_DEFAULT
@@ -652,7 +685,8 @@
 }
 
 static int bs_run(const DevGraph& g, const Bufs& b, FusedWorkspace& ws, const BsPlan& p, const float* llr,
-                  const BsReq& r, const BsOut& o, hipStream_t s) {
+                  const BsReq& r, const BsOut& o, bool frozen, hipStream_t s) {
+    ws.bs_frozen = frozen;
     void*& graph = r.es ? ws.bs_es_graph : ws.bs_graph;
     int st = bs_graph_tables(g, p, graph, r.es ? ws.bs_es_graph_inst : ws.bs_graph_inst, s);
     if (st != LDPC_OK) return st;
@@ -670,6 +704,7 @@
     a.iter_hist = o.iter_hist;
     a.hdw = o.hdw;
     a.word = o.word ? 1 : 0;
+    a.frozen = frozen;
     a.llr = llr;
     a.gen = bs_gen(b, q8_tab_lds(p));
     a.B = b.B;
@@ -725,7 +760,7 @@
     const uint64_t rkey = (uint64_t)p.inst << 48 | (uint64_t)p.nw << 32 | (uint64_t)lds;
     if (ws.bs_resident_key != rkey) {
         ws.bs_resident_key = rkey;
-        std::fill(ws.bs_resident, ws.bs_resident + 3, 0);
+        std::fill(ws.bs_resident, ws.bs_resident + 5, 0);
     }
 #ifdef BS_STAMP
     static unsigned long long* dst = nullptr;
@@ -737,8 +772,9 @@
     if (st != LDPC_OK || hipMemcpyAsync(hst, dst, sizeof(hst), hipMemcpyDeviceToHost, s) != hipSuccess ||
         hipStreamSynchronize(s) != hipSuccess)
         return st != LDPC_OK ? st : LDPC_ERR_HIP;
-    fprintf(stderr, "bs_stamp inst %d T %d q8 %d: per pack, shader clocks [check, check-barrier, var, var-barrier | "
-            "entry, channel, ch-barrier, tables, first-var, check-setup | epilogue]\n", p.inst, b.T, b.q8 != nullptr);
+    fprintf(stderr, "bs_stamp inst %d T %d q8 %d frozen %d: per pack, shader clocks [check, check-barrier, var, var-barrier | "
+            "entry, channel, ch-barrier, tables, first-var, check-setup | epilogue]\n", p.inst, b.T, b.q8 != nullptr,
+            (int)frozen);
     static const int order[] = {0, 1, 2, 3, 8, 9, 10, 11, 12, 4, 5};
     for (int w = 0; w < p.nw && w < 16; ++w) {
         const double n = (double)(hst[16 * w + 15] ? hst[16 * w + 15] : 1);
@@ -756,9 +792,11 @@
 int bs_decode(const DevGraph& g, const Bufs& b, FusedWorkspace& ws, const float* llr, const BsReq& r,
               const BsOut& o, hipStream_t s) {
     bool to_bsc;
-    const BsPlan p = bs_route(g, r, &to_bsc);
+    BsPlan p = bs_route(g, r, &to_bsc);
+    ws.bs_frozen = false;
     if (!p.ok) return to_bsc ? bsc_decode(g, b, ws, llr, r, o, s) : LDPC_ERR_UNSUPPORTED;
-    return bs_run(g, b, ws, p, llr, r, o, s);
+    const bool frozen = bs_frozen_fit(g, p, r, o.hdx != nullptr || o.hdw != nullptr);
+    return bs_run(g, b, ws, p, llr, r, o, frozen, s);
 }
 
 }
@@ -911,6 +949,43 @@
     return r.violations;
 }
 }
+}
+
+extern "C" int ldpc_debug_bs_frozen(const int32_t* proto, int32_t M, int32_t N, int32_t z, int32_t T,
+                                    int32_t mode, int32_t alpha_uniform, int32_t beta_uniform, int32_t ucn,
+                                    int32_t kind, float clip, int32_t* plan, int32_t* frozen, int32_t n,
+                                    char* names, int32_t names_len) {
+    using namespace ldpc;
+    using namespace ldpc::bs;
+    if (!proto || T <= 0 || kind < 0 || kind > 2 || n < 0) return LDPC_ERR_ARG;
+    host::GraphTables h;
+    const int st = host::build_graph(proto, M, N, z, h);
+    if (st != LDPC_OK) return st;
+    DevGraph g{};
+    g.M = h.M; g.N = h.N; g.z = h.z; g.E = h.E;
+    g.n_checks = h.M * h.z; g.n_vars = h.N * h.z; g.n_edges = h.E * h.z; g.max_cdeg = h.max_cdeg;
+    g.h_row_ptr = h.row_ptr.data();
+    g.host = &h;
+    g.w_alpha_uniform = alpha_uniform;
+    g.w_alpha_pair_uniform = alpha_uniform;
+    g.w_beta_uniform = beta_uniform;
+    g.w_beta_nonneg = 1;
+    const BsReq r{mode, ucn != 0, false, clip, T, kind == 1};
+    bool to_bsc;
+    BsPlan p = bs_route(g, r, &to_bsc);
+    const bool fz = bs_frozen_fit(g, p, r, kind == 2);
+    const BsGeoFields pf = bs_plan_fields(g, p), ff = bs_frozen_fields();
+    for (int i = 0; i < n && i < kBsFrozenFields; ++i) {
+        if (plan) plan[i] = p.ok ? pf[(size_t)i] : -1;
+        if (frozen) frozen[i] = ff[(size_t)i];
+    }
+    if (names && names_len > 0) {
+        std::string all;
+        for (int i = 0; i < kBsFrozenFields; ++i) all += std::string(i ? "," : "") + bs_frozen_names[i];
+        std::strncpy(names, all.c_str(), (size_t)names_len - 1);
+        names[names_len - 1] = 0;
+    }
+    return fz ? 1 : 0;
 }
 
 extern "C" int ldpc_debug_bs_bounds(const int32_t* proto, int32_t M, int32_t N, int32_t z, int32_t T,
diff --git a/ldpc_error_floor_amd/csrc/ldpc_bs_frozen.h b/ldpc_error_floor_amd/csrc/ldpc_bs_frozen.h
--- /dev/null
+++ b/ldpc_error_floor_amd/csrc/ldpc_bs_frozen.h
@@ -0,0 +1,25 @@
+#pragma once
+#include <cstdint>
+
+namespace ldpc {
+namespace bs {
+
+struct BsFrozenWman {
+    static constexpr int inst = 0;
+    static constexpr int n_vars = 576, n_checks = 144, z = 24, N = 24;
+    static constexpr int btid_n = N;
+    static constexpr int cn_lanes = 576, cn_dmin = 14;
+    static constexpr int NT = 576, nw = 9;
+    static constexpr int arows = 1, bcols = 1;
+    static constexpr int AL = 64, BL = 68;
+    static constexpr uint32_t cstride = 480;
+    static constexpr uint32_t off_slots = 0, off_pad = 48480, off_zero = 48500, off_red = 48528,
+                              off_alut = 48800, off_blut = 49312, off_ch = 49856;
+    static constexpr uint32_t lds = 52160;
+    static constexpr int T_CAP = 20;
+};
+
+constexpr int kBsFrozenFields = 22;
+
+}
+}
diff --git a/ldpc_error_floor_amd/csrc/ldpc_bs_kernel.h b/ldpc_error_floor_amd/csrc/ldpc_bs_kernel.h
--- a/ldpc_error_floor_amd/csrc/ldpc_bs_kernel.h
+++ b/ldpc_error_floor_amd/csrc/ldpc_bs_kernel.h
@@ -6,6 +6,7 @@
 #include "ldpc_fused.h"
 #include "ldpc_fused5_kernel.h"
 #include "ldpc_bitplane.h"
+#include "ldpc_bs_frozen.h"
 
 namespace ldpc {
 namespace bs {
@@ -446,25 +447,30 @@
     const int64_t b0 = (int64_t)(pk) * PACK;                                                       \
     const int nvalid = (int)min<int64_t>(PACK, a.B - b0);                                          \
     const uint32_t valid = (nvalid >= 32) ? 0xFFFFFFFFu : ((1u << nvalid) - 1u);                   \
-    uint32_t* RED = reinterpret_cast<uint32_t*>(smem + a.off_red);                                 \
+    uint32_t* RED = reinterpret_cast<uint32_t*>(smem + (FZ ? W::off_red : a.off_red));             \
     const int flor = 16 + ((a.T + 3) & ~3);                                                        \
-    const int AR = UCN ? 2 * a.arows : a.arows;                                                    \
-    const int AL = AR * LUT_W, BL = a.bcols * BLUT_W;                                              \
-    uint32_t* ALUT = reinterpret_cast<uint32_t*>(smem + a.off_alut);                               \
-    uint32_t* BLUT = reinterpret_cast<uint32_t*>(smem + a.off_blut);                               \
+    const int AR = UCN ? 2 * (FZ ? W::arows : a.arows) : (FZ ? W::arows : a.arows);                \
+    const int AL = AR * LUT_W, BL = (FZ ? W::bcols : a.bcols) * BLUT_W;                            \
+    uint32_t* ALUT = reinterpret_cast<uint32_t*>(smem + (FZ ? W::off_alut : a.off_alut));          \
+    uint32_t* BLUT = reinterpret_cast<uint32_t*>(smem + (FZ ? W::off_blut : a.off_blut));          \
     const bool ucn = UCN && a.ucn;                                                                 \
     auto ucn_on = [&](int t) __attribute__((always_inline)) -> bool {                              \
         return ucn && (t >= 64 || ((a.ucn_iter >> t) & 1));                                        \
     };
 
 template <int D, int DV, int LPC, int VPL, int CPL, bool UCN, bool BIG, bool PK, int WPE, bool XP, int LB, bool Q8,
-          bool ES = false, bool EW = false>
+          bool ES = false, bool EW = false, bool FZ = false>
 __global__ void __launch_bounds__(LB) __attribute__((amdgpu_waves_per_eu(WPE)))
 k_bs(std::conditional_t<ES, std::conditional_t<EW, BsArgsEw, BsArgsEs>, std::conditional_t<XP, BsArgsXp, BsArgs>> a) {
     static_assert(LPC == 2 || LPC == 4, "lanes per check");
     using KArgs = std::conditional_t<ES, std::conditional_t<EW, BsArgsEw, BsArgsEs>, std::conditional_t<XP, BsArgsXp, BsArgs>>;
     static_assert(!ES || (UCN && VPL == 1 && CPL == 1 && !XP), "early stop: one-chunk UCN-compiled instances");
     static_assert(!EW || ES, "the stop-iteration word: early-stop builds");
+    static_assert(!FZ || (BS_LOOP_TU && !UCN && !XP && !ES && VPL == 1 && CPL == 1 && D == 15 && DV == 6 && LPC == 4),
+                  "frozen geometry: the wman pack-loop builds");
+    using W = BsFrozenWman;
+    static_assert(W::cstride == W::z * SLOT_B && W::AL == W::arows * LUT_W && W::BL == W::bcols * BLUT_W &&
+                  W::NT == 64 * W::nw && W::off_zero == W::off_pad + SLOT_B, "BsFrozenWman is consistent");
     constexpr int SB = (DV * QMAX + QMAX <= 127) ? 8 : 9;
     constexpr int EPL = (D + LPC - 1) / LPC;
     constexpr bool SKIPM = CPL > 1;
@@ -497,11 +503,11 @@
 #define BS_ST(i) ((void)0)
 #endif
     const int tid = threadIdx.x;
-    const int NT = blockDim.x;
+    const int NT = FZ ? W::NT : (int)blockDim.x;
     const int lane = tid & 63;
     const int wave = __builtin_amdgcn_readfirstlane(tid >> 6);
     const int nwv = NT >> 6;
-    const int nv = a.n_vars;
+    const int nv = (FZ ? W::n_vars : a.n_vars);
 #if !BS_LOOP_TU
     BS_PACK_SETUP(blockIdx.x)
 #endif
@@ -519,10 +525,10 @@
         dw[u] = __builtin_amdgcn_readfirstlane(a.vn_wdeg[3 * (u * nwv + wave)]);
         dwmin[u] = __builtin_amdgcn_readfirstlane(a.vn_wdeg[3 * (u * nwv + wave) + 1]);
         pcol[u] = __builtin_amdgcn_readfirstlane(a.vn_wdeg[3 * (u * nwv + wave) + 2]);
-        tab_b[u] = (a.bcols > 1 && vv[u] >= 0) ? (uint32_t)(((UCN ? (vv[u] & 0xFFFF) : vv[u]) / (nv / a.bcols)) * BLUT_W * 4) : 0u;
+        tab_b[u] = ((FZ ? W::bcols : a.bcols) > 1 && vv[u] >= 0) ? (uint32_t)(((UCN ? (vv[u] & 0xFFFF) : vv[u]) / (nv / (FZ ? W::bcols : a.bcols))) * BLUT_W * 4) : 0u;
     }
     constexpr int FOLDB = BS_LOOP_TU ? 0x100 : 0;
-    int cn_dmin = a.cn_dmin | ((FOLDB && (uint32_t)wave == a.fold_wave) ? FOLDB : 0);
+    int cn_dmin = (FZ ? W::cn_dmin : a.cn_dmin) | ((FOLDB && (uint32_t)wave == a.fold_wave) ? FOLDB : 0);
 
     if (a.stagger > 0 && (int)blockIdx.x < a.stagger_n) {
         const int n = (int)(((uint32_t)blockIdx.x * 97u % (uint32_t)a.stagger_n) * (uint32_t)a.stagger /
@@ -550,17 +556,20 @@
     PackArgs& a = *kap;
     const int tid = wave * 64 + lane_now(), lane = tid & 63;
     BS_PACK_SETUP(pack)
+    [[maybe_unused]] const int pack_tbits = FZ ? a.target_bits : 0;
+#define BS_TBITS (FZ ? pack_tbits : a.target_bits)
 #define BS_PK pack
 #define BS_NEXT_PACK continue
 #define BS_LANE_IS0 (lane_now() == 0)
 #else
+#define BS_TBITS a.target_bits
 #define BS_PK blockIdx.x
 #define BS_NEXT_PACK return
 #define BS_LANE_IS0 (lane == 0)
 #endif
     if (tid < SLOT_W) {
-        reinterpret_cast<uint32_t*>(smem + a.off_pad)[tid] = 0xFFFFFFFFu;
-        reinterpret_cast<uint32_t*>(smem + a.off_zero)[tid] = 0u;
+        reinterpret_cast<uint32_t*>(smem + (FZ ? W::off_pad : a.off_pad))[tid] = 0xFFFFFFFFu;
+        reinterpret_cast<uint32_t*>(smem + (FZ ? W::off_zero : a.off_zero))[tid] = 0u;
     }
     if (UCN && tid == 0) lds_put(a.off_hdz, 0u);
     if (tid < 8) RED[tid] = (tid == 1) ? 0xFFFFFFFFu : 0u;
@@ -602,8 +611,8 @@
     uint32_t cs[VPL], cm[VPL][4], bg[VPL];
     int off = 0;
     if (T0A) {
-        copy_async(a.off_alut, a.alut, AL, wave, NT);
-        copy_async(a.off_blut, a.blut, BL, wave, NT);
+        copy_async((FZ ? W::off_alut : a.off_alut), a.alut, AL, wave, NT);
+        copy_async((FZ ? W::off_blut : a.off_blut), a.blut, BL, wave, NT);
     }
     const __amdgpu_buffer_rsrc_t llr_rs = __builtin_amdgcn_make_buffer_rsrc(
         (void*)(a.llr + b0 * nv), 0, nvalid * nv * 4, 0x00020000);
@@ -690,10 +699,10 @@
         int bk = -1;
         if constexpr (!XP) {
             if (use_bk && a.btid) {
-                const int col = (a.bcols == 1) ? 0 : pcol[u];
+                const int col = ((FZ ? W::bcols : a.bcols) == 1) ? 0 : pcol[u];
                 if (BKPF) bk = __builtin_amdgcn_readfirstlane(bkp[u]);
                 else if (col >= 0)
-                    bk = __builtin_amdgcn_readfirstlane((int)((const ConstW*)a.btid)[(size_t)tb * a.btid_n + col]);
+                    bk = __builtin_amdgcn_readfirstlane((int)((const ConstW*)a.btid)[(size_t)tb * (FZ ? W::btid_n : a.btid_n) + col]);
             }
         }
         if (ABL(2) || (tb < 64 && ((a.beta_id >> tb) & 1))) {
@@ -704,7 +713,7 @@
             PH("vn_beta_fix", u);
             beta_asm(lw, cmu, bk);
             if constexpr (BIG) {
-                if (a.bcols == 1) {
+                if ((FZ ? W::bcols : a.bcols) == 1) {
                     const ConstW* tg = (const ConstW*)(a.blut) + (size_t)tb * BLUT_W;
 #pragma unroll
                     for (int i = 0; i < 4; ++i) lw[i] = mux(bg[u], tg[LUT_W + i], lw[i]);
@@ -716,7 +725,7 @@
                     lw[3] = mux(bg[u], gb.w, lw[3]);
                 }
             }
-        } else if (a.bcols == 1) {
+        } else if ((FZ ? W::bcols : a.bcols) == 1) {
             PH("vn_beta_sg", u);
             const ConstW* tg = (const ConstW*)(a.blut) + (size_t)tb * BLUT_W;
             lut_s(lw, cmu, tg);
@@ -758,7 +767,7 @@
             const int v = (UCN && vv[u] >= 0) ? (vv[u] & 0xFFFF) : vv[u];
             const uint32_t hda = UCN ? 4u * ((uint32_t)vv[u] >> 16) : 0u;
             const uint32_t cmu[4] = {cm[u][0], cm[u][1], cm[u][2], cm[u][3]};
-            const bool counted = v >= 0 && v < a.target_bits;
+            const bool counted = v >= 0 && v < BS_TBITS;
             uint32_t lw[1][4];
             PH("vn_beta", (last ? 100 : 0) + u);
             if (!last) beta_lw(u, bslice, tb, cmu, lw[0], !first);
@@ -845,7 +854,7 @@
                     abs_sat(X, x);
 #pragma unroll
                     for (int f = 0; f < DV; ++f)
-                        if (f < dwu && (f < dwm || vaddr(f) != a.off_zero)) write_slot(vaddr(f), x[6], X);
+                        if (f < dwu && (f < dwm || vaddr(f) != (FZ ? W::off_zero : a.off_zero))) write_slot(vaddr(f), x[6], X);
                 } else {
 #pragma unroll
                     for (int f = 0; f < DV; ++f) {
@@ -865,7 +874,7 @@
                             }
                             sub_tv(x, Tv, b, n);
                             abs_sat(X, x);
-                            if (f < dwm || vaddr(f) != a.off_zero) write_slot(vaddr(f), x[6], X);
+                            if (f < dwm || vaddr(f) != (FZ ? W::off_zero : a.off_zero)) write_slot(vaddr(f), x[6], X);
                         }
                     }
                 }
@@ -901,7 +910,7 @@
         }
     };
 
-    vn_phase(true, false, a.off_blut, 0);
+    vn_phase(true, false, (FZ ? W::off_blut : a.off_blut), 0);
     BS_ST(12);
     const int cj = lane % LPC;
     int gchunk[CPL], gdeg[CPL], gm[CPL];
@@ -911,15 +920,15 @@
         gchunk[c] = (CPL == 1) ? wave : __builtin_amdgcn_readfirstlane(a.cn_chunk[wave * CPL + c]);
         const int ql = max(gchunk[c], 0) * 64 + lane;
         const int cc = ql / LPC;
-        const int ci = min(cc / a.z, a.n_checks / a.z - 1);
-        gdeg[c] = (cc < a.n_checks) ? a.row_ptr[ci + 1] - a.row_ptr[ci] : 0;
+        const int ci = min(cc / (FZ ? W::z : a.z), (FZ ? W::n_checks : a.n_checks) / (FZ ? W::z : a.z) - 1);
+        gdeg[c] = (cc < (FZ ? W::n_checks : a.n_checks)) ? a.row_ptr[ci + 1] - a.row_ptr[ci] : 0;
         gm[c] = SKIPM ? (int)__popc(wave_or((1u << ((gdeg[c] + LPC - 1) / LPC)) - 1u)) : EPL;
-        gbase[c] = a.off_slots + (uint32_t)((a.row_lay[2 * ci] + cj * a.row_lay[2 * ci + 1] + (cc - ci * a.z)) * SLOT_B);
-        gtab[c] = a.off_alut + (uint32_t)((a.arows > 1 ? ci : 0) * LUT_W * 4) + (uint32_t)(cj * OB * 64);
+        gbase[c] = (FZ ? W::off_slots : a.off_slots) + (uint32_t)((a.row_lay[2 * ci] + cj * a.row_lay[2 * ci + 1] + (cc - ci * (FZ ? W::z : a.z))) * SLOT_B);
+        gtab[c] = (FZ ? W::off_alut : a.off_alut) + (uint32_t)(((FZ ? W::arows : a.arows) > 1 ? ci : 0) * LUT_W * 4) + (uint32_t)(cj * OB * 64);
         if constexpr (PKG) gbase[c] |= gtab[c] << 16;
         if constexpr (UCN) {
 #pragma unroll
-            for (int p = 0; p < HDW; ++p) ghd[c][p] = ((ES || ucn) && gchunk[c] >= 0 && ql < a.cn_lanes) ? a.cn_hd[(size_t)ql * HDW + p] : 0u;
+            for (int p = 0; p < HDW; ++p) ghd[c][p] = ((ES || ucn) && gchunk[c] >= 0 && ql < (FZ ? W::cn_lanes : a.cn_lanes)) ? a.cn_hd[(size_t)ql * HDW + p] : 0u;
         }
     }
     constexpr bool RPW = CPL > 1;
@@ -932,10 +941,10 @@
 #pragma unroll
         for (int m = 0; m < EPL; ++m)
             if (RPW && (LPC * m + LPC - 1 < cn_dmin || LPC * m + cj < gdeg[c])) rpk |= 1u << (RB * c + m);
-    const uint32_t cstride = (uint32_t)(a.z * SLOT_B);
-    const uint32_t tabu = (uint32_t)(a.arows * LUT_W * 4);
+    const uint32_t cstride = (uint32_t)((FZ ? W::z : a.z) * SLOT_B);
+    const uint32_t tabu = (uint32_t)((FZ ? W::arows : a.arows) * LUT_W * 4);
     constexpr bool GBL = CPL == 1;
-    if constexpr (GBL) lds_put(a.off_ch + 4u * (uint32_t)tid, gbase[0]);
+    if constexpr (GBL) lds_put((FZ ? W::off_ch : a.off_ch) + 4u * (uint32_t)tid, gbase[0]);
     constexpr bool HDL = UCN && CPL == 1;
     if constexpr (HDL) {
 #pragma unroll
@@ -958,26 +967,28 @@
 #pragma unroll
         for (int u = 0; u < VPL; ++u) asm volatile("" : "+s"(dw[u]), "+s"(dwmin[u]));
         if (!RPW) asm volatile("" : "+s"(cn_dmin));
-        const int cdm = FOLDB ? (cn_dmin & (FOLDB - 1)) : cn_dmin;
+        const int cdm = FZ ? W::cn_dmin : FOLDB ? (cn_dmin & (FOLDB - 1)) : cn_dmin;
         if (RPW) {
 #pragma unroll
             for (int u = 0; u < VPL; ++u) asm volatile("" : "+v"(vv[u]));
         }
         if (t + 1 < a.T) {
-            int cw = wave, al = AL, bl = BL, bcl = a.bcols;
-            if (!(Q8 && VPL == 1 && CPL == 1 && !UCN))
+            int cw = wave, al = AL, bl = BL, bcl = (FZ ? W::bcols : a.bcols);
+            if (!FZ && !(Q8 && VPL == 1 && CPL == 1 && !UCN))
                 asm volatile("" : "+s"(cw), "+s"(al), "+s"(bl), "+s"(bcl));
             const uint32_t* alut_p = a.alut;
             const uint32_t* blut_p = a.blut;
-            uint32_t off_al = a.off_alut, off_bl = a.off_blut;
+            uint32_t off_al = (FZ ? W::off_alut : a.off_alut), off_bl = (FZ ? W::off_blut : a.off_blut);
             if constexpr (VPL == 1 && CPL == 1 && !(Q8 && !UCN)) {
                 typedef __attribute__((address_space(4))) const BsArgs ConstArgs;
                 ConstArgs* ka = (ConstArgs*)__builtin_amdgcn_kernarg_segment_ptr();
                 asm volatile("" : "+s"(ka));
                 alut_p = ka->alut;
                 blut_p = ka->blut;
-                off_al = ka->off_alut;
-                off_bl = ka->off_blut;
+                if constexpr (!FZ) {
+                    off_al = ka->off_alut;
+                    off_bl = ka->off_blut;
+                }
             }
             copy_async(off_al + 4u * (uint32_t)(nx * al), alut_p + (size_t)(t + 1) * al, al, cw, NT);
             if (bcl > 1)
@@ -987,8 +998,8 @@
             if (t + 1 < a.T && a.btid) {
 #pragma unroll
                 for (int u = 0; u < VPL; ++u) {
-                    const int col = (a.bcols == 1) ? 0 : pcol[u];
-                    bkp[u] = col >= 0 ? a.btid[(size_t)(t + 1) * a.btid_n + col] : -1;
+                    const int col = ((FZ ? W::bcols : a.bcols) == 1) ? 0 : pcol[u];
+                    bkp[u] = col >= 0 ? a.btid[(size_t)(t + 1) * (FZ ? W::btid_n : a.btid_n) + col] : -1;
                 }
             }
         }
@@ -996,7 +1007,7 @@
         if (PRIO == 4) __builtin_amdgcn_s_setprio(2);
 #pragma unroll
         for (int c = 0; c < CPL; ++c) {
-            const bool active = (CPL == 1) ? wave * 64 < a.cn_lanes : (gchunk[c] >= 0);
+            const bool active = (CPL == 1) ? (FZ && W::cn_lanes >= W::NT) || wave * 64 < (FZ ? W::cn_lanes : a.cn_lanes) : (gchunk[c] >= 0);
             if (!active || ABL(1)) continue;
             PH("ck_addr", c);
             uint32_t cbase;
@@ -1004,7 +1015,7 @@
                 uint32_t all = ~0u;
                 asm volatile("" : "+s"(all));
                 const uint32_t ln = __builtin_amdgcn_mbcnt_hi(all, __builtin_amdgcn_mbcnt_lo(all, 0u));
-                cbase = lds_w(a.off_ch + ((uint32_t)wave << 8) + 4u * ln);
+                cbase = lds_w((FZ ? W::off_ch : a.off_ch) + ((uint32_t)wave << 8) + 4u * ln);
             } else {
                 cbase = gbase[c];
                 asm volatile("" : "+v"(cbase));
@@ -1021,7 +1032,7 @@
                 else return LPC * m + LPC - 1 < cdm || LPC * m + cj < cdeg;
             };
             auto caddr = [&](int m) __attribute__((always_inline)) -> uint32_t {
-                return real(m) ? cbase + m * cstride : a.off_pad;
+                return real(m) ? cbase + m * cstride : (FZ ? W::off_pad : a.off_pad);
             };
             uint32_t Xs[EPL][4], ns[EPL];
             PH("ck_read", c);
@@ -1184,7 +1195,7 @@
             if (dw[0] >= DV - 1) __builtin_amdgcn_s_setprio(1);
             else __builtin_amdgcn_s_setprio(0);
         }
-        const uint32_t bslice = a.off_blut + (uint32_t)(nx * BL * 4);
+        const uint32_t bslice = (FZ ? W::off_blut : a.off_blut) + (uint32_t)(nx * BL * 4);
         if (t == a.T - 1) vn_phase(false, true, bslice, t + 1);
         else vn_phase(false, false, bslice, t + 1);
         BS_ST(2);
@@ -1299,6 +1310,7 @@
 #elif defined(BS_STAMP)
     const unsigned long long npk = 1ull;
 #endif
+#undef BS_TBITS
 #undef BS_PK
 #undef BS_NEXT_PACK
 #undef BS_LANE_IS0
@@ -1310,7 +1322,7 @@
         atomicAdd(a.stamps + 16 * wave + 15, npk);
         uint32_t hw;
         asm volatile("s_getreg_b32 %0, hwreg(HW_REG_HW_ID)" : "=s"(hw));
-        const uint32_t simd = (((hw >> 4) & 3u) - reinterpret_cast<uint32_t*>(smem + a.off_red)[12]) & 3u;
+        const uint32_t simd = (((hw >> 4) & 3u) - reinterpret_cast<uint32_t*>(smem + (FZ ? W::off_red : a.off_red))[12]) & 3u;
         atomicAdd(a.stamps + 16 * wave + 13 + (simd >> 1), npk << (32 * (simd & 1)));
     }
 #endif
@@ -1319,6 +1331,7 @@
 
 struct BsLaunch : BsArgsEw {
     int word;
+    bool frozen;
 };
 
 template <class K>
@@ -1341,11 +1354,11 @@
     return hipGetLastError() == hipSuccess ? LDPC_OK : LDPC_ERR_HIP;
 }
 
-template <int I, bool XP, bool Q8>
+template <int I, bool XP, bool Q8, bool FZ = false>
 int launch_bs_x(const BsLaunch& a, int npacks, int nw, size_t lds, hipStream_t s, int grid, int* resident) {
     constexpr BsInst k = kBsInst[I];
     static_assert(bs_loops(k) == (BS_LOOP_TU != 0), "BS_LOOP_TU lists the instances of bs_loops");
-    constexpr auto fn = &k_bs<k.D, k.DV, k.LPC, k.VPL, k.CPL, k.UCN, k.BIG, k.PK, k.WPE, XP, 1024, Q8>;
+    constexpr auto fn = &k_bs<k.D, k.DV, k.LPC, k.VPL, k.CPL, k.UCN, k.BIG, k.PK, k.WPE, XP, 1024, Q8, false, false, FZ>;
     int nblocks = npacks;
     if constexpr (bs_loops(k)) {
         if (grid < 0) {
@@ -1386,6 +1399,11 @@
         return q8 ? launch_bs_es_x<I, true, false>(a, npacks, nw, lds, s)
                   : launch_bs_es_x<I, false, false>(a, npacks, nw, lds, s);
     } else {
+        if constexpr (I == BsFrozenWman::inst) {
+            if (a.frozen && !a.hdx)
+                return q8 ? launch_bs_x<I, false, true, true>(a, npacks, nw, lds, s, grid, resident + 4)
+                          : launch_bs_x<I, false, false, true>(a, npacks, nw, lds, s, grid, resident + 3);
+        }
         if (a.hdx) return q8 ? LDPC_ERR_UNSUPPORTED : launch_bs_x<I, true, false>(a, npacks, nw, lds, s, grid, resident + 1);
         return q8 ? launch_bs_x<I, false, true>(a, npacks, nw, lds, s, grid, resident + 2)
                   : launch_bs_x<I, false, false>(a, npacks, nw, lds, s, grid, resident);
diff --git a/ldpc_error_floor_amd/csrc/ldpc_capi.hip b/ldpc_error_floor_amd/csrc/ldpc_capi.hip
--- a/ldpc_error_floor_amd/csrc/ldpc_capi.hip
+++ b/ldpc_error_floor_amd/csrc/ldpc_capi.hip
@@ -795,6 +795,11 @@
     return decode_bs_impl(c, llr_dev, B, p, false, bs_outs(o), stream, nullptr, nullptr);
 }
 
+int ldpc_ctx_last_frozen(const ldpc_ctx* c) {
+    if (!c) return LDPC_ERR_ARG;
+    return (c->fused.bs_frozen && std::strncmp(c->last_kernel, "bsl[", 4) == 0) ? 1 : 0;
+}
+
 int ldpc_ctx_last_kernel(const ldpc_ctx* c, char* name, int32_t name_len) {
     if (!c || !name || name_len <= 0) return LDPC_ERR_ARG;
     std::strncpy(name, c->last_kernel, (size_t)name_len - 1);
diff --git a/ldpc_error_floor_amd/csrc/ldpc_fused.h b/ldpc_error_floor_amd/csrc/ldpc_fused.h
--- a/ldpc_error_floor_amd/csrc/ldpc_fused.h
+++ b/ldpc_error_floor_amd/csrc/ldpc_fused.h
@@ -18,8 +18,9 @@
     size_t bs_lut_bytes = 0;
     uint32_t* bs_bad = nullptr;
     int64_t bs_bad_n = 0;
-    int bs_resident[3] = {0, 0, 0};
+    int bs_resident[5] = {0, 0, 0, 0, 0};
     uint64_t bs_resident_key = ~0ull;
+    bool bs_frozen = false;
     uint32_t* hdx = nullptr;
     int64_t hdx_elems = 0;
     bool bits_packed = false;
diff --git a/ldpc_error_floor_amd/csrc/pybind_module.cpp b/ldpc_error_floor_amd/csrc/pybind_module.cpp
--- a/ldpc_error_floor_amd/csrc/pybind_module.cpp
+++ b/ldpc_error_floor_amd/csrc/pybind_module.cpp
@@ -397,6 +397,14 @@
         },
         py::arg("ctx"));
     m.def(
+        "last_frozen",
+        [](Ctx& c) {
+            const int r = ldpc_ctx_last_frozen(c.h);
+            check(r < 0 ? r : 0, "ldpc_ctx_last_frozen");
+            return r == 1;
+        },
+        py::arg("ctx"));
+    m.def(
         "format_uncor_rows",
         [](py::array_t<float, py::array::c_style | py::array::forcecast> rows) {
             if (rows.ndim() != 2 || rows.shape(1) <= 0)
diff --git a/ldpc_error_floor_amd/decoder.py b/ldpc_error_floor_amd/decoder.py
--- a/ldpc_error_floor_amd/decoder.py
+++ b/ldpc_error_floor_amd/decoder.py
@@ -357,6 +357,9 @@
     def last_kernel(self) -> str:
         return "" if self._ctx is None else self._ext.last_kernel(self._ctx)
 
+    def last_frozen(self) -> bool:
+        return False if self._ctx is None else bool(self._ext.last_frozen(self._ctx))
+
     def _empty_result(self, T, nt, hard, synd, counters, flags, app, iter_wrong=False):
         torch = self._torch
         dev = self.device
```

Measured after the change: 288.8 million (median of 6 runs). 1.06x the previous value.
